# michal7kw/scRNA_seq_QAnnealing_Clustering

Measured on AMD Instinct MI355X. Metric: spin-flip updates/sec (node) + best QUBO energy vs neal, PBMC3k SNN, higher is better.
Workload: dtype f32

## Files before the change

### include/mi_sa.h

```cpp
#ifndef MI_SA_H
#define MI_SA_H

#include <stdint.h>

#ifdef __cplusplus
extern "C" {
#endif

#define MI_OK            0
#define MI_EINVAL       -1
#define MI_ENODEV       -2
#define MI_EHIP         -3
#define MI_ENOMEM       -4
#define MI_EUNSUPPORTED -5
#define MI_ESTATE       -6

#define MI_KIND_DENSE     1
#define MI_KIND_CSR_RANK1 2
#define MI_KIND_POTTS_CSR 3

typedef struct mi_sa_problem mi_sa_problem;

const char *mi_last_error(void);
int mi_abi_version(void);
int mi_device_count(int *out_count);
int mi_device_info(int device, char *name, int len, int *out_cus, uint64_t *out_hbm_bytes);


int mi_sa_problem_create_dense_f32(const float *Qs, int n, double offset, int device,
                                   mi_sa_problem **out);

int mi_sa_problem_create_csr_rank1_f32(const int32_t *rowptr, const int32_t *col, const float *val,
                                       const float *lin, float c_pair, int n, double offset,
                                       int device, mi_sa_problem **out);

int mi_sa_problem_create_potts_csr_f32(const int32_t *rowptr, const int32_t *col, const float *val,
                                       float c_pair, int n, int K, double lin_offset, int device,
                                       mi_sa_problem **out);

int mi_sa_problem_set_energy_model_f64(mi_sa_problem *p, const double *val, const double *lin, double c_pair);

int mi_sa_problem_destroy(mi_sa_problem *p);
int mi_sa_problem_info(const mi_sa_problem *p, int *kind, int *n, int *num_cases, int *device);

int mi_sa_set_option(mi_sa_problem *p, const char *key, long value);

int mi_sa_debug_pace(mi_sa_problem *p, unsigned int *out, int words);

int mi_sa_plan_slot_order(const int32_t *rowptr, const int32_t *col, int n, int slot, int64_t *out_perm);

int mi_sa_plan_slot_layout(const int32_t *rowptr, const int32_t *col, int n, int slot, int max_slots,
                           int64_t *out_pos, int *out_slots, int *out_clashes);

int mi_sa_problem_set_absent(mi_sa_problem *p, const uint8_t *absent);

int mi_sa_problem_set_pair_weights(mi_sa_problem *p, const int32_t *weights);

int mi_sa_problem_set_node_weights(mi_sa_problem *p, const int32_t *wq, const float *cw, const double *w64);

int mi_sa_problem_set_node_weight_groups(mi_sa_problem *p, int G, const float *cw, const double *c64, const double *offset);

int mi_sa_problem_set_merge_moves(mi_sa_problem *p, int interval, int proposals, const double *cq);

int mi_sa_debug_stats(mi_sa_problem *p, uint64_t *out, int words);


int mi_sa_anneal(mi_sa_problem *p, int R, uint32_t replica_offset, int num_sweeps,
                 const double *betas, uint64_t seed, const void *init, int resync_interval);

#define MI_F_CONTINUE         1u
#define MI_F_BETA_PER_REPLICA 2u
#define MI_F_TEMPS_RESIDENT   4u
#define MI_F_BETA_PER_GROUP   8u
int mi_sa_anneal_ex(mi_sa_problem *p, int R, uint32_t replica_offset, int num_sweeps,
                    const double *betas, uint64_t seed, const void *init, int resync_interval,
                    uint32_t sweep_offset, uint32_t flags);

int mi_sa_tempering_begin(mi_sa_problem *p, const double *ladder_betas, int T, int chains,
                          uint32_t first_replica, int R_local);
int mi_sa_tempering_exchange(mi_sa_problem *p, uint32_t round, uint64_t seed, const double *all_energies);
int mi_sa_tempering_exchange_dev(mi_sa_problem *p, uint32_t round, uint64_t seed, const double *d_all_energies);
int mi_sa_tempering_state(mi_sa_problem *p, int32_t *out_rung, uint64_t *out_proposed, uint64_t *out_accepted);

int mi_sa_sync(mi_sa_problem *p);

int mi_sa_device_results(mi_sa_problem *p, void **out_d_states, double **out_d_energy, int *out_R);

int mi_sa_last_kernel_ms(mi_sa_problem *p, float *out_ms);

int mi_sa_last_launch_count(mi_sa_problem *p, int *out_launches);

int mi_sa_last_kernel_name(mi_sa_problem *p, char *out, int len);

int mi_sa_fetch(mi_sa_problem *p, void *out_states, double *out_energy, uint64_t *out_stats);

int mi_sa_problem_label_agreement(mi_sa_problem *p, int groups, double *out_ari, double *out_nmi, int64_t *out_pair_sum,
                                  float *out_kernel_ms);

int mi_sa_problem_coassociation(mi_sa_problem *p, int groups, const uint16_t *ref, int Kref, const int32_t *eu,
                                const int32_t *ev, int64_t m, int64_t *out_hist, int64_t *out_rowsum, int32_t *out_edge,
                                int32_t *out_counts, float *out_kernel_ms);

int mi_sa_problem_components(mi_sa_problem *p, int32_t *out_labels, int32_t *out_count, float *out_kernel_ms);

int mi_sa_best(mi_sa_problem *p, int *out_index, double *out_energy, uint64_t *out_key,
               void *out_state);

int mi_multi_gpu_anneal(mi_sa_problem *const *problems, int ndev, int R_total, uint32_t replica_offset,
                        int num_sweeps, const double *betas, uint64_t seed, int resync_interval);
int mi_multi_gpu_best(mi_sa_problem *const *problems, int ndev, int *out_owner, uint32_t *out_global_id,
                      double *out_energy, void *out_state);
int mi_multi_gpu_fetch(mi_sa_problem *const *problems, int ndev, void *out_states, double *out_energy,
                       uint64_t *out_stats);


int mi_sa_qubo_dense_f32(const float *Qs, int n, double offset, int R, int num_sweeps,
                         const double *betas, uint64_t seed, const uint8_t *init,
                         uint8_t *out_states, double *out_energy, uint64_t *out_stats, int device);

int mi_energy_dense_f32(const float *Qs, int n, const uint8_t *X, int R, double offset,
                        double *out_energy, int device);
int mi_energy_dense_f64(const double *Qs, int n, const uint8_t *X, int R, double offset,
                        double *out_energy, int device);
int mi_energy_dense_f32_ex(const float *Qs, int n, const uint8_t *X, int R, double offset,
                           double *out_energy, int device, int path, float *out_kernel_ms);

#ifdef __cplusplus
}
#endif
#endif
```

### scrna_seq_qannealing_clustering_amd/_lib.py

```python
from __future__ import annotations

import ctypes as C
import os
import threading

_HERE = os.path.dirname(os.path.abspath(__file__))
LIB_PATH = os.environ.get("MI_SA_LIB") or os.path.join(_HERE, "libmi_sa.so")

MI_OK = 0
KIND_DENSE, KIND_CSR_RANK1, KIND_POTTS_CSR = 1, 2, 3

_lock = threading.Lock()
_lib = None


class MiSaError(RuntimeError):

    def __init__(self, code, message):
        super().__init__("libmi_sa error %d: %s" % (code, message))
        self.code = code
        self.message = message


def _declare(lib):
    u8p, u16p = C.POINTER(C.c_uint8), C.POINTER(C.c_uint16)
    i32p, f32p, f64p = C.POINTER(C.c_int32), C.POINTER(C.c_float), C.POINTER(C.c_double)
    u64p, ip, vp = C.POINTER(C.c_uint64), C.POINTER(C.c_int), C.c_void_p
    pp = C.POINTER(C.c_void_p)
    sig = {
        "mi_last_error": (C.c_char_p, []),
        "mi_abi_version": (C.c_int, []),
        "mi_device_count": (C.c_int, [ip]),
        "mi_device_info": (C.c_int, [C.c_int, C.c_char_p, C.c_int, ip, u64p]),
        "mi_sa_problem_create_dense_f32": (C.c_int, [f32p, C.c_int, C.c_double, C.c_int, pp]),
        "mi_sa_problem_create_csr_rank1_f32": (C.c_int, [i32p, i32p, f32p, f32p, C.c_float, C.c_int,
                                                         C.c_double, C.c_int, pp]),
        "mi_sa_problem_create_potts_csr_f32": (C.c_int, [i32p, i32p, f32p, C.c_float, C.c_int,
                                                         C.c_int, C.c_double, C.c_int, pp]),
        "mi_sa_problem_destroy": (C.c_int, [vp]),
        "mi_sa_problem_info": (C.c_int, [vp, ip, ip, ip, ip]),
        "mi_sa_set_option": (C.c_int, [vp, C.c_char_p, C.c_long]),
        "mi_sa_plan_slot_order": (C.c_int, [i32p, i32p, C.c_int, C.c_int, C.POINTER(C.c_int64)]),
        "mi_sa_problem_set_absent": (C.c_int, [C.c_void_p, C.POINTER(C.c_uint8)]),
        "mi_sa_problem_set_pair_weights": (C.c_int, [C.c_void_p, C.POINTER(C.c_int32)]),
        "mi_sa_problem_set_node_weights": (C.c_int, [C.c_void_p, C.POINTER(C.c_int32), C.POINTER(C.c_float),
                                                     C.POINTER(C.c_double)]),
        "mi_sa_problem_set_node_weight_groups": (C.c_int, [C.c_void_p, C.c_int, C.POINTER(C.c_float),
                                                           C.POINTER(C.c_double), C.POINTER(C.c_double)]),
        "mi_sa_problem_set_merge_moves": (C.c_int, [C.c_void_p, C.c_int, C.c_int, C.POINTER(C.c_double)]),
        "mi_sa_plan_slot_layout": (C.c_int, [i32p, i32p, C.c_int, C.c_int, C.c_int, C.POINTER(C.c_int64), C.POINTER(C.c_int), C.POINTER(C.c_int)]),
        "mi_sa_problem_set_energy_model_f64": (C.c_int, [vp, C.POINTER(C.c_double), C.POINTER(C.c_double), C.c_double]),
        "mi_sa_debug_pace": (C.c_int, [vp, C.POINTER(C.c_uint32), C.c_int]),
        "mi_sa_debug_stats": (C.c_int, [vp, u64p, C.c_int]),
        "mi_sa_anneal": (C.c_int, [vp, C.c_int, C.c_uint32, C.c_int, f64p, C.c_uint64, vp, C.c_int]),
        "mi_sa_anneal_ex": (C.c_int, [vp, C.c_int, C.c_uint32, C.c_int, f64p, C.c_uint64, vp, C.c_int,
                                      C.c_uint32, C.c_uint32]),
        "mi_sa_tempering_begin": (C.c_int, [vp, f64p, C.c_int, C.c_int, C.c_uint32, C.c_int]),
        "mi_sa_tempering_exchange": (C.c_int, [vp, C.c_uint32, C.c_uint64, f64p]),
        "mi_sa_tempering_exchange_dev": (C.c_int, [vp, C.c_uint32, C.c_uint64, vp]),
        "mi_sa_device_results": (C.c_int, [vp, pp, pp, ip]),
        "mi_sa_tempering_state": (C.c_int, [vp, i32p, u64p, u64p]),
        "mi_sa_sync": (C.c_int, [vp]),
        "mi_sa_last_kernel_ms": (C.c_int, [vp, f32p]),
        "mi_sa_last_launch_count": (C.c_int, [vp, ip]),
        "mi_sa_last_kernel_name": (C.c_int, [vp, C.c_char_p, C.c_int]),
        "mi_sa_fetch": (C.c_int, [vp, vp, f64p, u64p]),
        "mi_sa_best": (C.c_int, [vp, ip, f64p, u64p, vp]),
        "mi_multi_gpu_anneal": (C.c_int, [pp, C.c_int, C.c_int, C.c_uint32, C.c_int, f64p, C.c_uint64, C.c_int]),
        "mi_multi_gpu_best": (C.c_int, [pp, C.c_int, ip, C.POINTER(C.c_uint32), f64p, vp]),
        "mi_multi_gpu_fetch": (C.c_int, [pp, C.c_int, vp, f64p, u64p]),
        "mi_sa_qubo_dense_f32": (C.c_int, [f32p, C.c_int, C.c_double, C.c_int, C.c_int, f64p,
                                           C.c_uint64, u8p, u8p, f64p, u64p, C.c_int]),
        "mi_energy_dense_f32": (C.c_int, [f32p, C.c_int, u8p, C.c_int, C.c_double, f64p, C.c_int]),
        "mi_energy_dense_f64": (C.c_int, [f64p, C.c_int, u8p, C.c_int, C.c_double, f64p, C.c_int]),
        "mi_energy_dense_f32_ex": (C.c_int, [f32p, C.c_int, u8p, C.c_int, C.c_double, f64p, C.c_int, C.c_int,
                                             f32p]),
        "mi_snn_build_f32": (C.c_int, [f32p, C.c_int, C.c_int, C.c_int, C.c_double, C.c_int, C.c_int, pp]),
        "mi_snn_build_ex_f32": (C.c_int, [f32p, C.c_int, C.c_int, C.c_int, C.c_double, C.c_int, C.c_uint32, C.c_double,
                                          C.c_int, C.c_int, pp]),
        "mi_snn_build_rounded_f32": (C.c_int, [f32p, C.c_int, C.c_int, C.c_int, C.c_double, C.c_int, C.c_int, C.c_double,
                                               C.c_int, pp]),
        "mi_snn_fetch_codes": (C.c_int, [vp, u8p]),
        "mi_snn_info": (C.c_int, [vp, ip, ip, C.POINTER(C.c_int64), ip]),
        "mi_snn_fetch": (C.c_int, [vp, i32p, C.POINTER(C.c_int64), i32p, i32p]),
        "mi_snn_kernel_ms": (C.c_int, [vp, f32p, f32p, f32p]),
        "mi_snn_destroy": (C.c_int, [vp]),
        "mi_jaccard_cluster_stats": (C.c_int, [u64p, C.c_int, C.c_int, i32p, C.c_int, C.c_int, f64p, f64p, f64p, f64p,
                                               f64p, f32p, f32p]),
        "mi_label_agreement_u16": (C.c_int, [u16p, C.c_int, u16p, C.c_int, C.c_int, C.c_int, C.c_int, C.c_int, C.c_int,
                                             C.c_int, f64p, f64p, C.POINTER(C.c_int64), i32p, f32p]),
        "mi_sa_problem_label_agreement": (C.c_int, [vp, C.c_int, f64p, f64p, C.POINTER(C.c_int64), f32p]),
        "mi_coassociation_u16": (C.c_int, [u16p, C.c_int, C.c_int, C.c_int, C.c_int, u16p, C.c_int, i32p, i32p, C.c_int64,
                                           C.c_int, C.POINTER(C.c_int64), C.POINTER(C.c_int64), i32p, i32p, f32p]),
        "mi_sa_problem_coassociation": (C.c_int, [vp, C.c_int, u16p, C.c_int, i32p, i32p, C.c_int64, C.POINTER(C.c_int64),
                                                  C.POINTER(C.c_int64), i32p, i32p, f32p]),
        "mi_graph_components": (C.c_int, [i32p, i32p, C.c_int, u16p, u8p, C.c_int, C.c_int, C.c_uint32, i32p, i32p, f32p]),
        "mi_sa_problem_components": (C.c_int, [vp, i32p, i32p, f32p]),
        "mi_rank_sum_markers_f32": (C.c_int, [f32p, C.c_int, C.c_int, u16p, C.c_int, C.c_int, C.c_int, C.c_uint32,
                                              C.POINTER(C.c_int64), i32p, f64p, C.POINTER(C.c_int64), f32p]),
        "mi_prep_create_f32": (C.c_int, [f32p, C.c_int, C.c_int, C.c_int, pp]),
        "mi_prep_destroy": (C.c_int, [vp]),
        "mi_prep_normalize": (C.c_int, [vp, C.c_double, f32p]),
        "mi_prep_fetch_normalized": (C.c_int, [vp, f32p]),
        "mi_prep_gene_stats": (C.c_int, [vp, C.c_int, f64p, f64p, i32p, f32p]),
        "mi_prep_clipped_variance": (C.c_int, [vp, f64p, f64p, C.c_double, f64p, f32p]),
        "mi_prep_select": (C.c_int, [vp, i32p, C.c_int, f64p, f64p, C.c_double, f32p]),
        "mi_prep_fetch_scaled": (C.c_int, [vp, f32p]),
        "mi_prep_gram": (C.c_int, [vp, f64p, f32p]),
        "mi_prep_project": (C.c_int, [vp, f32p, C.c_int, f32p, f32p]),
    }
    for name, (res, args) in sig.items():
        fn = getattr(lib, name)
        fn.restype = res
        fn.argtypes = args
    return sig


EXPORTS = (
    "mi_last_error", "mi_abi_version", "mi_device_count", "mi_device_info",
    "mi_sa_problem_create_dense_f32", "mi_sa_problem_create_csr_rank1_f32",
    "mi_sa_problem_create_potts_csr_f32", "mi_sa_problem_destroy", "mi_sa_problem_info",
    "mi_sa_set_option", "mi_sa_plan_slot_order", "mi_sa_plan_slot_layout", "mi_sa_problem_set_absent", "mi_sa_problem_set_pair_weights", "mi_sa_problem_set_node_weights", "mi_sa_problem_set_node_weight_groups", "mi_sa_problem_set_merge_moves", "mi_sa_problem_set_energy_model_f64", "mi_sa_debug_pace", "mi_sa_debug_stats", "mi_sa_anneal", "mi_sa_anneal_ex", "mi_sa_tempering_begin", "mi_sa_tempering_exchange", "mi_sa_tempering_exchange_dev", "mi_sa_device_results", "mi_sa_tempering_state", "mi_sa_sync", "mi_sa_last_kernel_ms", "mi_sa_last_launch_count", "mi_sa_last_kernel_name", "mi_sa_fetch", "mi_sa_best",
    "mi_multi_gpu_anneal", "mi_multi_gpu_best", "mi_multi_gpu_fetch", "mi_sa_qubo_dense_f32", "mi_energy_dense_f32", "mi_energy_dense_f64", "mi_energy_dense_f32_ex",
    "mi_snn_build_f32", "mi_snn_build_ex_f32", "mi_snn_build_rounded_f32", "mi_snn_fetch_codes", "mi_snn_info", "mi_snn_fetch", "mi_snn_kernel_ms", "mi_snn_destroy",
    "mi_jaccard_cluster_stats", "mi_label_agreement_u16", "mi_sa_problem_label_agreement",
    "mi_coassociation_u16", "mi_sa_problem_coassociation",
    "mi_graph_components", "mi_sa_problem_components",
    "mi_rank_sum_markers_f32",
    "mi_prep_create_f32", "mi_prep_destroy", "mi_prep_normalize", "mi_prep_fetch_normalized", "mi_prep_gene_stats",
    "mi_prep_clipped_variance", "mi_prep_select", "mi_prep_fetch_scaled", "mi_prep_gram", "mi_prep_project",
)


def load():
    global _lib
    with _lock:
        if _lib is not None:
            return _lib
        if not os.path.exists(LIB_PATH):
            raise RuntimeError(
                "MI355X engine not built: %s is missing.  Build it with "
                "`python -c 'import __graft_entry__ as g; g.build()'` or "
                "`make -C scrna_seq_qannealing_clustering_amd/csrc`.  There is no CPU fallback."
                % LIB_PATH)
        try:
            import torch
        except Exception:
            pass
        try:
            lib = C.CDLL(LIB_PATH, mode=getattr(os, "RTLD_NOW", 2))
        except OSError as exc:
            raise RuntimeError("cannot load %s: %s (no CPU fallback exists)" % (LIB_PATH, exc)) from exc
        _declare(lib)
        _lib = lib
        return _lib


def check(code):
    if code != MI_OK:
        msg = load().mi_last_error()
        raise MiSaError(code, msg.decode("utf-8", "replace") if msg else "")
    return code


def device_count() -> int:
    n = C.c_int(0)
    rc = load().mi_device_count(C.byref(n))
    if rc != MI_OK:
        return 0
    return int(n.value)


def device_info(device: int = 0):
    name = C.create_string_buffer(256)
    cus = C.c_int(0)
    mem = C.c_uint64(0)
    check(load().mi_device_info(device, name, 256, C.byref(cus), C.byref(mem)))
    return {"name": name.value.decode(), "compute_units": int(cus.value), "hbm_bytes": int(mem.value)}
```

### scrna_seq_qannealing_clustering_amd/csrc/mi_sa.hip

```cpp

#include <algorithm>
#include <cmath>
#include <cstdarg>
#include <cstdint>
#include <cstdio>
#include <cstdlib>
#include <cstring>
#include <mutex>
#include <new>
#include <string>
#include <thread>
#include <type_traits>
#include <vector>

#include "../../include/mi_sa.h"

#include "mi_sa_device.h"

namespace mi_sa_impl {

thread_local std::string g_err;

thread_local std::string g_kernel;

void note_kernel(const char *fmt, ...)
{
    char buf[128];
    va_list ap;
    va_start(ap, fmt);
    vsnprintf(buf, sizeof buf, fmt, ap);
    va_end(ap);
    if (g_kernel.find(buf) == std::string::npos) g_kernel += (g_kernel.empty() ? "" : " + ") + std::string(buf);
}

int fail(int code, const char *fmt, ...)
{
    char buf[512];
    va_list ap;
    va_start(ap, fmt);
    vsnprintf(buf, sizeof buf, fmt, ap);
    va_end(ap);
    g_err = buf;
    return code;
}



__device__ __forceinline__ uint32_t sortable_f32(float v)
{
    const uint32_t b = __float_as_uint(v);
    return (b & 0x80000000u) ? ~b : (b | 0x80000000u);
}

__global__ void __launch_bounds__(1024) k_best(const double *__restrict__ energy, int R,
                                               uint32_t replica_offset,
                                               unsigned long long *__restrict__ out_key)
{
    __shared__ double s_e[16];
    __shared__ int s_i[16];
    double be = INFINITY;
    int bi = 0x7fffffff;
    for (int r = threadIdx.x; r < R; r += blockDim.x) {
        const double e = energy[r];
        if (e < be || (e == be && r < bi)) { be = e; bi = r; }
    }
#pragma unroll
    for (int off = 32; off > 0; off >>= 1) {
        const double oe = __shfl_xor(be, off, 64);
        const int oi = __shfl_xor(bi, off, 64);
        if (oe < be || (oe == be && oi < bi)) { be = oe; bi = oi; }
    }
    if ((threadIdx.x & 63) == 0) { s_e[threadIdx.x >> 6] = be; s_i[threadIdx.x >> 6] = bi; }
    __syncthreads();
    if (threadIdx.x == 0) {
        for (int w = 1; w < (int)(blockDim.x >> 6); ++w)
            if (s_e[w] < be || (s_e[w] == be && s_i[w] < bi)) { be = s_e[w]; bi = s_i[w]; }
        if (bi == 0x7fffffff) bi = 0;
        out_key[0] = ((unsigned long long)sortable_f32((float)energy[bi]) << 32) |
                     (unsigned long long)(replica_offset + (uint32_t)bi);
    }
}

__global__ void __launch_bounds__(256) k_pt_exchange(const double *__restrict__ energy, int *__restrict__ rung,
                                                     const double *__restrict__ betas,
                                                     const float *__restrict__ ladder_temps,
                                                     float *__restrict__ temps_local, int T, int lo, int hi,
                                                     uint32_t rnd, uint32_t seed_lo, uint32_t seed_hi,
                                                     unsigned long long *__restrict__ stats)
{
    extern __shared__ int holder[];
    const int c = blockIdx.x;
    for (int t = threadIdx.x; t < T; t += blockDim.x) holder[rung[c * T + t]] = c * T + t;
    __syncthreads();
    unsigned int proposed = 0, accepted = 0;
    for (int k = (int)(rnd & 1u) + 2 * (int)threadIdx.x; k + 1 < T; k += 2 * (int)blockDim.x) {
        const int a = holder[k], b = holder[k + 1];
        const double arg = (betas[k] - betas[k + 1]) * (energy[a] - energy[b]);
        ++proposed;
        const bool acc = arg >= 0.0 ||
                         -arg < (double)neglog_u(chain_word_dev((uint32_t)(c * T + k), rnd, 0xffffffffu, 3u, seed_lo, seed_hi));
        if (acc) {
            rung[a] = k + 1;
            rung[b] = k;
            ++accepted;
        }
    }
    __syncthreads();
    for (int t = threadIdx.x; t < T; t += blockDim.x) {
        const int g = c * T + t;
        if (g >= lo && g < hi) temps_local[g - lo] = ladder_temps[rung[g]];
    }
    if (proposed) { atomicAdd(&stats[0], (unsigned long long)proposed); atomicAdd(&stats[1], (unsigned long long)accepted); }
}

}
using namespace mi_sa_impl;

struct mi_sa_problem {
    int kind = 0, n = 0, K = 0, device = 0;
    double offset = 0.0;
    hipStream_t stream = nullptr;
    hipEvent_t ev0 = nullptr, ev1 = nullptr;
    int NT = 0;
    float *d_Qp = nullptr;
    float *d_Qm = nullptr;
    float *d_Qs = nullptr;
    float *d_Q2xl = nullptr, *d_diagxl = nullptr;
    void *d_xg = nullptr;
    size_t xg_bytes = 0;
    int opt_xl_batched = 0;
    int opt_xl_chain = 0;
    int opt_xl_chunk = 8;
    int opt_xl_cold_permille = 20;
    int opt_xl_async = 1;
    std::thread worker;
    int worker_rc = MI_OK;
    std::string worker_err, worker_kernel;
    int xl_chunks = 0;
    int slots = 0, D = 0;
    float c_pair = 0.0f;
    uint32_t *d_ell_col = nullptr;
    float *d_ell_val = nullptr, *d_lin = nullptr;
    double *d_ell_val64 = nullptr, *d_lin64 = nullptr;
    double c_pair64 = 0.0;
    std::vector<int32_t> h_rowptr;
    uint2 *d_rows = nullptr;
    uint32_t *d_meta = nullptr;
    std::vector<uint32_t> h_meta;
    std::vector<uint8_t> h_hole;
    uint4 *d_adj4 = nullptr;
    uint4 *d_adj4p = nullptr;
    uint4 *d_adj4r = nullptr;
    int k2p_rw = 0;
    std::vector<uint32_t> h_adj4r;
    uint32_t *d_slot_flags = nullptr;
    int k2_state_bytes = 0;
    int32_t *d_wgt = nullptr;
    int wslot = -1;
    int32_t *d_nwq = nullptr;
    float *d_ncw = nullptr;
    double *d_nw64 = nullptr;
    int ngroups = 1;
    double *d_gconst = nullptr;
    int merge_interval = 0, merge_proposals = 0;
    std::vector<double> merge_cq;
    double *d_merge_cq = nullptr;
    double merge_sumabs = 0.0;
    int k2_free_block = 0;
    int cus = 0;
    int cap_R = 0, cap_sweeps = 0;
    int last_R = 0;
    uint32_t last_offset = 0;
    bool has_run = false;
    float *d_temps = nullptr;
    void *d_init = nullptr;
    void *d_states = nullptr;
    double *d_energy = nullptr;
    unsigned long long *d_stats = nullptr;
    unsigned int *d_pace = nullptr;
    int opt_pace = 1;
    int opt_variant = 0;
    int opt_mfma_permille = 600;

    int opt_chunk_sweeps = 32;
    float *d_fields = nullptr;
    unsigned int *d_ctrl = nullptr;
    int cap_fields_R = 0;
    int opt_ondemand_permille = 40;
    int opt_debug = 0;
    int opt_min_cluster_size = 0;
    int opt_k2_waves = 0;
    int opt_k2_pair = 0;
    int opt_k2_split = 0;
    int opt_k2_wide = 0;
    int opt_k3_fast = 0;
    int opt_k2_tw = 0;
    int opt_k2_trim = 0;
    int opt_k2_split_max = 1024;
    int opt_unit_rows = 0;
    int resident_waves = 0;
    int last_launches = 1;
    std::string last_kernel;
    size_t state_elem = 1;
    int pt_T = 0, pt_chains = 0, pt_lo = 0, pt_R_local = 0;
    int *d_pt_rung = nullptr;
    double *d_pt_betas = nullptr, *d_pt_energy = nullptr;
    float *d_pt_ladder = nullptr;
    float *d_pt_temps = nullptr;
    unsigned long long *d_pt_stats = nullptr;
};

namespace {

int select_device(int device)
{
    int cnt = 0;
    hipError_t e = hipGetDeviceCount(&cnt);
    if (e != hipSuccess || cnt <= 0)
        return fail(MI_ENODEV, "no HIP device visible (%s)", hipGetErrorString(e));
    if (device < 0 || device >= cnt) return fail(MI_EINVAL, "device %d out of range [0,%d)", device, cnt);
    HIP_TRY(hipSetDevice(device));
    return MI_OK;
}

int ensure_run_buffers(mi_sa_problem *p, int R, int num_sweeps, bool need_init)
{
    if (R > p->cap_R) {
        if (p->d_states) (void)hipFree(p->d_states);
        if (p->d_energy) (void)hipFree(p->d_energy);
        if (p->d_init) { (void)hipFree(p->d_init); p->d_init = nullptr; }
        p->d_states = nullptr; p->d_energy = nullptr;
        HIP_TRY(hipMalloc(&p->d_states, (size_t)R * p->n * p->state_elem));
        HIP_TRY(hipMalloc((void **)&p->d_energy, (size_t)R * sizeof(double)));
        p->cap_R = R;
    }
    if (need_init && !p->d_init) HIP_TRY(hipMalloc(&p->d_init, (size_t)p->cap_R * p->n * p->state_elem));
    if (num_sweeps > p->cap_sweeps || !p->d_temps) {
        if (p->d_temps) (void)hipFree(p->d_temps);
        p->d_temps = nullptr;
        HIP_TRY(hipMalloc((void **)&p->d_temps, (size_t)(num_sweeps > 0 ? num_sweeps : 1) * sizeof(float)));
        p->cap_sweeps = num_sweeps;
    }
    return MI_OK;
}

int dispatch_dense(mi_sa_problem *p, const DenseArgs &a, hipStream_t st)
{
    if (p->opt_chunk_sweeps > 0 && a.num_sweeps > p->opt_chunk_sweeps && p->opt_variant != 1 && a.R >= 32 &&
        (p->cap_fields_R < a.R || !p->d_fields)) {
        if (p->d_fields) (void)hipFree(p->d_fields);
        p->d_fields = nullptr;
        HIP_TRY(hipMalloc((void **)&p->d_fields, (size_t)a.R * p->NT * 64 * sizeof(float)));
        p->cap_fields_R = a.R;
    }
    if (!p->d_ctrl) {
        HIP_TRY(hipMalloc((void **)&p->d_ctrl, kCtrlWords * sizeof(unsigned int)));
        HIP_TRY(hipMemset(p->d_ctrl, 0, kCtrlWords * sizeof(unsigned int)));
    }
    DenseLaunchCtx ctx{p->device, p->opt_pace, p->opt_variant, p->opt_unit_rows, p->opt_ondemand_permille,
                       p->opt_chunk_sweeps, p->opt_mfma_permille, p->d_fields, p->d_ctrl, p->d_pace, &p->resident_waves,
                       &p->last_launches};
    p->last_launches = 1;
    switch (p->NT) {
#define MI_CASE(N) case N: return mi_launch_dense_nt##N(ctx, a, st);
        MI_CASE(4) MI_CASE(8) MI_CASE(12) MI_CASE(16) MI_CASE(20) MI_CASE(24) MI_CASE(28)
        MI_CASE(32) MI_CASE(36) MI_CASE(40) MI_CASE(44) MI_CASE(48) MI_CASE(52) MI_CASE(56)
        MI_CASE(60) MI_CASE(64)
#undef MI_CASE
    }
    return fail(MI_EUNSUPPORTED, "dense kernel not built for NT=%d", p->NT);
}

constexpr int kMaxDenseN = 64 * 64;
constexpr int kMaxDenseXlN = 16 * 4096;

}

static int settle(mi_sa_problem *p)
{
    if (!p || !p->worker.joinable()) return MI_OK;
    p->worker.join();
    p->last_kernel = p->worker_kernel;
    if (p->worker_rc) {
        const int rc = p->worker_rc;
        p->worker_rc = MI_OK;
        return fail(rc, "%s", p->worker_err.c_str());
    }
    return MI_OK;
}

extern "C" {

const char *mi_last_error(void) { return g_err.c_str(); }

int mi_abi_version(void) { return 1; }

int mi_device_count(int *out_count)
{
    if (!out_count) return fail(MI_EINVAL, "out_count is NULL");
    int cnt = 0;
    hipError_t e = hipGetDeviceCount(&cnt);
    if (e != hipSuccess) { *out_count = 0; return fail(MI_ENODEV, "hipGetDeviceCount: %s", hipGetErrorString(e)); }
    *out_count = cnt;
    return MI_OK;
}

int mi_device_info(int device, char *name, int len, int *out_cus, uint64_t *out_hbm_bytes)
{
    int rc = select_device(device);
    if (rc) return rc;
    hipDeviceProp_t prop;
    HIP_TRY(hipGetDeviceProperties(&prop, device));
    if (name && len > 0) snprintf(name, (size_t)len, "%s (%s)", prop.name, prop.gcnArchName);
    if (out_cus) *out_cus = prop.multiProcessorCount;
    if (out_hbm_bytes) *out_hbm_bytes = (uint64_t)prop.totalGlobalMem;
    return MI_OK;
}

static int problem_common_init(mi_sa_problem *p, int device)
{
    p->device = device;
    HIP_TRY(hipStreamCreateWithFlags(&p->stream, hipStreamNonBlocking));
    HIP_TRY(hipEventCreate(&p->ev0));
    HIP_TRY(hipEventCreate(&p->ev1));
    HIP_TRY(hipMalloc((void **)&p->d_stats, 16 * sizeof(unsigned long long)));
    HIP_TRY(hipMemset(p->d_stats, 0, 16 * sizeof(unsigned long long)));
    HIP_TRY(hipMalloc((void **)&p->d_pace, kMaxChunks * kPaceWords * sizeof(unsigned int)));
    HIP_TRY(hipDeviceGetAttribute(&p->cus, hipDeviceAttributeMultiprocessorCount, device));
    return MI_OK;
}

int mi_sa_problem_create_dense_f32(const float *Qs, int n, double offset, int device,
                                   mi_sa_problem **out)
{
    if (!Qs || !out) return fail(MI_EINVAL, "NULL argument");
    if (n < 1) return fail(MI_EINVAL, "n must be >= 1 (got %d)", n);
    if (n > kMaxDenseXlN)
        return fail(MI_EUNSUPPORTED, "dense kernels support n <= %d (got %d)", kMaxDenseXlN, n);
    int rc = select_device(device);
    if (rc) return rc;
    mi_sa_problem *p = new (std::nothrow) mi_sa_problem();
    if (!p) return fail(MI_ENOMEM, "out of host memory");
    p->kind = MI_KIND_DENSE; p->n = n; p->offset = offset; p->state_elem = 1;
    rc = problem_common_init(p, device);
    if (rc) { mi_sa_problem_destroy(p); return rc; }
    if (n > kMaxDenseN) {
        p->xl_chunks = (n + 4095) / 4096;
        const size_t xstride = (size_t)p->xl_chunks * 4096;
        rc = guarded([&]() -> int {
            HIP_TRY(hipMalloc((void **)&p->d_Q2xl, (size_t)n * xstride * sizeof(float)));
            HIP_TRY(hipMalloc((void **)&p->d_diagxl, xstride * sizeof(float)));
            const int rows_per_block = 256;
            std::vector<float> blk((size_t)rows_per_block * xstride), hd(xstride, 0.0f);
            for (int r0 = 0; r0 < n; r0 += rows_per_block) {
                const int nr = n - r0 < rows_per_block ? n - r0 : rows_per_block;
                std::fill(blk.begin(), blk.begin() + (size_t)nr * xstride, 0.0f);
                for (int i = 0; i < nr; ++i) {
                    const float *row = Qs + (size_t)(r0 + i) * n;
                    float *dst = blk.data() + (size_t)i * xstride;
                    for (int j = 0; j < n; ++j) dst[j] = row[j] + row[j];
                    dst[r0 + i] = 0.0f;
                    hd[r0 + i] = row[r0 + i];
                }
                HIP_TRY(hipMemcpy(p->d_Q2xl + (size_t)r0 * xstride, blk.data(), (size_t)nr * xstride * sizeof(float), hipMemcpyHostToDevice));
            }
            HIP_TRY(hipMemcpy(p->d_diagxl, hd.data(), xstride * sizeof(float), hipMemcpyHostToDevice));
            return MI_OK;
        });
        if (rc) { mi_sa_problem_destroy(p); return rc; }
        *out = p;
        return MI_OK;
    }
    rc = guarded([&]() -> int {
        const int slots = (n + 63) / 64;
        p->NT = ((slots + 3) / 4) * 4;
        const size_t stride = (size_t)p->NT * 64;
        const int diag_row = slots * 64;
        std::vector<float> hp((size_t)(diag_row + 1) * stride, 0.0f);
        for (int i = 0; i < n; ++i) {
            const float *row = Qs + (size_t)i * n;
            float *dst = hp.data() + (size_t)i * stride;
            for (int j = 0; j < n; ++j) {
                if (j == i) continue;
                const int t = j >> 6, lane = j & 63;
                dst[((size_t)(t >> 2) * 64 + lane) * 4 + (t & 3)] = row[j] + row[j];
            }
            hp[(size_t)diag_row * stride + ((size_t)((i >> 6) >> 2) * 64 + (i & 63)) * 4 + ((i >> 6) & 3)] = row[i];
        }
        HIP_TRY(hipMalloc((void **)&p->d_Qp, hp.size() * sizeof(float)));
        HIP_TRY(hipMemcpy(p->d_Qp, hp.data(), hp.size() * sizeof(float), hipMemcpyHostToDevice));
        if (p->NT <= kMaxMfmaNT) {
            const size_t npad = (size_t)p->NT * 64;
            std::vector<float> hm((npad + 1) * npad, 0.0f);
            for (int i = 0; i < n; ++i) {
                const float *row = Qs + (size_t)i * n;
                float *dst = hm.data() + (size_t)i * npad;
                for (int j = 0; j < n; ++j) dst[j] = (j == i) ? 0.0f : row[j] + row[j];
                hm[npad * npad + i] = row[i];
            }
            HIP_TRY(hipMalloc((void **)&p->d_Qm, hm.size() * sizeof(float)));
            HIP_TRY(hipMemcpy(p->d_Qm, hm.data(), hm.size() * sizeof(float), hipMemcpyHostToDevice));
        }
        return MI_OK;
    });
    if (rc) { mi_sa_problem_destroy(p); return rc; }
    *out = p;
    return MI_OK;
}

static std::vector<uint32_t> pack_pair_adjacency(const std::vector<uint32_t> &hc, const std::vector<float> &hv, int slots, int D, int RW)
{
    const int G = D / 4, LW = RW - 4 * (G - 1);
    const size_t slot_words = (size_t)(G - 1) * 512 + (LW == 3 ? 448 : (size_t)LW * 128);
    std::vector<uint32_t> out((size_t)slots * slot_words, 0u);
    for (int t = 0; t < slots; ++t)
        for (int lane = 0; lane < 64; ++lane)
            for (int k = 0; k < RW; ++k) {
                const int g = k / 4, w = g < G - 1 ? 4 : LW;
                const size_t grp = (size_t)t * slot_words + (size_t)g * 512;
                size_t at_col = grp + (size_t)lane * w + (k & 3), at_val = at_col + (size_t)w * 64;
                if (w == 3) {
                    at_col = grp + (size_t)lane * 4 + (k & 3);
                    at_val = (k & 3) < 2 ? grp + 256 + (size_t)lane * 2 + (k & 3) : grp + 384 + (size_t)lane;
                }
                out[at_col] = 4u * hc[((size_t)t * D + k) * 64 + lane];
                memcpy(&out[at_val], &hv[((size_t)t * D + k) * 64 + lane], 4);
            }
    return out;
}

static int upload_slot_ell(mi_sa_problem *p, const int32_t *rowptr, const int32_t *col, const float *val, int n)
{
    int maxdeg = 0;
    for (int i = 0; i < n; ++i) {
        const int d = rowptr[i + 1] - rowptr[i];
        if (d < 0) return fail(MI_EINVAL, "rowptr is not monotone at %d", i);
        if (d > maxdeg) maxdeg = d;
    }
    if (maxdeg > 4096)
        return fail(MI_EUNSUPPORTED, "max degree %d exceeds the widest adjacency layout (4096); use the dense kernel", maxdeg);
    const int D = maxdeg <= 16 ? 16 : (maxdeg <= 32 ? 32 : (maxdeg <= 64 ? 64 : ((maxdeg + 15) / 16) * 16));
    const int slots = (n + 63) / 64;
    std::vector<uint32_t> hc((size_t)slots * D * 64);
    std::vector<float> hv((size_t)slots * D * 64, 0.0f);
    for (int t = 0; t < slots; ++t)
        for (int lane = 0; lane < 64; ++lane) {
            const int i = t * 64 + lane;
            for (int k = 0; k < D; ++k) hc[((size_t)t * D + k) * 64 + lane] = (uint32_t)(i < n ? i : 0);
            if (i >= n) continue;
            for (int e = rowptr[i], k = 0; e < rowptr[i + 1]; ++e, ++k) {
                if (col[e] < 0 || col[e] >= n || col[e] == i)
                    return fail(MI_EINVAL, "bad column %d in row %d", col[e], i);
                hc[((size_t)t * D + k) * 64 + lane] = (uint32_t)col[e];
                hv[((size_t)t * D + k) * 64 + lane] = val[e];
            }
        }
    HIP_TRY(hipMalloc((void **)&p->d_ell_col, hc.size() * sizeof(uint32_t)));
    HIP_TRY(hipMalloc((void **)&p->d_ell_val, hv.size() * sizeof(float)));
    HIP_TRY(hipMemcpy(p->d_ell_col, hc.data(), hc.size() * sizeof(uint32_t), hipMemcpyHostToDevice));
    HIP_TRY(hipMemcpy(p->d_ell_val, hv.data(), hv.size() * sizeof(float), hipMemcpyHostToDevice));
    p->slots = slots;
    p->D = D;
    p->h_rowptr.assign(rowptr, rowptr + n + 1);
    {
        std::vector<uint2> hr((size_t)slots * 64 * D);
        std::vector<uint32_t> hm((size_t)slots * 64, 0u);
        for (int i = 0; i < slots * 64; ++i) {
            uint2 *row = hr.data() + (size_t)i * D;
            for (int k = 0; k < D; ++k) row[k] = make_uint2((uint32_t)(i < n ? i : 0), 0u);
            if (i >= n) { hm[i] = 0x80000000u; continue; }
            int k = 0, nin = 0;
            for (int pass = 0; pass < 2; ++pass)
                for (int e = rowptr[i]; e < rowptr[i + 1]; ++e) {
                    const bool in_slot = (col[e] >> 6) == (i >> 6);
                    if (in_slot != (pass == 0)) continue;
                    uint32_t bits;
                    memcpy(&bits, &val[e], 4);
                    row[k++] = make_uint2((uint32_t)col[e], bits);
                    nin += in_slot ? 1 : 0;
                }
            hm[i] = (uint32_t)nin | ((uint32_t)k << 8);
        }
        HIP_TRY(hipMalloc((void **)&p->d_rows, hr.size() * sizeof(uint2)));
        HIP_TRY(hipMalloc((void **)&p->d_meta, hm.size() * sizeof(uint32_t)));
        HIP_TRY(hipMemcpy(p->d_rows, hr.data(), hr.size() * sizeof(uint2), hipMemcpyHostToDevice));
        HIP_TRY(hipMemcpy(p->d_meta, hm.data(), hm.size() * sizeof(uint32_t), hipMemcpyHostToDevice));
        p->h_meta = hm;
        if (p->kind == MI_KIND_POTTS_CSR && (D == 16 || D == 32) && (size_t)slots * 128 + 256 <= 160 * 1024) {
            bool any_in_slot = false;
            for (size_t i = 0; i < hm.size(); ++i) any_in_slot = any_in_slot || (hm[i] & 0xffu) != 0u;
            if (!any_in_slot) {
                const int G = D / 4;
                std::vector<uint32_t> ha((size_t)slots * G * 2 * 64 * 4, 0u);
                for (int t = 0; t < slots; ++t)
                    for (int lane = 0; lane < 64; ++lane)
                        for (int k = 0; k < D; ++k) {
                            const size_t base = (((size_t)t * G + k / 4) * 2) * 256 + (size_t)lane * 4 + (k & 3);
                            ha[base] = 2u * hc[((size_t)t * D + k) * 64 + lane];
                            memcpy(&ha[base + 256], &hv[((size_t)t * D + k) * 64 + lane], 4);
                        }
                HIP_TRY(hipMalloc((void **)&p->d_adj4p, ha.size() * sizeof(uint32_t)));
                HIP_TRY(hipMemcpy(p->d_adj4p, ha.data(), ha.size() * sizeof(uint32_t), hipMemcpyHostToDevice));
            }
        }
        if (p->kind == MI_KIND_CSR_RANK1) {
            const int G = D / 4;
            const char *force = getenv("MI_K2_STATE");
#ifdef MI_K2_DEBUG_BUILD
            const bool debug_linear = getenv("MI_K2_DEBUG_LINEAR") != nullptr;
#endif
            const bool fits_half = (size_t)slots * 128 * 16 <= 144 * 1024, fits_byte = (size_t)slots * 64 * 16 <= 144 * 1024;
            p->k2_state_bytes = fits_half ? 2 : (fits_byte ? 1 : 0);
            if (force && !strcmp(force, "byte") && fits_byte) p->k2_state_bytes = 1;
            if (force && !strcmp(force, "bit")) p->k2_state_bytes = 0;
            std::vector<uint32_t> ha((size_t)slots * G * 2 * 64 * 4, 0u), hf((size_t)slots, 0u);
            for (int t = 0; t < slots; ++t)
                for (int lane = 0; lane < 64; ++lane) {
                    if (hm[(size_t)t * 64 + lane] & 0xffu) hf[t] = 1u;
                    for (int k = 0; k < D; ++k) {
                        const uint32_t c = hc[((size_t)t * D + k) * 64 + lane];
                        uint32_t vb;
                        memcpy(&vb, &hv[((size_t)t * D + k) * 64 + lane], 4);
                        const size_t base = (((size_t)t * G + k / 4) * 2) * 256 + (size_t)lane * 4 + (k & 3);
#ifdef MI_K2_DEBUG_BUILD
                        if (debug_linear) {
                            ha[base] = (uint32_t)((lane * 2 + ((k * 128) % (slots * 128))));
                            ha[base + 256] = vb;
                            continue;
                        }
#endif
                        ha[base] = p->k2_state_bytes == 2 ? 2u * c
                                 : (p->k2_state_bytes == 1 ? c : ((((c >> 5) * 4u) << 8) | (c & 31u)));
                        ha[base + 256] = vb;
                    }
                }
            HIP_TRY(hipMalloc((void **)&p->d_adj4, ha.size() * sizeof(uint32_t)));
            HIP_TRY(hipMalloc((void **)&p->d_slot_flags, hf.size() * sizeof(uint32_t)));
            HIP_TRY(hipMemcpy(p->d_adj4, ha.data(), ha.size() * sizeof(uint32_t), hipMemcpyHostToDevice));
            HIP_TRY(hipMemcpy(p->d_slot_flags, hf.data(), hf.size() * sizeof(uint32_t), hipMemcpyHostToDevice));
            bool any_general = false;
            for (int t = 0; t < slots; ++t) any_general = any_general || hf[t] != 0u;
            p->k2_free_block = any_general ? 0 : 64;
            for (int B : {256, 128}) {
                if (any_general || slots % 4 != 0) continue;
                bool ok = true;
                for (int i = 0; i < n && ok; ++i)
                    for (int e = rowptr[i]; e < rowptr[i + 1]; ++e)
                        if (col[e] / B == i / B) { ok = false; break; }
                if (ok) { p->k2_free_block = B; break; }
            }
            if (!any_general && (D == 16 || D == 32) && (size_t)slots * 256 + 4096 <= 160 * 1024) {
                for (int t = 0; t < slots; ++t)
                    for (int lane = 0; lane < 64; ++lane)
                        for (int k = 0; k < D; ++k)
                            ha[(((size_t)t * G + k / 4) * 2) * 256 + (size_t)lane * 4 + (k & 3)] =
#ifdef MI_K2_DEBUG_BUILD
                                debug_linear ? (uint32_t)(lane * 4 + (k * 256) % (slots * 256)) :
#endif
                                4u * hc[((size_t)t * D + k) * 64 + lane];
                HIP_TRY(hipMalloc((void **)&p->d_adj4p, ha.size() * sizeof(uint32_t)));
                HIP_TRY(hipMemcpy(p->d_adj4p, ha.data(), ha.size() * sizeof(uint32_t), hipMemcpyHostToDevice));
                if (D == 16 && maxdeg >= 13 && maxdeg < 16) {
                    p->h_adj4r = pack_pair_adjacency(hc, hv, slots, D, maxdeg);
                    p->k2p_rw = maxdeg;
                    if (maxdeg != 15) {
                        HIP_TRY(hipMalloc((void **)&p->d_adj4r, p->h_adj4r.size() * sizeof(uint32_t)));
                        HIP_TRY(hipMemcpy(p->d_adj4r, p->h_adj4r.data(), p->h_adj4r.size() * sizeof(uint32_t), hipMemcpyHostToDevice));
                        std::vector<uint32_t>().swap(p->h_adj4r);
                    }
                }
            }
        }
    }
    return MI_OK;
}

static int plan_slot_order_impl(const int32_t *rowptr, const int32_t *col, int n, int slot, int64_t *perm)
{
    const int nslots = (n + slot - 1) / slot;
    if (nslots <= 1 || n > (1 << 18)) {
        for (int i = 0; i < n; ++i) perm[i] = i;
        return MI_OK;
    }
    for (int i = 0; i < n; ++i)
        if (rowptr[i + 1] < rowptr[i]) return fail(MI_EINVAL, "rowptr is not monotone at %d", i);
    int maxdeg = 0;
    for (int i = 0; i < n; ++i) maxdeg = std::max(maxdeg, rowptr[i + 1] - rowptr[i]);
    std::vector<int> start((size_t)maxdeg + 2, 0), order((size_t)n);
    for (int i = 0; i < n; ++i) start[(size_t)(maxdeg - (rowptr[i + 1] - rowptr[i])) + 1]++;
    for (int d = 0; d <= maxdeg; ++d) start[(size_t)d + 1] += start[(size_t)d];
    for (int i = 0; i < n; ++i) order[(size_t)start[(size_t)(maxdeg - (rowptr[i + 1] - rowptr[i]))]++] = i;
    std::vector<int> fill((size_t)nslots, 0), cap((size_t)nslots, slot), where((size_t)n, -1), stamp((size_t)nslots, -1);
    cap[(size_t)nslots - 1] = n - slot * (nslots - 1);
    for (int v : order) {
        for (int e = rowptr[v]; e < rowptr[v + 1]; ++e) {
            if (col[e] < 0 || col[e] >= n) return fail(MI_EINVAL, "bad column %d in row %d", col[e], v);
            const int w = where[(size_t)col[e]];
            if (w >= 0) stamp[(size_t)w] = v;
        }
        int best = -1, best_nb = -1;
        for (int s = 0; s < nslots; ++s) {
            if (fill[(size_t)s] >= cap[(size_t)s]) continue;
            if (stamp[(size_t)s] == v) { if (best_nb < 0 || fill[(size_t)s] < fill[(size_t)best_nb]) best_nb = s; }
            else if (best < 0 || fill[(size_t)s] < fill[(size_t)best]) best = s;
        }
        const int s = best >= 0 ? best : best_nb;
        where[(size_t)v] = s;
        fill[(size_t)s]++;
    }
    std::vector<int> pos((size_t)nslots + 1, 0);
    for (int i = 0; i < n; ++i) pos[(size_t)where[(size_t)i] + 1]++;
    for (int s = 0; s < nslots; ++s) pos[(size_t)s + 1] += pos[(size_t)s];
    for (int i = 0; i < n; ++i) perm[pos[(size_t)where[(size_t)i]]++] = i;
    return MI_OK;
}

static int greedy_slots(const int32_t *rowptr, const int32_t *col, int n, int slot, int nslots,
                        const std::vector<int> &order, std::vector<int> &where)
{
    std::vector<int> fill((size_t)nslots, 0), stamp((size_t)nslots, -1);
    where.assign((size_t)n, -1);
    int clashes = 0;
    for (int v : order) {
        for (int e = rowptr[v]; e < rowptr[v + 1]; ++e) {
            const int w = where[(size_t)col[e]];
            if (w >= 0) stamp[(size_t)w] = v;
        }
        int best = -1, best_nb = -1;
        for (int s = 0; s < nslots; ++s) {
            if (fill[(size_t)s] >= slot) continue;
            if (stamp[(size_t)s] == v) { if (best_nb < 0 || fill[(size_t)s] < fill[(size_t)best_nb]) best_nb = s; }
            else if (best < 0 || fill[(size_t)s] < fill[(size_t)best]) best = s;
        }
        const int s = best >= 0 ? best : best_nb;
        if (best < 0) ++clashes;
        where[(size_t)v] = s;
        fill[(size_t)s]++;
    }
    return clashes;
}

static int plan_slot_layout_impl(const int32_t *rowptr, const int32_t *col, int n, int slot, int max_slots,
                                 int64_t *pos, int *out_slots, int *out_clashes)
{
    const int s0 = (n + slot - 1) / slot;
    if (max_slots < s0) max_slots = s0;
    for (int i = 0; i < n; ++i) {
        if (rowptr[i + 1] < rowptr[i]) return fail(MI_EINVAL, "rowptr is not monotone at %d", i);
        for (int e = rowptr[i]; e < rowptr[i + 1]; ++e)
            if (col[e] < 0 || col[e] >= n) return fail(MI_EINVAL, "bad column %d in row %d", col[e], i);
    }
    if (n > (1 << 18)) {
        int clashes = 0;
        for (int i = 0; i < n; ++i) {
            pos[i] = i;
            for (int e = rowptr[i]; e < rowptr[i + 1]; ++e)
                if (col[e] / slot == i / slot) { ++clashes; break; }
        }
        *out_slots = s0;
        if (out_clashes) *out_clashes = clashes;
        return MI_OK;
    }
    int maxdeg = 0;
    for (int i = 0; i < n; ++i) maxdeg = std::max(maxdeg, rowptr[i + 1] - rowptr[i]);
    std::vector<int> start((size_t)maxdeg + 2, 0), order((size_t)n);
    for (int i = 0; i < n; ++i) start[(size_t)(maxdeg - (rowptr[i + 1] - rowptr[i])) + 1]++;
    for (int d = 0; d <= maxdeg; ++d) start[(size_t)d + 1] += start[(size_t)d];
    for (int i = 0; i < n; ++i) order[(size_t)start[(size_t)(maxdeg - (rowptr[i + 1] - rowptr[i]))]++] = i;
    std::vector<int> where, first_where;
    int nslots = s0, clashes = 0, first_clashes = 0;
    for (;;) {
        clashes = greedy_slots(rowptr, col, n, slot, nslots, order, where);
        if (nslots == s0) { first_where = where; first_clashes = clashes; }
        if (clashes == 0) break;
        const int next = nslots + std::max(1, nslots / 8);
        if (next > max_slots) { where = first_where; clashes = first_clashes; nslots = s0; break; }
        nslots = next;
    }
    if (clashes == 0 && nslots > s0 && n <= 2048) {
        const int C = nslots;
        std::vector<unsigned char> seen((size_t)n * C, 0);
        std::vector<int> sat((size_t)n, 0), colour((size_t)n, -1), fill2((size_t)C, 0);
        int used = 0;
        bool ok = true;
        for (int step = 0; step < n && ok; ++step) {
            int v = -1;
            for (int u = 0; u < n; ++u) {
                if (colour[(size_t)u] >= 0) continue;
                if (v < 0) { v = u; continue; }
                const int du = rowptr[u + 1] - rowptr[u], dv = rowptr[v + 1] - rowptr[v];
                if (sat[(size_t)u] > sat[(size_t)v] || (sat[(size_t)u] == sat[(size_t)v] && du > dv)) v = u;
            }
            int c = 0;
            while (c < C && (seen[(size_t)v * C + c] || fill2[(size_t)c] >= slot)) ++c;
            if (c >= C) { ok = false; break; }
            colour[(size_t)v] = c;
            fill2[(size_t)c]++;
            used = std::max(used, c + 1);
            if (used >= C) { ok = false; break; }
            for (int e = rowptr[v]; e < rowptr[v + 1]; ++e) {
                const int u = col[e];
                if (!seen[(size_t)u * C + c]) { seen[(size_t)u * C + c] = 1; sat[(size_t)u]++; }
            }
        }
        if (ok && used < nslots && used >= s0) {
            where = colour;
            nslots = used;
        }
    }
    std::vector<int> seat((size_t)nslots, 0);
    for (int i = 0; i < n; ++i) pos[i] = (int64_t)where[(size_t)i] * slot + seat[(size_t)where[(size_t)i]]++;
    *out_slots = nslots;
    if (out_clashes) *out_clashes = clashes;
    return MI_OK;
}

int mi_sa_plan_slot_layout(const int32_t *rowptr, const int32_t *col, int n, int slot, int max_slots,
                           int64_t *out_pos, int *out_slots, int *out_clashes)
{
    if (!rowptr || !out_pos || !out_slots || (n > 0 && rowptr[n] > 0 && !col)) return fail(MI_EINVAL, "NULL argument");
    if (n < 1 || slot < 1) return fail(MI_EINVAL, "n and slot must be >= 1");
    return guarded([&]() -> int { return plan_slot_layout_impl(rowptr, col, n, slot, max_slots, out_pos, out_slots, out_clashes); });
}

int mi_sa_plan_slot_order(const int32_t *rowptr, const int32_t *col, int n, int slot, int64_t *out_perm)
{
    if (!rowptr || !out_perm || (n > 0 && rowptr[n] > 0 && !col)) return fail(MI_EINVAL, "NULL argument");
    if (n < 0 || slot < 1) return fail(MI_EINVAL, "n must be >= 0 and slot >= 1");
    return guarded([&]() -> int { return plan_slot_order_impl(rowptr, col, n, slot, out_perm); });
}

int mi_sa_problem_create_csr_rank1_f32(const int32_t *rowptr, const int32_t *col, const float *val,
                                       const float *lin, float c_pair, int n, double offset, int device,
                                       mi_sa_problem **out)
{
    if (!rowptr || !lin || !out || (rowptr[n > 0 ? n : 0] > 0 && (!col || !val))) return fail(MI_EINVAL, "NULL argument");
    if (n < 1) return fail(MI_EINVAL, "n must be >= 1 (got %d)", n);
    if (n > (1 << 20)) return fail(MI_EUNSUPPORTED, "csr_rank1 kernel supports n <= 1048576 (got %d)", n);
    int rc = select_device(device);
    if (rc) return rc;
    mi_sa_problem *p = new (std::nothrow) mi_sa_problem();
    if (!p) return fail(MI_ENOMEM, "out of host memory");
    p->kind = MI_KIND_CSR_RANK1; p->n = n; p->K = 2; p->offset = offset; p->state_elem = 1; p->c_pair = c_pair;
    rc = problem_common_init(p, device);
    if (!rc) rc = guarded([&]() -> int { return upload_slot_ell(p, rowptr, col, val, n); });
    if (!rc) rc = guarded([&]() -> int {
        std::vector<float> hl((size_t)p->slots * 64, INFINITY);
        for (int i = 0; i < n; ++i) hl[i] = lin[i];
        p->h_hole.assign((size_t)n, 0);
        for (int i = 0; i < n; ++i) p->h_hole[(size_t)i] = std::isinf(lin[i]) ? 1 : 0;
        HIP_TRY(hipMalloc((void **)&p->d_lin, hl.size() * sizeof(float)));
        HIP_TRY(hipMemcpy(p->d_lin, hl.data(), hl.size() * sizeof(float), hipMemcpyHostToDevice));
        if (!p->h_adj4r.empty()) {
            const size_t slot_words = p->h_adj4r.size() / (size_t)p->slots;
            for (int t = 0; t < p->slots; ++t)
                for (int lane = 0; lane < 64; ++lane)
                    memcpy(&p->h_adj4r[(size_t)t * slot_words + 3 * 512 + (size_t)lane * 4 + 3], &hl[(size_t)t * 64 + lane], 4);
            HIP_TRY(hipMalloc((void **)&p->d_adj4r, p->h_adj4r.size() * sizeof(uint32_t)));
            HIP_TRY(hipMemcpy(p->d_adj4r, p->h_adj4r.data(), p->h_adj4r.size() * sizeof(uint32_t), hipMemcpyHostToDevice));
            std::vector<uint32_t>().swap(p->h_adj4r);
        }
        return MI_OK;
    });
    if (rc) { mi_sa_problem_destroy(p); return rc; }
    *out = p;
    return MI_OK;
}

int mi_sa_problem_create_potts_csr_f32(const int32_t *rowptr, const int32_t *col, const float *val,
                                       float c_pair, int n, int K, double lin_offset, int device,
                                       mi_sa_problem **out)
{
    if (!rowptr || !out || (rowptr[n > 0 ? n : 0] > 0 && (!col || !val))) return fail(MI_EINVAL, "NULL argument");
    if (n < 1) return fail(MI_EINVAL, "n must be >= 1 (got %d)", n);
    if (K < 1 || K > 64) return fail(MI_EUNSUPPORTED, "potts kernel supports 1 <= K <= 64 cases (got %d)", K);
    if (n > 40000) return fail(MI_EUNSUPPORTED, "potts kernel supports n <= 40000 (got %d)", n);
    int rc = select_device(device);
    if (rc) return rc;
    mi_sa_problem *p = new (std::nothrow) mi_sa_problem();
    if (!p) return fail(MI_ENOMEM, "out of host memory");
    p->kind = MI_KIND_POTTS_CSR; p->n = n; p->K = K; p->offset = lin_offset; p->state_elem = 2; p->c_pair = c_pair;
    for (int e = 0; e < rowptr[n]; ++e) p->merge_sumabs += std::fabs((double)val[e]);
    rc = problem_common_init(p, device);
    if (!rc) rc = guarded([&]() -> int { return upload_slot_ell(p, rowptr, col, val, n); });
    if (rc) { mi_sa_problem_destroy(p); return rc; }
    *out = p;
    return MI_OK;
}

static int set_energy_model_impl(mi_sa_problem *p, const double *val, const double *lin, double c_pair)
{
    if (const int rc_w = settle(p)) return rc_w;
    if (!p) return fail(MI_EINVAL, "NULL problem");
    if (p->kind != MI_KIND_CSR_RANK1 && p->kind != MI_KIND_POTTS_CSR)
        return fail(MI_EUNSUPPORTED, "an fp64 energy model is defined for the structured kinds only");
    const int n = p->n, D = p->D;
    const int64_t nnz = p->h_rowptr.empty() ? 0 : p->h_rowptr[n];
    if ((nnz > 0 && !val) || (p->kind == MI_KIND_CSR_RANK1 && !lin)) return fail(MI_EINVAL, "NULL argument");
    HIP_TRY(hipSetDevice(p->device));
    HIP_TRY(hipStreamSynchronize(p->stream));
    std::vector<double> hv((size_t)p->slots * D * 64, 0.0), hl((size_t)p->slots * 64, 0.0);
    for (int i = 0; i < n; ++i) {
        const int t = i >> 6, lane = i & 63;
        for (int e = p->h_rowptr[i], k = 0; e < p->h_rowptr[i + 1]; ++e, ++k) hv[((size_t)t * D + k) * 64 + lane] = val[e];
        if (lin) hl[i] = lin[i];
    }
    if (!p->d_ell_val64) HIP_TRY(hipMalloc((void **)&p->d_ell_val64, hv.size() * sizeof(double)));
    if (!p->d_lin64) HIP_TRY(hipMalloc((void **)&p->d_lin64, hl.size() * sizeof(double)));
    HIP_TRY(hipMemcpy(p->d_ell_val64, hv.data(), hv.size() * sizeof(double), hipMemcpyHostToDevice));
    HIP_TRY(hipMemcpy(p->d_lin64, hl.data(), hl.size() * sizeof(double), hipMemcpyHostToDevice));
    p->c_pair64 = c_pair;
    return MI_OK;
}

int mi_sa_problem_set_absent(mi_sa_problem *p, const uint8_t *absent)
{
    if (!p || !absent) return fail(MI_EINVAL, "NULL argument");
    if (const int rc_w = settle(p)) return rc_w;
    if (p->kind != MI_KIND_POTTS_CSR)
        return fail(MI_EUNSUPPORTED, "holes of a Potts model only (a binary CSR model marks them by lin = +inf)");
    return guarded([&]() -> int {
        for (int i = 0; i < p->n; ++i) {
            if (absent[i] && (p->h_meta[(size_t)i] & 0x00ffff00u))
                return fail(MI_EINVAL, "variable %d is marked absent but has couplings", i);
            p->h_meta[(size_t)i] = (p->h_meta[(size_t)i] & 0x7fffffffu) | (absent[i] ? 0x80000000u : 0u);
        }
        HIP_TRY(hipSetDevice(p->device));
        HIP_TRY(hipStreamSynchronize(p->stream));
        HIP_TRY(hipMemcpy(p->d_meta, p->h_meta.data(), p->h_meta.size() * sizeof(uint32_t), hipMemcpyHostToDevice));
        return MI_OK;
    });
}

int mi_sa_problem_set_pair_weights(mi_sa_problem *p, const int32_t *weights)
{
    if (!p || !weights) return fail(MI_EINVAL, "NULL argument");
    if (const int rc_w = settle(p)) return rc_w;
    if (p->kind != MI_KIND_CSR_RANK1)
        return fail(MI_EUNSUPPORTED, "pair-term weights: structured binary (CSR + uniform pair) problems only");
    return guarded([&]() -> int {
        int wslot = -1;
        for (int i = 0; i < p->n; ++i) {
            if (p->h_meta[(size_t)i] >> 31) continue;
            const bool hole = !p->h_hole.empty() && p->h_hole[(size_t)i];
            if (hole) continue;
            if (weights[i] < 1) return fail(MI_EINVAL, "weight %d of variable %d: weights are positive integers", weights[i], i);
            if (weights[i] > (1 << 20)) return fail(MI_EINVAL, "weight %d of variable %d exceeds 2^20", weights[i], i);
            if (weights[i] == 1) continue;
            if (p->h_rowptr[(size_t)i + 1] != p->h_rowptr[(size_t)i])
                return fail(MI_EINVAL, "variable %d has weight %d and sparse couplings: weighted variables couple through the pair term only", i, weights[i]);
            if (wslot >= 0 && wslot != i / 64)
                return fail(MI_EINVAL, "variables with weights other than 1 in slots %d and %d: they must share one 64-variable slot", wslot, i / 64);
            wslot = i / 64;
        }
        std::vector<int32_t> hw(64, 0);
        if (wslot >= 0) {
            for (int l = 0; l < 64; ++l) {
                const int i = wslot * 64 + l;
                if (i >= p->n || (!p->h_hole.empty() && p->h_hole[(size_t)i])) continue;
                hw[(size_t)l] = weights[i];
            }
            for (int l = 0; l < 64; ++l) {
                const int i = wslot * 64 + l;
                if (i < p->n && hw[(size_t)l] != 0 && p->h_rowptr[(size_t)i + 1] != p->h_rowptr[(size_t)i])
                    return fail(MI_EINVAL, "variable %d shares the weighted slot %d and has sparse couplings", i, wslot);
            }
        }
        HIP_TRY(hipSetDevice(p->device));
        HIP_TRY(hipStreamSynchronize(p->stream));
        if (!p->d_wgt) HIP_TRY(hipMalloc((void **)&p->d_wgt, 64 * sizeof(int32_t)));
        HIP_TRY(hipMemcpy(p->d_wgt, hw.data(), 64 * sizeof(int32_t), hipMemcpyHostToDevice));
        p->wslot = wslot;
        return MI_OK;
    });
}

int mi_sa_problem_set_node_weights(mi_sa_problem *p, const int32_t *wq, const float *cw, const double *w64)
{
    if (!p || !wq || !cw) return fail(MI_EINVAL, "NULL argument");
    if (const int rc_w = settle(p)) return rc_w;
    if (p->kind != MI_KIND_POTTS_CSR) return fail(MI_EINVAL, "node weights: Potts problems only");
    if (p->has_run) return fail(MI_EINVAL, "node weights must be set before the first anneal");
    if (p->opt_min_cluster_size > 0) return fail(MI_EUNSUPPORTED, "node weights together with min_cluster_size are not supported");
    return guarded([&]() -> int {
        const size_t seats = (size_t)p->slots * 64;
        std::vector<int32_t> hq(seats, 0);
        std::vector<float> hc(seats, 0.0f);
        std::vector<double> hw(seats, 0.0);
        int64_t total = 0;
        for (int i = 0; i < p->n; ++i) {
            if (p->h_meta[(size_t)i] >> 31) continue;
            if (wq[i] < 0 || (w64 && !(w64[i] >= 0.0)))
                return fail(MI_EINVAL, "weight of variable %d is negative", i);
            total += wq[i];
            if (total > (int64_t)1 << 30) return fail(MI_EINVAL, "the node weights sum to more than 2^30");
            hq[(size_t)i] = wq[i];
            hc[(size_t)i] = cw[i];
            hw[(size_t)i] = w64 ? w64[i] : (double)wq[i];
        }
        HIP_TRY(hipSetDevice(p->device));
        HIP_TRY(hipStreamSynchronize(p->stream));
        if (!p->d_nwq) HIP_TRY(hipMalloc((void **)&p->d_nwq, seats * sizeof(int32_t)));
        if (!p->d_ncw) HIP_TRY(hipMalloc((void **)&p->d_ncw, seats * sizeof(float)));
        if (!p->d_nw64) HIP_TRY(hipMalloc((void **)&p->d_nw64, seats * sizeof(double)));
        HIP_TRY(hipMemcpy(p->d_nwq, hq.data(), seats * sizeof(int32_t), hipMemcpyHostToDevice));
        HIP_TRY(hipMemcpy(p->d_ncw, hc.data(), seats * sizeof(float), hipMemcpyHostToDevice));
        HIP_TRY(hipMemcpy(p->d_nw64, hw.data(), seats * sizeof(double), hipMemcpyHostToDevice));
        return MI_OK;
    });
}

int mi_sa_problem_set_node_weight_groups(mi_sa_problem *p, int G, const float *cw, const double *c64, const double *offset)
{
    if (!p || !cw || !c64 || !offset) return fail(MI_EINVAL, "NULL argument");
    if (const int rc_w = settle(p)) return rc_w;
    if (G < 1 || G > 256) return fail(MI_EINVAL, "resolution groups: 1 .. 256 (got %d)", G);
    if (!p->d_nwq) return fail(MI_EINVAL, "resolution groups need node weights (mi_sa_problem_set_node_weights) first");
    if (p->has_run) return fail(MI_EINVAL, "resolution groups must be set before the first anneal");
    return guarded([&]() -> int {
        const size_t seats = (size_t)p->slots * 64;
        std::vector<float> hc((size_t)G * seats, 0.0f);
        for (int g = 0; g < G; ++g) {
            for (int i = 0; i < p->n; ++i)
                if (!(p->h_meta[(size_t)i] >> 31)) hc[(size_t)g * seats + i] = cw[(size_t)g * p->n + i];
        }
        HIP_TRY(hipSetDevice(p->device));
        HIP_TRY(hipStreamSynchronize(p->stream));
        if (G != p->ngroups) {
            HIP_TRY(hipFree(p->d_ncw));
            p->d_ncw = nullptr;
            HIP_TRY(hipMalloc((void **)&p->d_ncw, (size_t)G * seats * sizeof(float)));
            p->ngroups = G;
        }
        if (!p->d_gconst) HIP_TRY(hipMalloc((void **)&p->d_gconst, 2 * 256 * sizeof(double)));
        std::vector<double> hk(c64, c64 + G);
        hk.insert(hk.end(), offset, offset + G);
        HIP_TRY(hipMemcpy(p->d_ncw, hc.data(), hc.size() * sizeof(float), hipMemcpyHostToDevice));
        HIP_TRY(hipMemcpy(p->d_gconst, hk.data(), hk.size() * sizeof(double), hipMemcpyHostToDevice));
        return MI_OK;
    });
}

static int merge_fixed_exponent(double sumabs)
{
    if (!(sumabs > 0.0)) return 0;
    int E = 0;
    const double m = std::frexp(sumabs, &E);
    const int f = 62 - E + (m == 0.5 ? 1 : 0);
    return f < -1000 ? -1000 : (f > 1000 ? 1000 : f);
}

int mi_sa_problem_set_merge_moves(mi_sa_problem *p, int interval, int proposals, const double *cq)
{
    if (!p) return fail(MI_EINVAL, "NULL problem");
    if (const int rc_w = settle(p)) return rc_w;
    if (p->kind != MI_KIND_POTTS_CSR) return fail(MI_EINVAL, "merge moves: Potts problems only");
    if (interval < 0) return fail(MI_EINVAL, "merge interval must be >= 0 (got %d)", interval);
    if (proposals < 1) return fail(MI_EINVAL, "merge proposals must be >= 1 (got %d)", proposals);
    if (interval == 0) { p->merge_interval = 0; return MI_OK; }
    if (p->K < 2) return fail(MI_EINVAL, "merge moves need K >= 2");
    if (p->d_nwq && !cq) return fail(MI_EINVAL, "merge moves on a problem with node weights need the coefficients cq");
    if (p->opt_min_cluster_size > 0) return fail(MI_EUNSUPPORTED, "merge moves together with min_cluster_size are not supported");
    if (p->pt_T > 0) return fail(MI_EUNSUPPORTED, "merge moves under tempering are not supported");
    return guarded([&]() -> int {
        const int G = p->ngroups;
        std::vector<double> h((size_t)G, (double)p->c_pair);
        if (cq)
            for (int g = 0; g < G; ++g) {
                if (!std::isfinite(cq[g])) return fail(MI_EINVAL, "cq[%d] is not finite", g);
                h[(size_t)g] = cq[g];
            }
        HIP_TRY(hipSetDevice(p->device));
        HIP_TRY(hipStreamSynchronize(p->stream));
        if (!p->d_merge_cq) HIP_TRY(hipMalloc((void **)&p->d_merge_cq, 256 * sizeof(double)));
        HIP_TRY(hipMemcpy(p->d_merge_cq, h.data(), h.size() * sizeof(double), hipMemcpyHostToDevice));
        p->merge_cq = cq ? h : std::vector<double>();
        p->merge_interval = interval;
        p->merge_proposals = proposals;
        return MI_OK;
    });
}

int mi_sa_problem_set_energy_model_f64(mi_sa_problem *p, const double *val, const double *lin, double c_pair)
{
    return guarded([&]() -> int { return set_energy_model_impl(p, val, lin, c_pair); });
}

int mi_sa_problem_destroy(mi_sa_problem *p)
{
    if (!p) return MI_OK;
    (void)settle(p);
    (void)hipSetDevice(p->device);
    if (p->stream) (void)hipStreamSynchronize(p->stream);
    void *bufs[] = {p->d_merge_cq, p->d_gconst, p->d_nwq, p->d_ncw, p->d_nw64, p->d_wgt, p->d_xg, p->d_pt_rung, p->d_pt_betas, p->d_pt_energy, p->d_pt_ladder, p->d_pt_temps, p->d_pt_stats, p->d_adj4p, p->d_adj4r, p->d_ell_val64, p->d_lin64, p->d_Q2xl, p->d_diagxl, p->d_rows, p->d_meta, p->d_adj4, p->d_slot_flags, p->d_Qm, p->d_fields, p->d_ctrl, p->d_ell_col, p->d_ell_val, p->d_lin, p->d_pace, p->d_Qp, p->d_Qs, p->d_temps, p->d_init, p->d_states, p->d_energy, p->d_stats};
    for (void *b : bufs)
        if (b) (void)hipFree(b);
    if (p->ev0) (void)hipEventDestroy(p->ev0);
    if (p->ev1) (void)hipEventDestroy(p->ev1);
    if (p->stream) (void)hipStreamDestroy(p->stream);
    delete p;
    return MI_OK;
}

int mi_sa_problem_info(const mi_sa_problem *p, int *kind, int *n, int *num_cases, int *device)
{
    if (!p) return fail(MI_EINVAL, "NULL problem");
    if (kind) *kind = p->kind;
    if (n) *n = p->n;
    if (num_cases) *num_cases = p->K;
    if (device) *device = p->device;
    return MI_OK;
}

int mi_sa_debug_stats(mi_sa_problem *p, uint64_t *out, int words)
{
    if (!p || !out) return fail(MI_EINVAL, "NULL argument");
    if (const int rc_w = settle(p)) return rc_w;
    HIP_TRY(hipSetDevice(p->device));
    HIP_TRY(hipStreamSynchronize(p->stream));
    if (words > 16) words = 16;
    HIP_TRY(hipMemcpy(out, p->d_stats, (size_t)words * sizeof(uint64_t), hipMemcpyDeviceToHost));
    if (words == 16 && p->d_ctrl) {
        unsigned int c[2] = {0, 0};
        HIP_TRY(hipMemcpy(c, p->d_ctrl + 4, sizeof c, hipMemcpyDeviceToHost));
        out[14] = c[0]; out[15] = c[1];
    }
    return MI_OK;
}

int mi_sa_debug_pace(mi_sa_problem *p, unsigned int *out, int words)
{
    if (!p || !out) return fail(MI_EINVAL, "NULL argument");
    if (const int rc_w = settle(p)) return rc_w;
    HIP_TRY(hipSetDevice(p->device));
    HIP_TRY(hipStreamSynchronize(p->stream));
    if (words > kPaceWords) words = kPaceWords;
    HIP_TRY(hipMemcpy(out, p->d_pace, (size_t)words * sizeof(unsigned int), hipMemcpyDeviceToHost));
    return MI_OK;
}

int mi_sa_set_option(mi_sa_problem *p, const char *key, long value)
{
    if (!p || !key) return fail(MI_EINVAL, "NULL argument");
    if (const int rc_w = settle(p)) return rc_w;
    if (!strcmp(key, "pace")) { p->opt_pace = value != 0; return MI_OK; }
    if (!strcmp(key, "xl_batched") && value >= 0 && value <= 2) { p->opt_xl_batched = (int)value; return MI_OK; }
    if (!strcmp(key, "xl_chunk") && value >= 1) { p->opt_xl_chunk = (int)value; return MI_OK; }
    if (!strcmp(key, "xl_chain") && value >= 0 && value <= 2) { p->opt_xl_chain = (int)value; return MI_OK; }
    if (!strcmp(key, "xl_cold_permille") && value >= 0 && value <= 1000) { p->opt_xl_cold_permille = (int)value; return MI_OK; }
    if (!strcmp(key, "xl_async") && value >= 0 && value <= 1) { p->opt_xl_async = (int)value; return MI_OK; }
    if (!strcmp(key, "mfma_permille") && value >= 0 && value <= 1000) { p->opt_mfma_permille = (int)value; return MI_OK; }
    if (!strcmp(key, "chunk_sweeps") && value >= 0) { p->opt_chunk_sweeps = (int)value; return MI_OK; }
    if (!strcmp(key, "ondemand_permille") && value >= 0 && value <= 1000) { p->opt_ondemand_permille = (int)value; return MI_OK; }
    if (!strcmp(key, "debug")) { p->opt_debug = (int)value; return MI_OK; }
    if (!strcmp(key, "k2_waves") && ((value >= 0 && value <= 16) || value == 99)) { p->opt_k2_waves = (int)value; return MI_OK; }
    if (!strcmp(key, "k2_pair") && value >= 0 && value <= 2) { p->opt_k2_pair = (int)value; return MI_OK; }
    if (!strcmp(key, "k2_split") && value >= 0 && value <= 2) { p->opt_k2_split = (int)value; return MI_OK; }
    if (!strcmp(key, "k2_split_max") && value >= 0) { p->opt_k2_split_max = (int)value; return MI_OK; }
    if (!strcmp(key, "k2_wide") && value >= 0 && value <= 2) { p->opt_k2_wide = (int)value; return MI_OK; }
    if (!strcmp(key, "k2_tw") && value >= 0 && value <= 2) { p->opt_k2_tw = (int)value; return MI_OK; }
    if (!strcmp(key, "k2_trim") && value >= 0 && value <= 2) { p->opt_k2_trim = (int)value; return MI_OK; }
    if (!strcmp(key, "k3_fast") && value >= 0 && value <= 2) { p->opt_k3_fast = (int)value; return MI_OK; }
    if (!strcmp(key, "min_cluster_size") && value >= 0) {
        if (p->kind != MI_KIND_POTTS_CSR) return fail(MI_EINVAL, "min_cluster_size applies to Potts problems");
        if (value > 0 && p->d_nwq) return fail(MI_EUNSUPPORTED, "min_cluster_size together with node weights is not supported");
        if (value > 0 && p->merge_interval > 0) return fail(MI_EUNSUPPORTED, "min_cluster_size together with merge moves is not supported");
        p->opt_min_cluster_size = (int)value;
        return MI_OK;
    }
    if (!strcmp(key, "variant") && value >= 0 && value <= 4) { p->opt_variant = (int)value; return MI_OK; }
    if (!strcmp(key, "unit_rows") && (value == 0 || value == 2 || value == 4)) { p->opt_unit_rows = (int)value; return MI_OK; }
    return fail(MI_EINVAL, "unknown option '%s'", key);
}

static int anneal_ex_impl(mi_sa_problem *p, int R, uint32_t replica_offset, int num_sweeps,
                          const double *betas, uint64_t seed, const void *init, int resync_interval,
                          uint32_t sweep_offset, uint32_t flags)
{
    if (const int rc_w = settle(p)) return rc_w;
    const bool cont = (flags & MI_F_CONTINUE) != 0, resident = (flags & MI_F_TEMPS_RESIDENT) != 0;
    const bool per_replica = (flags & MI_F_BETA_PER_REPLICA) != 0 || resident;
    const bool per_group = (flags & MI_F_BETA_PER_GROUP) != 0;
    if (flags & ~(uint32_t)(MI_F_CONTINUE | MI_F_BETA_PER_REPLICA | MI_F_TEMPS_RESIDENT | MI_F_BETA_PER_GROUP))
        return fail(MI_EINVAL, "unknown flags 0x%x", flags);
    if (!p) return fail(MI_EINVAL, "NULL problem");
    const int G = p->ngroups;
    if (per_group && per_replica) return fail(MI_EINVAL, "MI_F_BETA_PER_GROUP together with per-replica temperatures");
    if (G > 1 && per_replica)
        return fail(MI_EUNSUPPORTED, "resolution groups together with per-replica or resident temperatures are not supported");
    if (R % G != 0) return fail(MI_EINVAL, "R = %d is not a multiple of the %d resolution groups", R, G);
    const int num_betas = per_replica ? R : (per_group ? G * num_sweeps : num_sweeps);
    if (resident && (p->pt_T == 0 || p->pt_R_local != R))
        return fail(MI_ESTATE, "MI_F_TEMPS_RESIDENT needs mi_sa_tempering_begin for %d replicas on this problem", R);
    if (R < 1) return fail(MI_EINVAL, "R must be >= 1 (got %d)", R);
    if (num_sweeps < 0) return fail(MI_EINVAL, "num_sweeps must be >= 0");
    if (num_betas > 0 && num_sweeps > 0 && !betas && !resident) return fail(MI_EINVAL, "betas is NULL");
    if (cont && (!p || !p->has_run || p->last_R != R))
        return fail(MI_ESTATE, "MI_F_CONTINUE needs a previous run with the same number of replicas");
    if (cont && init) return fail(MI_EINVAL, "MI_F_CONTINUE and init are mutually exclusive");
    if (resync_interval < 0) return fail(MI_EINVAL, "resync_interval must be >= 0");
    const bool merges = p->kind == MI_KIND_POTTS_CSR && p->merge_interval > 0 && num_sweeps > 0;
    if (merges && resident) return fail(MI_EUNSUPPORTED, "merge moves with resident (tempering) temperatures are not supported");
    if (merges && p->d_nwq && p->merge_cq.empty())
        return fail(MI_EINVAL, "merge moves on a problem with node weights need the coefficients cq");
    if (merges && !p->merge_cq.empty() && p->merge_cq.size() != (size_t)G)
        return fail(MI_EINVAL, "merge moves: %zu coefficients for %d resolution groups", p->merge_cq.size(), G);
    for (int s = 0; s < (num_sweeps > 0 && !resident ? num_betas : 0); ++s)
        if (!(betas[s] > 0.0) || !std::isfinite(betas[s]))
            return fail(MI_EINVAL, "betas[%d] = %g is not a positive finite number", s, betas[s]);
    HIP_TRY(hipSetDevice(p->device));
    int rc = ensure_run_buffers(p, R, G * num_sweeps > num_betas ? G * num_sweeps : num_betas, init != nullptr);
    if (rc) return rc;
    if (!resident) {
        std::vector<float> temps((size_t)(num_betas > 0 ? num_betas : 1), 1.0f);
        for (int s = 0; s < (num_sweeps > 0 ? num_betas : 0); ++s) temps[s] = (float)(1.0 / betas[s]);
        HIP_TRY(hipMemcpyAsync(p->d_temps, temps.data(), temps.size() * sizeof(float), hipMemcpyHostToDevice, p->stream));
    }
    if (init)
        HIP_TRY(hipMemcpyAsync(p->d_init, init, (size_t)R * p->n * p->state_elem, hipMemcpyHostToDevice, p->stream));
    HIP_TRY(hipMemsetAsync(p->d_stats, 0, 16 * sizeof(unsigned long long), p->stream));
    if (!resident || init)
        HIP_TRY(hipStreamSynchronize(p->stream));
    g_kernel.clear();
    const float *temps_buf = resident ? p->d_pt_temps : p->d_temps;

    if (p->kind == MI_KIND_DENSE && p->xl_chunks > 0) {
        DenseXlArgs a;
        a.Q2 = p->d_Q2xl; a.diag = p->d_diagxl; a.temps = temps_buf;
        a.init = cont ? (const uint8_t *)p->d_states : (init ? (const uint8_t *)p->d_init : nullptr);
        a.states = (uint8_t *)p->d_states; a.energy = p->d_energy; a.stats = p->d_stats;
        a.offset = p->offset; a.n = p->n; a.R = R; a.num_sweeps = num_sweeps; a.resync = resync_interval;
        a.replica_offset = replica_offset; a.seed_lo = (uint32_t)seed; a.seed_hi = (uint32_t)(seed >> 32);
        a.sweep_offset = sweep_offset; a.temps_per_replica = per_replica ? 1 : 0;
        a.xg_chain = p->opt_xl_chain;
        p->last_launches = 1;
        const bool batched = p->opt_xl_batched == 1 || (p->opt_xl_batched == 0 && (R >= 256 || p->n >= 16384));
        if (batched) {
            const size_t need = mi_dense_xg_workspace_bytes(p->n, R);
            if (need > p->xg_bytes) {
                if (p->d_xg) HIP_TRY(hipFree(p->d_xg));
                p->d_xg = nullptr; p->xg_bytes = 0;
                HIP_TRY(hipMalloc(&p->d_xg, need));
                p->xg_bytes = need;
            }
        }
        HIP_TRY(hipEventRecord(p->ev0, p->stream));
        if (!batched) {
            rc = mi_launch_dense_xl(a, p->xl_chunks, p->stream);
        } else if (resync_interval > 0 || per_replica || num_sweeps <= p->opt_xl_chunk || p->opt_xl_cold_permille == 0) {
            rc = mi_launch_dense_xg(a, p->xl_chunks, p->d_xg, p->stream, 3);
        } else {
            auto cooling_run = [p, a, num_sweeps, R]() -> int {
                HIP_TRY(hipSetDevice(p->device));
                int rc = MI_OK, s0 = 0;
                while (!rc && s0 < num_sweeps) {
                    const int len = num_sweeps - s0 < p->opt_xl_chunk ? num_sweeps - s0 : p->opt_xl_chunk;
                    DenseXlArgs b = a;
                    b.num_sweeps = len; b.temps = a.temps + s0; b.sweep_offset = a.sweep_offset + (uint32_t)s0;
                    unsigned long long before = 0, after = 0;
                    HIP_TRY(hipMemcpyAsync(&before, p->d_stats + 1, sizeof before, hipMemcpyDeviceToHost, p->stream));
                    rc = mi_launch_dense_xg(b, p->xl_chunks, p->d_xg, p->stream, (s0 == 0 ? 1 : 0) | 2);
                    if (rc) break;
                    s0 += len;
                    if (s0 >= num_sweeps) break;
                    HIP_TRY(hipMemcpyAsync(&after, p->d_stats + 1, sizeof after, hipMemcpyDeviceToHost, p->stream));
                    HIP_TRY(hipStreamSynchronize(p->stream));
                    const double share = (double)(after - before) / ((double)R * (double)p->n * (double)len);
                    if (share * 1000.0 < (double)p->opt_xl_cold_permille) {
                        DenseXlArgs c = a;
                        c.num_sweeps = num_sweeps - s0; c.temps = a.temps + s0; c.sweep_offset = a.sweep_offset + (uint32_t)s0;
                        c.init = (const uint8_t *)p->d_states;
                        c.fields_in = mi_dense_xg_fields(p->d_xg);
                        c.fin_ncols = (p->n + 255) / 256 * 256;
                        rc = mi_launch_dense_xl(c, p->xl_chunks, p->stream);
                        break;
                    }
                }
                if (rc) return rc;
                HIP_TRY(hipEventRecord(p->ev1, p->stream));
                return MI_OK;
            };
            if (p->opt_xl_async) {
                p->last_R = R; p->last_offset = replica_offset; p->has_run = true;
                p->worker = std::thread([p, cooling_run]() {
                    g_kernel.clear(); g_err.clear();
                    p->worker_rc = cooling_run();
                    p->worker_err = g_err;
                    p->worker_kernel = g_kernel;
                });
                return MI_OK;
            }
            rc = cooling_run();
            if (rc) return rc;
            p->last_R = R; p->last_offset = replica_offset; p->has_run = true;
            p->last_kernel = g_kernel;
            return MI_OK;
        }
        if (rc) return rc;
        HIP_TRY(hipEventRecord(p->ev1, p->stream));
    } else if (p->kind == MI_KIND_DENSE) {
        DenseArgs a;
        a.Qp = p->d_Qp; a.Qm = p->d_Qm; a.temps = temps_buf;
        a.init = cont ? (const uint8_t *)p->d_states : (init ? (const uint8_t *)p->d_init : nullptr);
        a.states = (uint8_t *)p->d_states; a.energy = p->d_energy; a.stats = p->d_stats; a.pace = nullptr;
        a.offset = p->offset; a.n = p->n; a.R = R; a.num_sweeps = num_sweeps; a.resync = resync_interval;
        a.replica_offset = replica_offset; a.seed_lo = (uint32_t)seed; a.seed_hi = (uint32_t)(seed >> 32);
        a.debug = p->opt_debug; a.ondemand_flips = 0; a.sweep_offset = sweep_offset; a.temps_per_replica = per_replica ? 1 : 0;
        HIP_TRY(hipEventRecord(p->ev0, p->stream));
        rc = dispatch_dense(p, a, p->stream);
        if (rc) return rc;
        HIP_TRY(hipEventRecord(p->ev1, p->stream));
    } else {
        EllArgs a;
        a.ell_col = p->d_ell_col; a.ell_val = p->d_ell_val; a.lin = p->d_lin; a.temps = temps_buf;
        a.init = cont ? p->d_states : (init ? p->d_init : nullptr); a.states = p->d_states; a.energy = p->d_energy; a.stats = p->d_stats;
        a.c_pair = p->c_pair; a.offset = p->offset; a.n = p->n; a.K = p->K; a.R = R; a.num_sweeps = num_sweeps;
        a.resync = resync_interval; a.slots = p->slots; a.D = p->D;
        a.replica_offset = replica_offset; a.seed_lo = (uint32_t)seed; a.seed_hi = (uint32_t)(seed >> 32);
        a.sweep_offset = sweep_offset; a.temps_per_replica = per_replica ? 1 : 0;
        a.rows = p->d_rows; a.meta = p->d_meta; a.adj4 = p->d_adj4; a.slot_flags = p->d_slot_flags; a.state_bytes = p->k2_state_bytes; a.waves_override = p->opt_k2_waves; a.min_size = p->opt_min_cluster_size;
        a.ell_val64 = p->d_ell_val64; a.lin64 = p->d_lin64; a.c_pair64 = p->c_pair64;
        a.wgt = p->d_wgt; a.wslot = p->kind == MI_KIND_CSR_RANK1 ? p->wslot : -1;
        a.adj4_trim = p->opt_k2_trim != 2 ? p->d_adj4r : nullptr; a.trim_rw = p->k2p_rw;
        a.nwq = p->d_nwq; a.ncw = p->d_ncw; a.nw64 = p->d_nw64;
        a.groups = G; a.temps_group_stride = per_group ? num_sweeps : 0; a.gconst = p->d_gconst;
        if (p->kind == MI_KIND_POTTS_CSR && init) {
            const uint16_t *l = static_cast<const uint16_t *>(init);
            for (size_t k = 0; k < (size_t)R * p->n; ++k)
                if (l[k] >= (uint16_t)p->K) return fail(MI_EINVAL, "initial label %u >= K = %d", (unsigned)l[k], p->K);
        }
        p->last_launches = 1;
        HIP_TRY(hipEventRecord(p->ev0, p->stream));
        if (p->kind == MI_KIND_POTTS_CSR) {
            const bool fast = p->d_adj4p && p->opt_k3_fast != 2 && mi_potts_fast_eligible(p->D, p->K, a.min_size);
            auto anneal_launch = [&](EllArgs &b) -> int {
                if (fast) {
                    b.adj4 = p->d_adj4p;
                    return mi_launch_potts_fast(b, p->opt_k2_tw != 2 && R <= 1024, p->stream);
                }
                return mi_launch_potts(b, p->stream);
            };
            if (!merges) {
                rc = anneal_launch(a);
            } else {
                MergeArgs m;
                m.ell_col = p->d_ell_col; m.ell_val = p->d_ell_val; m.meta = p->d_meta; m.nwq = p->d_nwq;
                m.cq = p->d_merge_cq; m.temps = temps_buf; m.temps_per_replica = per_replica ? 1 : 0;
                m.temps_group_stride = a.temps_group_stride; m.states = static_cast<uint16_t *>(p->d_states);
                m.stats = p->d_stats;
                const int f = merge_fixed_exponent(p->merge_sumabs);
                m.scale = std::ldexp(1.0, f); m.inv_scale = std::ldexp(1.0, -f);
                m.n = p->n; m.K = p->K; m.R = R; m.D = p->D; m.groups = G; m.proposals = p->merge_proposals;
                m.replica_offset = replica_offset; m.seed_lo = a.seed_lo; m.seed_hi = a.seed_hi;
                const uint32_t M = (uint32_t)p->merge_interval;
                const void *labels = a.init;
                int launches = 0, merge_launches = 0;
                for (int s0 = 0; !rc && s0 < num_sweeps;) {
                    const uint32_t s = sweep_offset + (uint32_t)s0;
                    if (s > 0 && s % M == 0) {
                        m.src = static_cast<const uint16_t *>(labels); m.sweep = s; m.sweep_local = s0;
                        rc = mi_launch_potts_merge(m, p->stream);
                        if (rc) break;
                        labels = p->d_states;
                        ++launches; ++merge_launches;
                    }
                    const int len = (int)std::min<uint32_t>((uint32_t)(num_sweeps - s0), M - s % M);
                    EllArgs b = a;
                    b.init = labels; b.num_sweeps = len; b.sweep_offset = s;
                    if (!per_replica) b.temps = a.temps + s0;
                    rc = anneal_launch(b);
                    labels = p->d_states;
                    ++launches;
                    s0 += len;
                }
                if (merge_launches) note_kernel("k_potts_merge");
                p->last_launches = launches;
            }
        } else {
            const bool split_ok = p->k2_free_block >= 64 && p->d_adj4p != nullptr, pair_ok = p->d_adj4p != nullptr;
            const bool tw = p->opt_k2_tw != 2;
            const long cus = p->cus > 0 ? p->cus : 256;
            auto one_round = [&](size_t lds_per_wg, long wgs) {
                return lds_per_wg * (size_t)((wgs + cus - 1) / cus) <= (size_t)160 * 1024;
            };
            const size_t cells = (size_t)p->slots * 256;
            const long pair_wgs = ((long)R + 1) / 2;
            const long tw_rounds = (pair_wgs + 8 * cus - 1) / (8 * cus);
            const bool tw_pair = tw && p->D == 16 &&
                                 ((pair_wgs <= 8 * cus && one_round(cells + 4096, pair_wgs)) ||
                                  (10 * pair_wgs >= 9 * tw_rounds * 8 * cus && (cells + 4096) * 8 <= (size_t)160 * 1024));
            const bool pair_run = pair_ok && (cells * 8 <= (size_t)150 * 1024 || one_round(cells + (tw_pair ? 4096 : 0), pair_wgs));
            int choice = 0;
            const bool weighted = p->wslot >= 0;
            if (weighted) {
                if (p->opt_k2_pair != 2 && pair_run && p->D == 16 && R > 1024) choice = 1;
                else if (p->opt_k2_split != 2 && tw && p->opt_k2_wide != 2 && split_ok &&
                         R <= p->opt_k2_split_max && one_round(cells + 2048, R)) choice = 2;
            } else
            if (p->opt_k2_split == 1 && split_ok) choice = 2;
            else if (p->opt_k2_pair == 1 && pair_ok) choice = 1;
            else if (p->opt_k2_split != 2 && split_ok && R <= p->opt_k2_split_max && one_round(cells + 2048, R)) choice = 2;
            else if (p->opt_k2_pair != 2 && pair_run && R > 1024) choice = 1;
            if (choice == 2 && weighted) {
                a.adj4 = p->d_adj4p;
                rc = mi_launch_csr_rank1_wide(a, 1, true, p->stream);
            } else if (choice == 2 && p->k2_free_block > 64 && p->opt_k2_wide != 2 && (p->D == 16 || p->k2_free_block == 128)) {
                a.adj4 = p->d_adj4p;
                rc = mi_launch_csr_rank1_wide(a, p->k2_free_block / 64, tw, p->stream);
            } else if (choice == 2 && p->k2_free_block == 64 && p->opt_k2_wide != 2 && tw) {
                a.adj4 = p->d_adj4p;
                rc = mi_launch_csr_rank1_wide(a, 1, true, p->stream);
            } else if (choice == 2) {
                a.adj4 = p->d_adj4p;
                rc = mi_launch_csr_rank1_split(a, p->k2_free_block / 64, p->stream);
            } else if (choice == 1) {
                a.adj4 = p->d_adj4p;
                rc = mi_launch_csr_rank1_pair(a, p->opt_k2_pair == 1 ? (tw && p->D == 16 && pair_wgs <= 8 * cus) : tw_pair, p->stream);
            } else {
                rc = mi_launch_csr_rank1(a, p->stream, tw && R <= 1024 && (p->D == 16 || p->D == 32) && p->k2_state_bytes <= 1);
            }
        }
        if (rc) return rc;
        HIP_TRY(hipEventRecord(p->ev1, p->stream));
    }
    p->last_R = R; p->last_offset = replica_offset; p->has_run = true;
    p->last_kernel = g_kernel;
    return MI_OK;
}

int mi_sa_tempering_begin(mi_sa_problem *p, const double *ladder_betas, int T, int chains,
                          uint32_t first_replica, int R_local)
{
    if (!p || !ladder_betas) return fail(MI_EINVAL, "NULL argument");
    if (const int rc_w = settle(p)) return rc_w;
    if (p->ngroups > 1) return fail(MI_EUNSUPPORTED, "tempering with resolution groups is not supported");
    if (p->merge_interval > 0) return fail(MI_EUNSUPPORTED, "tempering with merge moves is not supported");
    if (T < 2 || T > 1024) return fail(MI_EINVAL, "a tempering ladder has 2 .. 1024 temperatures (got %d)", T);
    if (chains < 1) return fail(MI_EINVAL, "chains must be >= 1");
    const long long total = (long long)T * chains;
    if (R_local < 1 || (long long)first_replica + R_local > total)
        return fail(MI_EINVAL, "local replicas [%u, %u + %d) do not lie inside the %lld replicas of the run", first_replica, first_replica, R_local, total);
    for (int k = 0; k < T; ++k)
        if (!(ladder_betas[k] > 0.0) || !std::isfinite(ladder_betas[k]))
            return fail(MI_EINVAL, "ladder beta %d = %g is not a positive finite number", k, ladder_betas[k]);
    HIP_TRY(hipSetDevice(p->device));
    HIP_TRY(hipStreamSynchronize(p->stream));
    int rc = ensure_run_buffers(p, R_local, R_local, false);
    if (rc) return rc;
    for (void *b : {(void *)p->d_pt_rung, (void *)p->d_pt_betas, (void *)p->d_pt_energy, (void *)p->d_pt_ladder, (void *)p->d_pt_temps, (void *)p->d_pt_stats})
        if (b) (void)hipFree(b);
    p->d_pt_rung = nullptr; p->d_pt_betas = nullptr; p->d_pt_energy = nullptr; p->d_pt_ladder = nullptr; p->d_pt_temps = nullptr; p->d_pt_stats = nullptr;
    p->pt_T = 0;
    rc = guarded([&]() -> int {
        std::vector<int> rung((size_t)total);
        for (long long g = 0; g < total; ++g) rung[(size_t)g] = (int)(g % T);
        std::vector<float> lt((size_t)T), local((size_t)R_local);
        for (int k = 0; k < T; ++k) lt[(size_t)k] = (float)(1.0 / ladder_betas[k]);
        for (int r = 0; r < R_local; ++r) local[(size_t)r] = lt[(size_t)(((long long)first_replica + r) % T)];
        HIP_TRY(hipMalloc((void **)&p->d_pt_rung, (size_t)total * sizeof(int)));
        HIP_TRY(hipMalloc((void **)&p->d_pt_betas, (size_t)T * sizeof(double)));
        HIP_TRY(hipMalloc((void **)&p->d_pt_energy, (size_t)total * sizeof(double)));
        HIP_TRY(hipMalloc((void **)&p->d_pt_ladder, (size_t)T * sizeof(float)));
        HIP_TRY(hipMalloc((void **)&p->d_pt_stats, 2 * sizeof(unsigned long long)));
        HIP_TRY(hipMalloc((void **)&p->d_pt_temps, (size_t)R_local * sizeof(float)));
        HIP_TRY(hipMemcpy(p->d_pt_rung, rung.data(), rung.size() * sizeof(int), hipMemcpyHostToDevice));
        HIP_TRY(hipMemcpy(p->d_pt_betas, ladder_betas, (size_t)T * sizeof(double), hipMemcpyHostToDevice));
        HIP_TRY(hipMemcpy(p->d_pt_ladder, lt.data(), lt.size() * sizeof(float), hipMemcpyHostToDevice));
        HIP_TRY(hipMemcpy(p->d_pt_temps, local.data(), local.size() * sizeof(float), hipMemcpyHostToDevice));
        HIP_TRY(hipMemset(p->d_pt_stats, 0, 2 * sizeof(unsigned long long)));
        return MI_OK;
    });
    if (rc) return rc;
    p->pt_T = T; p->pt_chains = chains; p->pt_lo = (int)first_replica; p->pt_R_local = R_local;
    return MI_OK;
}

static int tempering_exchange_impl(mi_sa_problem *p, uint32_t round, uint64_t seed, const double *all_energies, bool on_device)
{
    if (const int rc_w = settle(p)) return rc_w;
    if (!p) return fail(MI_EINVAL, "NULL problem");
    if (p->pt_T == 0) return fail(MI_ESTATE, "mi_sa_tempering_begin has not been called on this problem");
    if (!p->has_run || p->last_R != p->pt_R_local) return fail(MI_ESTATE, "no tempering round has run on this problem");
    const long long total = (long long)p->pt_T * p->pt_chains;
    if (!all_energies && p->pt_R_local != total)
        return fail(MI_EINVAL, "this GPU holds %d of the %lld replicas: the exchange needs all energies", p->pt_R_local, total);
    HIP_TRY(hipSetDevice(p->device));
    const double *en = p->d_energy;
    if (all_energies && on_device) {
        en = all_energies;
    } else if (all_energies) {
        HIP_TRY(hipMemcpyAsync(p->d_pt_energy, all_energies, (size_t)total * sizeof(double), hipMemcpyHostToDevice, p->stream));
        en = p->d_pt_energy;
    }
    hipLaunchKernelGGL(k_pt_exchange, dim3(p->pt_chains), dim3(256), (size_t)p->pt_T * sizeof(int), p->stream, en,
                       p->d_pt_rung, p->d_pt_betas, p->d_pt_ladder, p->d_pt_temps, p->pt_T, p->pt_lo, p->pt_lo + p->pt_R_local,
                       round, (uint32_t)seed, (uint32_t)(seed >> 32), p->d_pt_stats);
    HIP_TRY(hipGetLastError());
    if (all_energies) HIP_TRY(hipStreamSynchronize(p->stream));
    return MI_OK;
}

int mi_sa_tempering_exchange(mi_sa_problem *p, uint32_t round, uint64_t seed, const double *all_energies)
{
    return tempering_exchange_impl(p, round, seed, all_energies, false);
}

int mi_sa_tempering_exchange_dev(mi_sa_problem *p, uint32_t round, uint64_t seed, const double *d_all_energies)
{
    if (!d_all_energies) return fail(MI_EINVAL, "d_all_energies is NULL");
    return tempering_exchange_impl(p, round, seed, d_all_energies, true);
}

int mi_sa_device_results(mi_sa_problem *p, void **out_d_states, double **out_d_energy, int *out_R)
{
    if (!p) return fail(MI_EINVAL, "NULL problem");
    if (const int rc_w = settle(p)) return rc_w;
    if (!p->has_run) return fail(MI_ESTATE, "no anneal has been run on this problem");
    HIP_TRY(hipSetDevice(p->device));
    HIP_TRY(hipStreamSynchronize(p->stream));
    if (out_d_states) *out_d_states = p->d_states;
    if (out_d_energy) *out_d_energy = p->d_energy;
    if (out_R) *out_R = p->last_R;
    return MI_OK;
}

int mi_sa_tempering_state(mi_sa_problem *p, int32_t *out_rung, uint64_t *out_proposed, uint64_t *out_accepted)
{
    if (!p) return fail(MI_EINVAL, "NULL problem");
    if (const int rc_w = settle(p)) return rc_w;
    if (p->pt_T == 0) return fail(MI_ESTATE, "mi_sa_tempering_begin has not been called on this problem");
    HIP_TRY(hipSetDevice(p->device));
    HIP_TRY(hipStreamSynchronize(p->stream));
    if (out_rung)
        HIP_TRY(hipMemcpy(out_rung, p->d_pt_rung, (size_t)p->pt_T * p->pt_chains * sizeof(int), hipMemcpyDeviceToHost));
    unsigned long long st[2];
    HIP_TRY(hipMemcpy(st, p->d_pt_stats, sizeof st, hipMemcpyDeviceToHost));
    if (out_proposed) *out_proposed = st[0];
    if (out_accepted) *out_accepted = st[1];
    return MI_OK;
}

int mi_sa_anneal_ex(mi_sa_problem *p, int R, uint32_t replica_offset, int num_sweeps,
                    const double *betas, uint64_t seed, const void *init, int resync_interval,
                    uint32_t sweep_offset, uint32_t flags)
{
    return guarded([&]() -> int {
        return anneal_ex_impl(p, R, replica_offset, num_sweeps, betas, seed, init, resync_interval, sweep_offset, flags);
    });
}

int mi_sa_anneal(mi_sa_problem *p, int R, uint32_t replica_offset, int num_sweeps,
                 const double *betas, uint64_t seed, const void *init, int resync_interval)
{
    return mi_sa_anneal_ex(p, R, replica_offset, num_sweeps, betas, seed, init, resync_interval, 0u, 0u);
}

int mi_sa_sync(mi_sa_problem *p)
{
    if (!p) return fail(MI_EINVAL, "NULL problem");
    if (const int rc_w = settle(p)) return rc_w;
    HIP_TRY(hipSetDevice(p->device));
    HIP_TRY(hipStreamSynchronize(p->stream));
    return MI_OK;
}

int mi_sa_last_kernel_ms(mi_sa_problem *p, float *out_ms)
{
    if (!p || !out_ms) return fail(MI_EINVAL, "NULL argument");
    if (const int rc_w = settle(p)) return rc_w;
    if (!p->has_run) return fail(MI_ESTATE, "no anneal has been run on this problem");
    HIP_TRY(hipSetDevice(p->device));
    HIP_TRY(hipEventSynchronize(p->ev1));
    HIP_TRY(hipEventElapsedTime(out_ms, p->ev0, p->ev1));
    return MI_OK;
}

int mi_sa_last_launch_count(mi_sa_problem *p, int *out_launches)
{
    if (!p || !out_launches) return fail(MI_EINVAL, "NULL argument");
    if (const int rc_w = settle(p)) return rc_w;
    if (!p->has_run) return fail(MI_ESTATE, "no anneal has been run on this problem");
    *out_launches = p->last_launches;
    return MI_OK;
}

int mi_sa_last_kernel_name(mi_sa_problem *p, char *out, int len)
{
    if (!p || !out || len < 1) return fail(MI_EINVAL, "NULL argument");
    if (const int rc_w = settle(p)) return rc_w;
    if (!p->has_run) return fail(MI_ESTATE, "no anneal has been run on this problem");
    snprintf(out, (size_t)len, "%s", p->last_kernel.c_str());
    return MI_OK;
}

int mi_sa_fetch(mi_sa_problem *p, void *out_states, double *out_energy, uint64_t *out_stats)
{
    if (!p) return fail(MI_EINVAL, "NULL problem");
    if (const int rc_w = settle(p)) return rc_w;
    if (!p->has_run) return fail(MI_ESTATE, "no anneal has been run on this problem");
    HIP_TRY(hipSetDevice(p->device));
    HIP_TRY(hipStreamSynchronize(p->stream));
    if (out_states)
        HIP_TRY(hipMemcpy(out_states, p->d_states, (size_t)p->last_R * p->n * p->state_elem, hipMemcpyDeviceToHost));
    if (out_energy)
        HIP_TRY(hipMemcpy(out_energy, p->d_energy, (size_t)p->last_R * sizeof(double), hipMemcpyDeviceToHost));
    if (out_stats) {
        unsigned long long st[4];
        HIP_TRY(hipMemcpy(st, p->d_stats, sizeof st, hipMemcpyDeviceToHost));
        out_stats[0] = st[0]; out_stats[1] = st[1]; out_stats[2] = st[2];
    }
    return MI_OK;
}

int mi_sa_problem_label_agreement(mi_sa_problem *p, int groups, double *out_ari, double *out_nmi, int64_t *out_pair_sum,
                                  float *out_kernel_ms)
{
    if (!p) return fail(MI_EINVAL, "NULL problem");
    if (const int rc_w = settle(p)) return rc_w;
    if (p->kind != MI_KIND_POTTS_CSR) return fail(MI_ESTATE, "label agreement needs a Potts problem");
    if (!p->has_run) return fail(MI_ESTATE, "no anneal has been run on this problem");
    const int G = groups > 0 ? groups : p->ngroups;
    if (p->last_R % G != 0) return fail(MI_EINVAL, "R = %d is not a multiple of groups = %d", p->last_R, G);
    return guarded([&]() -> int {
        int n_real = 0;
        for (int i = 0; i < p->n; ++i) n_real += (p->h_meta[(size_t)i] >> 31) ? 0 : 1;
        if (n_real < 1) return fail(MI_EINVAL, "every variable of the problem is a hole");
        HIP_TRY(hipSetDevice(p->device));
        AgreeArgs a;
        a.A = static_cast<const uint16_t *>(p->d_states); a.lda = (size_t)p->n;
        a.Ra = p->last_R; a.cols = p->n; a.Ka = a.Kb = p->K; a.groups = G;
        a.meta = p->d_meta; a.n_real = n_real;
        return mi_label_agreement_dev(a, p->stream, out_ari, out_nmi, out_pair_sum, nullptr, out_kernel_ms);
    });
}

int mi_sa_problem_coassociation(mi_sa_problem *p, int groups, const uint16_t *ref, int Kref, const int32_t *eu,
                                const int32_t *ev, int64_t m, int64_t *out_hist, int64_t *out_rowsum, int32_t *out_edge,
                                int32_t *out_counts, float *out_kernel_ms)
{
    if (!p) return fail(MI_EINVAL, "NULL problem");
    if (const int rc_w = settle(p)) return rc_w;
    if (p->kind != MI_KIND_POTTS_CSR) return fail(MI_ESTATE, "co-association needs a Potts problem");
    if (!p->has_run) return fail(MI_ESTATE, "no anneal has been run on this problem");
    const int G = groups > 0 ? groups : p->ngroups;
    if (const int rc = mi_coassociation_check(p->last_R, p->n, p->K, G, ref, Kref, eu, ev, m, out_rowsum, out_edge)) return rc;
    return guarded([&]() -> int {
        HIP_TRY(hipSetDevice(p->device));
        CoassocArgs a;
        a.L = static_cast<const uint16_t *>(p->d_states); a.ld = (size_t)p->n;
        a.R = p->last_R; a.cols = p->n; a.K = p->K; a.groups = G; a.meta = p->d_meta;
        a.ref = ref; a.Kref = ref ? Kref : 1; a.eu = eu; a.ev = ev; a.m = out_edge ? m : 0;
        return mi_coassociation_dev(a, p->stream, out_hist, out_rowsum, out_edge, out_counts, out_kernel_ms);
    });
}

int mi_sa_problem_components(mi_sa_problem *p, int32_t *out_labels, int32_t *out_count, float *out_kernel_ms)
{
    if (!p) return fail(MI_EINVAL, "NULL problem");
    if (!out_labels || !out_count) return fail(MI_EINVAL, "NULL argument");
    if (const int rc_w = settle(p)) return rc_w;
    if (p->kind != MI_KIND_POTTS_CSR) return fail(MI_ESTATE, "components need a Potts problem");
    if (!p->has_run) return fail(MI_ESTATE, "no anneal has been run on this problem");
    return guarded([&]() -> int {
        HIP_TRY(hipSetDevice(p->device));
        ComponentsArgs a;
        a.rows = p->d_rows; a.meta = p->d_meta; a.D = p->D; a.n = p->n;
        a.L = static_cast<const uint16_t *>(p->d_states); a.ldl = (size_t)p->n;
        return mi_components_dev(a, p->last_R, false, p->stream, out_labels, out_count, out_kernel_ms);
    });
}

int mi_sa_best(mi_sa_problem *p, int *out_index, double *out_energy, uint64_t *out_key, void *out_state)
{
    if (!p) return fail(MI_EINVAL, "NULL problem");
    if (const int rc_w = settle(p)) return rc_w;
    if (p->ngroups > 1) return fail(MI_EUNSUPPORTED, "best of a run with resolution groups: one minimum across different objectives");
    if (!p->has_run) return fail(MI_ESTATE, "no anneal has been run on this problem");
    HIP_TRY(hipSetDevice(p->device));
    unsigned long long init_key = ~0ull, key = 0;
    HIP_TRY(hipMemcpyAsync(p->d_stats + 3, &init_key, sizeof init_key, hipMemcpyHostToDevice, p->stream));
    hipLaunchKernelGGL(k_best, dim3(1), dim3(1024), 0, p->stream, p->d_energy, p->last_R, p->last_offset, p->d_stats + 3);
    HIP_TRY(hipGetLastError());
    HIP_TRY(hipMemcpyAsync(&key, p->d_stats + 3, sizeof key, hipMemcpyDeviceToHost, p->stream));
    HIP_TRY(hipStreamSynchronize(p->stream));
    const int idx = (int)((uint32_t)(key & 0xffffffffull) - p->last_offset);
    if (idx < 0 || idx >= p->last_R) return fail(MI_EHIP, "best-of reduction returned an invalid index %d", idx);
    if (out_index) *out_index = idx;
    if (out_key) *out_key = key;
    if (out_energy) HIP_TRY(hipMemcpy(out_energy, p->d_energy + idx, sizeof(double), hipMemcpyDeviceToHost));
    if (out_state)
        HIP_TRY(hipMemcpy(out_state, (const char *)p->d_states + (size_t)idx * p->n * p->state_elem,
                          (size_t)p->n * p->state_elem, hipMemcpyDeviceToHost));
    return MI_OK;
}

static void shard_of(int R_total, int d, int ndev, int *lo, int *hi)
{
    const int base = R_total / ndev, rem = R_total % ndev;
    *lo = d * base + (d < rem ? d : rem);
    *hi = *lo + base + (d < rem ? 1 : 0);
}

static int multi_check(mi_sa_problem *const *problems, int ndev)
{
    if (!problems || ndev < 1) return fail(MI_EINVAL, "need ndev >= 1 problem handles");
    for (int d = 0; d < ndev; ++d) {
        if (!problems[d]) return fail(MI_EINVAL, "problem %d is NULL", d);
        if (problems[d]->ngroups > 1) return fail(MI_EUNSUPPORTED, "problem %d has resolution groups: not sharded over GPUs", d);
        if (problems[d]->kind != problems[0]->kind || problems[d]->n != problems[0]->n || problems[d]->K != problems[0]->K)
            return fail(MI_EINVAL, "problem %d is not the model of problem 0 (kind / size differ)", d);
    }
    return MI_OK;
}

int mi_multi_gpu_anneal(mi_sa_problem *const *problems, int ndev, int R_total, uint32_t replica_offset,
                        int num_sweeps, const double *betas, uint64_t seed, int resync_interval)
{
    int rc = multi_check(problems, ndev);
    if (rc) return rc;
    if (R_total < ndev) return fail(MI_EINVAL, "R_total = %d replicas cannot be sharded over %d devices", R_total, ndev);
    for (int d = 0; d < ndev; ++d) {
        int lo, hi;
        shard_of(R_total, d, ndev, &lo, &hi);
        rc = mi_sa_anneal_ex(problems[d], hi - lo, replica_offset + (uint32_t)lo, num_sweeps, betas, seed, nullptr,
                             resync_interval, 0u, 0u);
        if (rc) return rc;
    }
    return MI_OK;
}

int mi_multi_gpu_best(mi_sa_problem *const *problems, int ndev, int *out_owner, uint32_t *out_global_id,
                      double *out_energy, void *out_state)
{
    int rc = multi_check(problems, ndev);
    if (rc) return rc;
    int owner = -1, best_idx = 0;
    uint64_t best_key = ~0ull;
    double best_e = 0.0;
    for (int d = 0; d < ndev; ++d) {
        int idx = 0;
        uint64_t key = 0;
        double e = 0.0;
        rc = mi_sa_best(problems[d], &idx, &e, &key, nullptr);
        if (rc) return rc;
        if (owner < 0 || e < best_e) { owner = d; best_key = key; best_idx = idx; best_e = e; }
    }
    mi_sa_problem *p = problems[owner];
    HIP_TRY(hipSetDevice(p->device));
    if (out_owner) *out_owner = owner;
    if (out_global_id) *out_global_id = (uint32_t)(best_key & 0xffffffffull);
    if (out_energy) HIP_TRY(hipMemcpy(out_energy, p->d_energy + best_idx, sizeof(double), hipMemcpyDeviceToHost));
    if (out_state)
        HIP_TRY(hipMemcpy(out_state, (const char *)p->d_states + (size_t)best_idx * p->n * p->state_elem,
                          (size_t)p->n * p->state_elem, hipMemcpyDeviceToHost));
    return MI_OK;
}

int mi_multi_gpu_fetch(mi_sa_problem *const *problems, int ndev, void *out_states, double *out_energy, uint64_t *out_stats)
{
    int rc = multi_check(problems, ndev);
    if (rc) return rc;
    size_t done = 0;
    uint64_t tot[3] = {0, 0, 0};
    for (int d = 0; d < ndev; ++d) {
        mi_sa_problem *p = problems[d];
        if (!p->has_run) return fail(MI_ESTATE, "no anneal has been run on problem %d", d);
        uint64_t st[3] = {0, 0, 0};
        rc = mi_sa_fetch(p, out_states ? (char *)out_states + done * p->n * p->state_elem : nullptr,
                         out_energy ? out_energy + done : nullptr, st);
        if (rc) return rc;
        for (int k = 0; k < 3; ++k) tot[k] += st[k];
        done += (size_t)p->last_R;
    }
    if (out_stats) { out_stats[0] = tot[0]; out_stats[1] = tot[1]; out_stats[2] = tot[2]; }
    return MI_OK;
}

int mi_sa_qubo_dense_f32(const float *Qs, int n, double offset, int R, int num_sweeps,
                         const double *betas, uint64_t seed, const uint8_t *init,
                         uint8_t *out_states, double *out_energy, uint64_t *out_stats, int device)
{
    mi_sa_problem *p = nullptr;
    int rc = mi_sa_problem_create_dense_f32(Qs, n, offset, device, &p);
    if (rc) return rc;
    rc = mi_sa_anneal(p, R, 0, num_sweeps, betas, seed, init, 0);
    if (!rc) rc = mi_sa_fetch(p, out_states, out_energy, out_stats);
    if (!rc && out_stats) out_stats[0] = (uint64_t)R * (uint64_t)num_sweeps * (uint64_t)n;
    mi_sa_problem_destroy(p);
    return rc;
}

int mi_energy_dense_f32_ex(const float *Qs, int n, const uint8_t *X, int R, double offset,
                           double *out_energy, int device, int path, float *out_kernel_ms)
{
    if (!Qs || !X || !out_energy) return fail(MI_EINVAL, "NULL argument");
    if (n < 1 || R < 1) return fail(MI_EINVAL, "n and R must be >= 1");
    if (path < 0 || path > 2) return fail(MI_EINVAL, "path must be 0 (auto), 1 (VALU) or 2 (MFMA)");
    if (path != 1 && (path == 2 || R >= 32)) {
        bool symmetric = true;
        for (int i = 0; i < n && symmetric; ++i)
            for (int j = i + 1; j < n; ++j)
                if (Qs[(size_t)i * n + j] != Qs[(size_t)j * n + i]) { symmetric = false; break; }
        if (!symmetric) {
            if (path == 2) return fail(MI_EINVAL, "the MFMA energy path (path = 2) needs a symmetric Qs; use (Q + Q^T) / 2 or path 0 / 1");
            path = 1;
        }
    }
    if (path == 0) path = (R >= 32) ? 2 : 1;
    int rc = select_device(device);
    if (rc) return rc;
    float *dQ = nullptr; uint8_t *dX = nullptr, *dXt = nullptr; double *dE = nullptr;
    hipEvent_t e0 = nullptr, e1 = nullptr;
    rc = [&]() -> int {
        const size_t ldq = path == 2 ? ((size_t)n + 127) / 128 * 128 : (size_t)n;
        const size_t rows = path == 2 ? ldq : (size_t)n;
        HIP_TRY(hipMalloc((void **)&dQ, rows * ldq * sizeof(float)));
        HIP_TRY(hipMalloc((void **)&dX, (size_t)R * n));
        HIP_TRY(hipMalloc((void **)&dE, (size_t)R * sizeof(double)));
        if (path == 2) {
            HIP_TRY(hipMalloc((void **)&dXt, mi_energy_dense_scratch_bytes(n, R)));
            HIP_TRY(hipMemset(dQ, 0, rows * ldq * sizeof(float)));
        }
        HIP_TRY(hipMemcpy2D(dQ, ldq * sizeof(float), Qs, (size_t)n * sizeof(float), (size_t)n * sizeof(float), (size_t)n,
                            hipMemcpyHostToDevice));
        HIP_TRY(hipMemcpy(dX, X, (size_t)R * n, hipMemcpyHostToDevice));
        HIP_TRY(hipEventCreate(&e0));
        HIP_TRY(hipEventCreate(&e1));
        HIP_TRY(hipEventRecord(e0, 0));
        int r2 = mi_launch_energy_dense(dQ, n, (int)ldq, dX, R, offset, dE, dXt, path, 0);
        if (r2) return r2;
        HIP_TRY(hipEventRecord(e1, 0));
        HIP_TRY(hipEventSynchronize(e1));
        if (out_kernel_ms) HIP_TRY(hipEventElapsedTime(out_kernel_ms, e0, e1));
        HIP_TRY(hipMemcpy(out_energy, dE, (size_t)R * sizeof(double), hipMemcpyDeviceToHost));
        return MI_OK;
    }();
    if (e0) (void)hipEventDestroy(e0);
    if (e1) (void)hipEventDestroy(e1);
    if (dQ) (void)hipFree(dQ);
    if (dX) (void)hipFree(dX);
    if (dXt) (void)hipFree(dXt);
    if (dE) (void)hipFree(dE);
    return rc;
}

int mi_energy_dense_f64(const double *Qs, int n, const uint8_t *X, int R, double offset,
                        double *out_energy, int device)
{
    if (!Qs || !X || !out_energy) return fail(MI_EINVAL, "NULL argument");
    if (n < 1 || R < 1) return fail(MI_EINVAL, "n and R must be >= 1");
    int rc = select_device(device);
    if (rc) return rc;
    double *dQ = nullptr, *dE = nullptr; uint8_t *dX = nullptr;
    rc = [&]() -> int {
        HIP_TRY(hipMalloc((void **)&dQ, (size_t)n * n * sizeof(double)));
        HIP_TRY(hipMalloc((void **)&dX, (size_t)R * n));
        HIP_TRY(hipMalloc((void **)&dE, (size_t)R * sizeof(double)));
        HIP_TRY(hipMemcpy(dQ, Qs, (size_t)n * n * sizeof(double), hipMemcpyHostToDevice));
        HIP_TRY(hipMemcpy(dX, X, (size_t)R * n, hipMemcpyHostToDevice));
        int r2 = mi_launch_energy_dense_f64(dQ, n, dX, R, offset, dE, 0);
        if (r2) return r2;
        HIP_TRY(hipMemcpy(out_energy, dE, (size_t)R * sizeof(double), hipMemcpyDeviceToHost));
        return MI_OK;
    }();
    if (dQ) (void)hipFree(dQ);
    if (dX) (void)hipFree(dX);
    if (dE) (void)hipFree(dE);
    return rc;
}

int mi_energy_dense_f32(const float *Qs, int n, const uint8_t *X, int R, double offset,
                        double *out_energy, int device)
{
    return mi_energy_dense_f32_ex(Qs, n, X, R, offset, out_energy, device, 0, nullptr);
}

}
```

### scrna_seq_qannealing_clustering_amd/csrc/mi_sa_device.h

```cpp
#pragma once

#include <hip/hip_runtime.h>

#include <cmath>
#include <cstdint>
#include <exception>
#include <new>
#include <type_traits>

#include "../../include/mi_sa.h"

namespace mi_sa_impl {

int fail(int code, const char *fmt, ...);
void note_kernel(const char *fmt, ...);

template <typename F>
int guarded(F &&body) noexcept
{
    try {
        return body();
    } catch (const std::bad_alloc &) {
        return fail(MI_ENOMEM, "out of host memory");
    } catch (const std::exception &e) {
        return fail(MI_EINVAL, "unexpected C++ exception: %s", e.what());
    } catch (...) {
        return fail(MI_EINVAL, "unexpected C++ exception");
    }
}

#define HIP_TRY(expr)                                                                            \
    do {                                                                                         \
        hipError_t e_ = (expr);                                                                  \
        if (e_ != hipSuccess)                                                                    \
            return ::mi_sa_impl::fail(MI_EHIP, "%s failed: %s (%s:%d)", #expr, hipGetErrorString(e_),  \
                                      __FILE__, __LINE__);                                       \
    } while (0)

constexpr uint32_t PH_M0 = 0xD2511F53u, PH_M1 = 0xCD9E8D57u;
constexpr uint32_t PH_W0 = 0x9E3779B9u, PH_W1 = 0xBB67AE85u;

__device__ __forceinline__ void philox4x32_10(uint32_t c0, uint32_t c1, uint32_t c2, uint32_t c3,
                                              uint32_t k0, uint32_t k1, uint32_t (&out)[4])
{
#pragma unroll
    for (int r = 0; r < 10; ++r) {
        const uint64_t p0 = (uint64_t)PH_M0 * c0, p1 = (uint64_t)PH_M1 * c2;
        const uint32_t hi0 = (uint32_t)(p0 >> 32), lo0 = (uint32_t)p0;
        const uint32_t hi1 = (uint32_t)(p1 >> 32), lo1 = (uint32_t)p1;
        const uint32_t n0 = hi1 ^ c1 ^ k0, n2 = hi0 ^ c3 ^ k1;
        c0 = n0; c1 = lo1; c2 = n2; c3 = lo0;
        k0 += PH_W0; k1 += PH_W1;
    }
    out[0] = c0; out[1] = c1; out[2] = c2; out[3] = c3;
}

__device__ __forceinline__ float neglog_u(uint32_t r)
{
    const float mm = __uint_as_float(0x3f800000u | (r >> 9));
    const float u = 2.0f - mm;
    const uint32_t ub = __float_as_uint(u);
    const int neg_e = 127 - (int)((ub + 0x004afb0cu) >> 23);
    const float m = __uint_as_float(ub + ((uint32_t)neg_e << 23));
    const float t = m - 1.0f;
    float p = -0x1.9f9af6p-4f;
    p = __fmaf_rn(p, t, 0x1.4cd8dcp-3f);
    p = __fmaf_rn(p, t, -0x1.61491cp-3f);
    p = __fmaf_rn(p, t, 0x1.977bcp-3f);
    p = __fmaf_rn(p, t, -0x1.ff611p-3f);
    p = __fmaf_rn(p, t, 0x1.555a22p-2f);
    p = __fmaf_rn(p, t, -0x1.00007cp-1f);
    p = __fmaf_rn(p, t, 0x1.fffffep-1f);
    const float lnm = p * t;
    return __fmaf_rn((float)neg_e, 0x1.62e43p-1f, -lnm);
}

typedef float f32x2_t __attribute__((ext_vector_type(2)));
__device__ __forceinline__ f32x2_t neglog_u2(uint32_t ra, uint32_t rb)
{
    const f32x2_t mm = {__uint_as_float(__builtin_amdgcn_alignbit(0x7fu, ra, 9)),
                        __uint_as_float(__builtin_amdgcn_alignbit(0x7fu, rb, 9))};
    const f32x2_t u = f32x2_t{2.0f, 2.0f} - mm;
    const uint32_t ta = (__float_as_uint(u.x) + 0x004afb0cu) & 0x7f800000u;
    const uint32_t tb = (__float_as_uint(u.y) + 0x004afb0cu) & 0x7f800000u;
    const f32x2_t scale = {__uint_as_float(0x7f000000u - ta), __uint_as_float(0x7f000000u - tb)};
    const f32x2_t m = u * scale;
    const f32x2_t ef = {(float)(int)ta, (float)(int)tb};
    const f32x2_t neg_e = __builtin_elementwise_fma(ef, f32x2_t{-0x1p-23f, -0x1p-23f}, f32x2_t{127.0f, 127.0f});
    const f32x2_t t = m - f32x2_t{1.0f, 1.0f};
    f32x2_t p = {-0x1.9f9af6p-4f, -0x1.9f9af6p-4f};
    p = __builtin_elementwise_fma(p, t, f32x2_t{0x1.4cd8dcp-3f, 0x1.4cd8dcp-3f});
    p = __builtin_elementwise_fma(p, t, f32x2_t{-0x1.61491cp-3f, -0x1.61491cp-3f});
    p = __builtin_elementwise_fma(p, t, f32x2_t{0x1.977bcp-3f, 0x1.977bcp-3f});
    p = __builtin_elementwise_fma(p, t, f32x2_t{-0x1.ff611p-3f, -0x1.ff611p-3f});
    p = __builtin_elementwise_fma(p, t, f32x2_t{0x1.555a22p-2f, 0x1.555a22p-2f});
    p = __builtin_elementwise_fma(p, t, f32x2_t{-0x1.00007cp-1f, -0x1.00007cp-1f});
    p = __builtin_elementwise_fma(p, t, f32x2_t{0x1.fffffep-1f, 0x1.fffffep-1f});
    const f32x2_t lnm = p * t;
    return __builtin_elementwise_fma(neg_e, f32x2_t{0x1.62e43p-1f, 0x1.62e43p-1f}, -lnm);
}

__device__ __forceinline__ float readlane_f(float v, int l)
{
    return __int_as_float(__builtin_amdgcn_readlane(__float_as_int(v), l));
}


template <int I, int N, typename F>
__device__ __forceinline__ void static_for(F &&body)
{
    if constexpr (I < N) {
        body(std::integral_constant<int, I>{});
        static_for<I + 1, N>(body);
    }
}

__device__ __forceinline__ double wave_sum_f64(double v)
{
#pragma unroll
    for (int off = 32; off > 0; off >>= 1) v += __shfl_xor(v, off, 64);
    return v;
}

constexpr int kPaceWords = 32 * 9;
constexpr long long kPaceStartTicks = 400000;
constexpr long long kPaceSweepTicks = 200000;

__device__ __forceinline__ unsigned int pace_load(const unsigned int *p)
{
    return (unsigned int)__builtin_amdgcn_readfirstlane(
        (int)__hip_atomic_load(p, __ATOMIC_RELAXED, __HIP_MEMORY_SCOPE_AGENT));
}

__device__ __forceinline__ long long pace_clock()
{
    return (long long)__builtin_amdgcn_s_memrealtime();
}

__device__ __forceinline__ unsigned int sweep_pace_begin(unsigned int *pace, unsigned int total_waves,
                                                         unsigned int &xcc)
{
    if (!pace) return 0;
    xcc = (unsigned int)__builtin_amdgcn_readfirstlane(
              (int)__builtin_amdgcn_s_getreg(20 | (0 << 6) | (3 << 11))) & 7u;
    if ((threadIdx.x & 63) == 0) {
        atomicAdd(&pace[32 * (1 + xcc)], 1u);
        __builtin_amdgcn_fence(__ATOMIC_RELEASE, "agent");
        atomicAdd(&pace[0], 1u);
    }
    const long long t0 = pace_clock();
    bool ok = true;
    while (pace_load(&pace[0]) < total_waves) {
        if (pace_load(&pace[1]) != 0 || pace_clock() - t0 > kPaceStartTicks) { ok = false; break; }
        __builtin_amdgcn_s_sleep(32);
    }
    if (!ok) {
        if ((threadIdx.x & 63) == 0)
            __hip_atomic_store(&pace[1], 1u, __ATOMIC_RELAXED, __HIP_MEMORY_SCOPE_AGENT);
        return 0;
    }
    return pace_load(&pace[32 * (1 + xcc)]);
}

__device__ __forceinline__ void sweep_pace_arrive_wait(unsigned int *pace, unsigned int xcc,
                                                       unsigned int pop, unsigned int sweeps_done,
                                                       bool wait = true)
{
    unsigned int *arr = &pace[32 * (1 + xcc) + 1];
    if ((threadIdx.x & 63) == 0) atomicAdd(arr, 1u);
    if (!wait) return;
    const unsigned int target = pop * sweeps_done;
    const long long t0 = pace_clock();
    while (pace_load(arr) < target) {
        if (pace_clock() - t0 > kPaceSweepTicks) {
            if ((threadIdx.x & 63) == 0) atomicAdd(&pace[2], 1u);
            break;
        }
        __builtin_amdgcn_s_sleep(64);
    }
}

struct DenseArgs {
    const float *Qp;
    const float *Qm;
    const float *temps;
    const uint8_t *init;
    uint8_t *states;
    double *energy;
    unsigned long long *stats;
    unsigned int *pace;
    double offset;
    int n, R, num_sweeps, resync;
    uint32_t replica_offset, seed_lo, seed_hi;
    uint32_t sweep_offset;
    int temps_per_replica;
    float *fields;
    unsigned int *ctrl;
    int flags;
    int resync_first;
    int my_mode;
    int chunk_index;
    unsigned int mode_up_flips;
    int ondemand_flips;
    int debug;
};

constexpr int kDenseFieldsIn = 1;
constexpr int kDenseFieldsOut = 2;
constexpr int kDenseNoEnergy = 4;

typedef float f32x4 __attribute__((ext_vector_type(4)));
typedef unsigned int u32x4 __attribute__((ext_vector_type(4)));
typedef unsigned int u32x2 __attribute__((ext_vector_type(2)));


typedef float f32x2 __attribute__((ext_vector_type(2)));

struct EllArgs {
    const uint32_t *ell_col;
    const float *ell_val;
    const float *lin;
    const float *temps;
    const void *init;
    void *states;
    double *energy;
    unsigned long long *stats;
    float c_pair;
    double offset;
    int n, K, R, num_sweeps, resync, slots, D;
    uint32_t replica_offset, seed_lo, seed_hi;
    uint32_t sweep_offset;
    int temps_per_replica;
    const uint2 *rows;
    const uint32_t *meta;
    const uint4 *adj4;
    int state_bytes;
    const uint32_t *slot_flags;
    int waves_override;
    int min_size;
    const double *ell_val64;
    const double *lin64;
    double c_pair64;
    const int32_t *wgt = nullptr;
    int wslot = -1;
    int ring_off = 0;
    const uint4 *adj4_trim = nullptr;
    int trim_rw = 0;
    const int32_t *nwq = nullptr;
    const float *ncw = nullptr;
    const double *nw64 = nullptr;
    int groups = 1;
    int temps_group_stride = 0;
    const double *gconst = nullptr;
};

struct ReplicaGroup { int g; int rank; };
__device__ __forceinline__ ReplicaGroup replica_group(const EllArgs &a, int r)
{
    if (a.groups <= 1) return {0, r};
    const int rg = a.R / a.groups;
    const int g = r / rg;
    return {g, r - g * rg};
}

template <typename LabelF>
__device__ double node_weight_energy(const EllArgs &a, int lane, int grp, LabelF label)
{
    double own = 0.0, tot = 0.0;
    for (int t = 0; t < a.slots; ++t) {
        const double w = a.nw64[t * 64 + lane];
        own -= w * w;
    }
    for (int q = 0; q < a.K; ++q) {
        double s = 0.0;
        for (int t = 0; t < a.slots; ++t) {
            const int i = t * 64 + lane;
            if (label(i) == (uint32_t)q) s += a.nw64[i];
        }
        s = wave_sum_f64(s);
        tot += s * s;
    }
    const double c64 = a.gconst ? a.gconst[grp] : (a.ell_val64 ? a.c_pair64 : (double)a.c_pair);
    return 0.5 * c64 * (own + (lane == 0 ? tot : 0.0));
}

__device__ __forceinline__ uint64_t weighted_slot_sweep(float g, float thr, int w, float c_pair, uint32_t z, int &A, int lane)
{
    const float cw = c_pair * (float)w;
    uint64_t todo = __ballot(w != 0), flipped = 0ull;
    uint32_t zz = z;
    while (todo != 0ull) {
        const int l = __ffsll((unsigned long long)todo) - 1;
        todo &= todo - 1ull;
        const float f = g + cw * (float)(A - w * (int)zz);
        const float dE = zz ? -f : f;
        if ((__ballot(dE < thr) >> l) & 1ull) {
            const int wl = __builtin_amdgcn_readlane(w, l);
            const int zl = __builtin_amdgcn_readlane((int)zz, l);
            A += zl ? -wl : wl;
            if (lane == l) zz ^= 1u;
            flipped |= 1ull << l;
        }
    }
    return flipped;
}

__device__ __forceinline__ long long wave_sum_i64(long long v)
{
#pragma unroll
    for (int off = 32; off > 0; off >>= 1) v += __shfl_xor(v, off, 64);
    return v;
}
int mi_launch_csr_rank1(const EllArgs &, hipStream_t, bool tw = false);
int mi_launch_csr_rank1_pair(const EllArgs &, bool tw, hipStream_t);
int mi_launch_csr_rank1_split(const EllArgs &, int nw, hipStream_t);
int mi_launch_csr_rank1_wide(const EllArgs &, int spb, bool tw, hipStream_t);
int mi_launch_potts(const EllArgs &, hipStream_t);
bool mi_potts_fast_eligible(int D, int K, int min_size);
int mi_launch_potts_fast(const EllArgs &, bool tw, hipStream_t);
struct MergeArgs {
    const uint32_t *ell_col;
    const float *ell_val;
    const uint32_t *meta;
    const int32_t *nwq;
    const double *cq;
    const float *temps;
    int temps_per_replica, temps_group_stride, sweep_local;
    const uint16_t *src;
    uint16_t *states;
    unsigned long long *stats;
    double scale, inv_scale;
    int n, K, R, D, groups, proposals;
    uint32_t sweep, replica_offset, seed_lo, seed_hi;
};
size_t mi_potts_merge_lds_bytes(int K);
int mi_launch_potts_merge(const MergeArgs &, hipStream_t);

struct DenseXlArgs {
    const float *Q2;
    const float *diag;
    const float *temps;
    const uint8_t *init;
    uint8_t *states;
    double *energy;
    unsigned long long *stats;
    double offset;
    int n, R, num_sweeps, resync;
    uint32_t replica_offset, seed_lo, seed_hi, sweep_offset;
    int temps_per_replica;
    const float *fields_in = nullptr;
    int fin_ncols = 0;
    int xg_chain = 0;
};
int mi_launch_dense_xl(const DenseXlArgs &, int chunks, hipStream_t);
size_t mi_dense_xg_workspace_bytes(int n, int R);
int mi_launch_dense_xg(const DenseXlArgs &, int chunks, void *workspace, hipStream_t, int phase);
const float *mi_dense_xg_fields(void *workspace);

__device__ __forceinline__ uint32_t chain_word_dev(uint32_t i, uint32_t s, uint32_t g, uint32_t tag, uint32_t k0, uint32_t k1)
{
    uint32_t w[4];
    philox4x32_10(((i >> 8) << 6) | (i & 63u), s, g, tag, k0, k1, w);
    const uint32_t sel = (i >> 6) & 3u;
    return sel == 0 ? w[0] : (sel == 1 ? w[1] : (sel == 2 ? w[2] : w[3]));
}

size_t mi_energy_dense_scratch_bytes(int n, int R);
int mi_launch_energy_dense(const float *dQ, int n, int ldq, const uint8_t *dX, int R, double offset, double *dE,
                           uint8_t *dXt, int path, hipStream_t st);
int mi_launch_energy_dense_f64(const double *dQ, int n, const uint8_t *dX, int R, double offset, double *dE, hipStream_t st);

struct AgreeArgs {
    const uint16_t *A = nullptr, *B = nullptr;
    size_t lda = 0, ldb = 0;
    int Ra = 0, Rb = 0, cols = 0, Ka = 0, Kb = 0, groups = 1;
    const uint32_t *meta = nullptr;
    int n_real = 0;
};
int mi_label_agreement_dev(const AgreeArgs &a, hipStream_t st, double *out_ari, double *out_nmi, int64_t *out_pair_sum,
                           int32_t *out_tables, float *out_kernel_ms);

struct CoassocArgs {
    const uint16_t *L = nullptr;
    size_t ld = 0;
    int R = 0, cols = 0, K = 0, groups = 1;
    const uint32_t *meta = nullptr;
    const uint16_t *ref = nullptr;
    int Kref = 1;
    const int32_t *eu = nullptr, *ev = nullptr;
    int64_t m = 0;
};
int mi_coassociation_check(int R, int n, int K, int groups, const uint16_t *ref, int Kref, const int32_t *eu, const int32_t *ev,
                           int64_t m, const int64_t *out_rowsum, const int32_t *out_edge);
int mi_coassociation_dev(const CoassocArgs &a, hipStream_t st, int64_t *out_hist, int64_t *out_rowsum, int32_t *out_edge,
                         int32_t *out_counts, float *out_kernel_ms);

struct ComponentsArgs {
    const int32_t *rowptr = nullptr, *col = nullptr;
    const uint2 *rows = nullptr;
    const uint32_t *meta = nullptr;
    int D = 0, n = 0;
    long long nnz = 0;
    const uint16_t *L = nullptr;
    size_t ldl = 0;
    const uint8_t *keep = nullptr;
};
int mi_components_dev(const ComponentsArgs &a, int B, bool force_global, hipStream_t st, int32_t *out_labels,
                      int32_t *out_count, float *out_kernel_ms);

template <int NT>
__device__ __forceinline__ double dense_energy_f64(__amdgpu_buffer_rsrc_t rsrc, int diag_row, uint64_t xb,
                                                   int lane)
{
    constexpr int G = NT / 4;
    const int voff = lane * 16;
    double pair = 0.0, lin = 0.0;
#pragma unroll 1
    for (int t = -1; t < NT; ++t) {
        uint64_t m = (t < 0) ? 1ull : __ballot((xb >> t) & 1ull);
        while (m) {
            const int l = __ffsll((unsigned long long)m) - 1;
            m &= m - 1;
            const int soff = ((t < 0) ? diag_row : t * 64 + l) * (NT * 256);
            double acc = 0.0;
#pragma unroll
            for (int g = 0; g < G; ++g) {
                const u32x4 q = __builtin_amdgcn_raw_buffer_load_b128(rsrc, voff, soff + g * 1024, 0);
                acc += ((xb >> (4 * g + 0)) & 1ull) ? (double)__uint_as_float(q.x) : 0.0;
                acc += ((xb >> (4 * g + 1)) & 1ull) ? (double)__uint_as_float(q.y) : 0.0;
                acc += ((xb >> (4 * g + 2)) & 1ull) ? (double)__uint_as_float(q.z) : 0.0;
                acc += ((xb >> (4 * g + 3)) & 1ull) ? (double)__uint_as_float(q.w) : 0.0;
            }
            if (t < 0) lin = acc; else pair += acc;
        }
    }
    return wave_sum_f64(lin + 0.5 * pair);
}

constexpr unsigned int kModeWg = 0, kModeMfma = 1;
constexpr int kCtrlModes = 8, kCtrlWords = 4096;

__device__ __forceinline__ bool sched_my_turn(const DenseArgs &a)
{
    if (!a.ctrl) return true;
    return (unsigned int)__builtin_amdgcn_readfirstlane(
               (int)__hip_atomic_load(a.ctrl + kCtrlModes + a.chunk_index, __ATOMIC_RELAXED,
                                      __HIP_MEMORY_SCOPE_AGENT)) == (unsigned int)a.my_mode;
}

__device__ __forceinline__ void sched_finish(const DenseArgs &a, unsigned int wg_flips)
{
    if (!a.ctrl) return;
    atomicAdd(&a.ctrl[2], wg_flips);
    __threadfence();
    const unsigned int ticket = atomicAdd(&a.ctrl[1], 1u);
    if (ticket == gridDim.x - 1) {
        __threadfence();
        const unsigned int total = __hip_atomic_load(&a.ctrl[2], __ATOMIC_RELAXED, __HIP_MEMORY_SCOPE_AGENT);
        const unsigned int next = (a.mode_up_flips != 0 && total >= a.mode_up_flips) ? kModeMfma : kModeWg;
        __hip_atomic_store(&a.ctrl[kCtrlModes + a.chunk_index + 1], next, __ATOMIC_RELAXED, __HIP_MEMORY_SCOPE_AGENT);
        __hip_atomic_store(&a.ctrl[1], 0u, __ATOMIC_RELAXED, __HIP_MEMORY_SCOPE_AGENT);
        __hip_atomic_store(&a.ctrl[2], 0u, __ATOMIC_RELAXED, __HIP_MEMORY_SCOPE_AGENT);
        atomicAdd(&a.ctrl[4 + a.my_mode], 1u);
    }
}

#define MI_DECLARE_MFMA(N) int mi_launch_dense_mfma_nt##N(const DenseArgs &, hipStream_t);
MI_DECLARE_MFMA(4) MI_DECLARE_MFMA(8) MI_DECLARE_MFMA(12) MI_DECLARE_MFMA(16) MI_DECLARE_MFMA(20)
MI_DECLARE_MFMA(24) MI_DECLARE_MFMA(28) MI_DECLARE_MFMA(32) MI_DECLARE_MFMA(36) MI_DECLARE_MFMA(40)
MI_DECLARE_MFMA(44)
#undef MI_DECLARE_MFMA
constexpr int kMaxMfmaNT = 44;

struct DenseLaunchCtx {
    int device;
    int opt_pace, opt_variant, opt_unit_rows, opt_ondemand_permille, opt_chunk_sweeps, opt_mfma_permille;
    float *d_fields;
    unsigned int *d_ctrl;
    unsigned int *d_pace;
    int *resident_waves;
    int *launches;
};

constexpr int kMaxChunks = 64;

#define MI_DECLARE_DENSE(N) int mi_launch_dense_nt##N(const DenseLaunchCtx &, const DenseArgs &, hipStream_t);
MI_DECLARE_DENSE(4) MI_DECLARE_DENSE(8) MI_DECLARE_DENSE(12) MI_DECLARE_DENSE(16) MI_DECLARE_DENSE(20)
MI_DECLARE_DENSE(24) MI_DECLARE_DENSE(28) MI_DECLARE_DENSE(32) MI_DECLARE_DENSE(36) MI_DECLARE_DENSE(40)
MI_DECLARE_DENSE(44) MI_DECLARE_DENSE(48) MI_DECLARE_DENSE(52) MI_DECLARE_DENSE(56) MI_DECLARE_DENSE(60)
MI_DECLARE_DENSE(64)
#undef MI_DECLARE_DENSE

}
```

### scrna_seq_qannealing_clustering_amd/csrc/sparse_pair_kernels.hip

```cpp
#include "mi_sa_device.h"

namespace mi_sa_impl {

namespace {

typedef _Float16 half_t;

#ifdef MI_K2P_PROFILE
#define K2P_TICK(var) do { asm volatile("s_waitcnt lgkmcnt(0)" ::: "memory"); const unsigned long long now_ = __builtin_amdgcn_s_memtime(); var += now_ - tick_; tick_ = now_; } while (0)
#else
#define K2P_TICK(var) do { } while (0)
#endif

__device__ __forceinline__ float half_lo(uint32_t w) { return (float)__builtin_bit_cast(half_t, (uint16_t)w); }
__device__ __forceinline__ float half_hi(uint32_t w) { return (float)__builtin_bit_cast(half_t, (uint16_t)(w >> 16)); }

template <int D, bool TW, bool WGT = false, int RW = D>
__global__ void __launch_bounds__(TW ? 128 : 64, TW ? 1 : 2) k_anneal_csr_rank1_pair(EllArgs a)
{
    static_assert(RW > D - 4 && RW <= D, "trimmed rows drop part of the last group of four only");
    extern __shared__ __attribute__((aligned(16))) char lds[];
    const int lane = threadIdx.x & 63;
    const int pair = blockIdx.x;
    const int rA = 2 * pair, rB = 2 * pair + 1;
    if (rA >= a.R) return;
    const bool liveB = rB < a.R;
    const uint32_t gidA = a.replica_offset + (uint32_t)rA, gidB = gidA + 1u;
    const int n = a.n, slots = a.slots;
    const uint8_t *init = static_cast<const uint8_t *>(a.init);
    uint32_t *cell = reinterpret_cast<uint32_t *>(lds);
    const uint32_t ring_lane = (uint32_t)slots * 256u + (uint32_t)lane * 8u;

    if constexpr (TW) {
        if (__builtin_amdgcn_readfirstlane((int)(threadIdx.x >> 6)) == 1) {
            uint32_t wa[4], wb[4];
            uint32_t buf = 0;
            for (int s = 0; s < a.num_sweeps; ++s) {
                float TA, TB;
                if (a.temps_per_replica) {
                    TA = __int_as_float(__builtin_amdgcn_readfirstlane(__float_as_int(a.temps[rA])));
                    TB = __int_as_float(__builtin_amdgcn_readfirstlane(__float_as_int(a.temps[liveB ? rB : rA])));
                } else {
                    TA = TB = __int_as_float(__builtin_amdgcn_readfirstlane(__float_as_int(a.temps[s])));
                }
                const uint32_t sw = (uint32_t)s + a.sweep_offset;
#pragma unroll 1
                for (int t = 0; t < slots; t += 4) {
#ifdef MI_K2P_DBG_NOPROD
                    for (int c = 0; c < 4; ++c) wa[c] = wb[c] = (uint32_t)(t + c) * 0x9E3779B9u + lane * 77u;
#else
                    philox4x32_10((uint32_t)((t >> 2) * 64 + lane), sw, gidA, 0u, a.seed_lo, a.seed_hi, wa);
                    philox4x32_10((uint32_t)((t >> 2) * 64 + lane), sw, gidB, 0u, a.seed_lo, a.seed_hi, wb);
#endif
                    const uint32_t at = ring_lane + buf;
#pragma unroll
                    for (int c = 0; c < 4; ++c) {
                        const f32x2_t thr = neglog_u2(wa[c], wb[c]) * f32x2_t{TA, TB};
                        asm volatile("ds_write_b64 %0, %1 offset:%2" :: "v"(at), "v"(thr), "n"(c * 512) : "memory");
                    }
                    buf ^= 2048u;
                    asm volatile("s_waitcnt lgkmcnt(0)" ::: "memory");
                    __builtin_amdgcn_s_barrier();
                }
            }
            return;
        }
    }

    const int wslot = WGT ? a.wslot : -1;
    const int wl = wslot >= 0 ? a.wgt[lane] : 0;
    int SA = 0, SB = 0;
    for (int tg = 0; tg * 4 < slots; ++tg) {
        uint32_t wa[4] = {0u, 0u, 0u, 0u}, wb[4] = {0u, 0u, 0u, 0u};
        if (!init) {
            philox4x32_10((uint32_t)(tg * 64 + lane), 0u, gidA, 1u, a.seed_lo, a.seed_hi, wa);
            philox4x32_10((uint32_t)(tg * 64 + lane), 0u, gidB, 1u, a.seed_lo, a.seed_hi, wb);
        }
#pragma unroll
        for (int c = 0; c < 4; ++c) {
            const int t = 4 * tg + c;
            if (t >= slots) break;
            const int i = t * 64 + lane;
            bool xa, xb;
            const bool real = i < n && a.lin[i] < INFINITY;
            if (init) {
                xa = real && init[(size_t)rA * n + i] != 0;
                xb = real && liveB && init[(size_t)rB * n + i] != 0;
            } else {
                xa = real && (wa[c] >> 31);
                xb = real && (wb[c] >> 31);
            }
            cell[i] = (xa ? 0x3c00u : 0u) | (xb ? 0x3c000000u : 0u);
            if (WGT && t == wslot) {
                SA += (int)wave_sum_i64(xa ? (long long)wl : 0ll);
                SB += (int)wave_sum_i64(xb ? (long long)wl : 0ll);
            } else {
                SA += __popcll(__ballot(xa));
                SB += __popcll(__ballot(xb));
            }
        }
    }

    constexpr int G = D / 4;
    constexpr int LW = RW - 4 * (G - 1);
    constexpr int SLOT_BYTES = (G - 1) * 2048 + (LW == 3 ? 1792 : LW * 512);
    const __amdgpu_buffer_rsrc_t rs_adj = __builtin_amdgcn_make_buffer_rsrc(
        const_cast<uint4 *>(a.adj4), 0, slots * SLOT_BYTES, 0x00020000);
    const __amdgpu_buffer_rsrc_t rs_lin = __builtin_amdgcn_make_buffer_rsrc(
        const_cast<float *>(a.lin), 0, slots * 256, 0x00020000);
    struct SlotAdj { u32x4 col[G]; u32x4 val[G]; uint32_t lin; };
    const int lane16 = lane * 16;
#ifdef MI_K2P_NOFETCH
    auto fetch_real = [&](int t) {
#else
    auto fetch_adj = [&](int t) {
#endif
        SlotAdj p;
        const int tt = t < slots ? t : slots - 1;
        const int soff = tt * SLOT_BYTES;
#pragma unroll
        for (int g = 0; g < G; ++g) {
            const int so = soff + (g / 2) * 4096, io = (g & 1) * 2048;
            if (LW == 4 || g < G - 1) {
                p.col[g] = __builtin_amdgcn_raw_buffer_load_b128(rs_adj, lane16 + io, so, 0);
                p.val[g] = __builtin_amdgcn_raw_buffer_load_b128(rs_adj, lane16 + io + 1024, so, 0);
            } else if constexpr (LW == 3) {
                p.col[g] = __builtin_amdgcn_raw_buffer_load_b128(rs_adj, lane16 + io, so, 0);
                const u32x2 v = __builtin_amdgcn_raw_buffer_load_b64(rs_adj, lane * 8 + io + 1024, so, 0);
                p.val[g] = u32x4{v.x, v.y, __builtin_amdgcn_raw_buffer_load_b32(rs_adj, lane * 4 + io + 1536, so, 0), 0u};
            } else if constexpr (LW == 2) {
                const u32x2 c = __builtin_amdgcn_raw_buffer_load_b64(rs_adj, lane * 8 + io, so, 0);
                const u32x2 v = __builtin_amdgcn_raw_buffer_load_b64(rs_adj, lane * 8 + io + 512, so, 0);
                p.col[g] = __builtin_shufflevector(c, c, 0, 1, -1, -1);
                p.val[g] = __builtin_shufflevector(v, v, 0, 1, -1, -1);
            } else {
                p.col[g][0] = __builtin_amdgcn_raw_buffer_load_b32(rs_adj, lane * 4 + io, so, 0);
                p.val[g][0] = __builtin_amdgcn_raw_buffer_load_b32(rs_adj, lane * 4 + io + 256, so, 0);
            }
        }
        if constexpr (LW == 3) p.lin = p.col[G - 1][3];
        else p.lin = __builtin_amdgcn_raw_buffer_load_b32(rs_lin, lane * 4, tt * 256, 0);
        return p;
    };
#ifdef MI_K2P_NOFETCH
    const SlotAdj adj0 = fetch_real(0);
    auto fetch_adj = [&](int) { return adj0; };
#endif

#ifdef MI_K2P_PROFILE
    unsigned long long tick_ = __builtin_amdgcn_s_memtime(), t_top = 0, t_gather = 0, t_sum = 0, t_rounds = 0, t_barrier = 0;
#endif
#ifndef MI_K2P_DBG_NOPRIO
    if constexpr (TW) __builtin_amdgcn_s_setprio(3);
#endif
    unsigned long long accepted = 0;
    uint32_t accA = 0, accB = 0;
    uint32_t wa[4] = {0u, 0u, 0u, 0u}, wb[4] = {0u, 0u, 0u, 0u};
    float TA = 1.0f, TB = 1.0f;
    const float cp = a.c_pair;
    uint32_t ring_buf = 0u;

    auto slot_body = [&](auto c_in_group, int t, const SlotAdj &cur, uint32_t wordA, uint32_t wordB) {
        constexpr int C = decltype(c_in_group)::value;
        const int i = t * 64 + lane;
        uint32_t own;
        float gA = __uint_as_float(cur.lin), gB = gA;
        float thrA = 0.0f, thrB = 0.0f;
        f32x2_t thr2 = {0.0f, 0.0f};
        uint32_t xiA = 0u, xiB = 0u, sgA = 0u, sgB = 0u;
        uint64_t XA = 0ull, XB = 0ull;
        f32x2_t cs = {0.0f, 0.0f}, csf = {0.0f, 0.0f};
        int ownA = 0, ownB = 0;
        auto own_terms = [&]() {
            xiA = (own >> 13) & 1u;
            xiB = own >> 29;
            XA = __ballot((own & 0xffffu) != 0u);
            XB = __ballot((own >> 16) != 0u);
            sgA = xiA << 31;
            sgB = xiB << 31;
            cs = f32x2_t{__uint_as_float(__float_as_uint(cp) ^ sgA), __uint_as_float(__float_as_uint(cp) ^ sgB)};
            ownA = SA - (int)xiA;
            ownB = SB - (int)xiB;
            csf = cs * f32x2_t{(float)ownA, (float)ownB};
        };
        K2P_TICK(t_top);
#pragma unroll
        for (int g0 = 0; g0 < G; g0 += 4) {
            constexpr int NK0 = RW < 16 ? RW : 16;
            const int NK = g0 == 0 ? NK0 : (RW - 4 * g0 < 16 ? RW - 4 * g0 : 16);
            uint32_t word[16];
            if (g0 == 0) asm volatile("ds_read_b32 %0, %1" : "=v"(own) : "v"(i * 4));
            if (g0 == 0 && TW) asm volatile("ds_read_b64 %0, %1 offset:%2" : "=v"(thr2) : "v"(ring_lane + ring_buf), "n"(C * 512));
#pragma unroll
            for (int k = 0; k < 16; ++k)
                if (k < NK)
#ifdef MI_K2P_DBG_LINEAR
                asm volatile("ds_read_b32 %0, %1" : "=v"(word[k]) : "v"((cur.col[g0 + k / 4][k & 3] & 0x3f00u) + lane * 4));
#else
                asm volatile("ds_read_b32 %0, %1" : "=v"(word[k]) : "v"(cur.col[g0 + k / 4][k & 3]));
#endif
            if (g0 == 0 && TW) {
                asm volatile("s_waitcnt lgkmcnt(%2)" : "+v"(own), "+v"(thr2) : "n"(NK0 < 15 ? NK0 : 15) : "memory");
#ifndef MI_K2P_DBG_TERMS_AFTER
                own_terms();
#endif
                asm volatile("s_waitcnt lgkmcnt(0)"
                             : "+v"(word[0]), "+v"(word[1]), "+v"(word[2]), "+v"(word[3]), "+v"(word[4]), "+v"(word[5]),
                               "+v"(word[6]), "+v"(word[7]), "+v"(word[8]), "+v"(word[9]), "+v"(word[10]), "+v"(word[11]),
                               "+v"(word[12]), "+v"(word[13]), "+v"(word[14]), "+v"(word[15]), "+v"(csf)
                             :: "memory");
                thrA = thr2.x;
                thrB = thr2.y;
            } else if (g0 == 0) {
                asm volatile("" : "+v"(wordA), "+v"(wordB));
                const f32x2_t thr = neglog_u2(wordA, wordB) * f32x2_t{TA, TB};
                thrA = thr.x;
                thrB = thr.y;
                asm volatile("s_waitcnt lgkmcnt(0)"
                             : "+v"(word[0]), "+v"(word[1]), "+v"(word[2]), "+v"(word[3]), "+v"(word[4]), "+v"(word[5]),
                               "+v"(word[6]), "+v"(word[7]), "+v"(word[8]), "+v"(word[9]), "+v"(word[10]), "+v"(word[11]),
                               "+v"(word[12]), "+v"(word[13]), "+v"(word[14]), "+v"(word[15]), "+v"(own), "+v"(thrA), "+v"(thrB)
                             :: "memory");
            } else {
                asm volatile("s_waitcnt lgkmcnt(0)"
                             : "+v"(word[0]), "+v"(word[1]), "+v"(word[2]), "+v"(word[3]), "+v"(word[4]), "+v"(word[5]),
                               "+v"(word[6]), "+v"(word[7]), "+v"(word[8]), "+v"(word[9]), "+v"(word[10]), "+v"(word[11]),
                               "+v"(word[12]), "+v"(word[13]), "+v"(word[14]), "+v"(word[15])
                             :: "memory");
            }
            K2P_TICK(t_gather);
#pragma unroll
            for (int k = 0; k < NK; ++k) {
                const float v = __uint_as_float(cur.val[g0 + k / 4][k & 3]);
                gA = __builtin_fmaf(v, half_lo(word[k]), gA);
                gB = __builtin_fmaf(v, half_hi(word[k]), gB);
            }
        }
#ifdef MI_K2P_DBG_TERMS_AFTER
        own_terms();
#else
        if constexpr (!TW) own_terms();
#endif
        if (WGT && t == wslot) {
            const uint64_t FA = weighted_slot_sweep(gA, thrA, wl, cp, xiA, SA, lane);
            const uint64_t FB = weighted_slot_sweep(gB, thrB, wl, cp, xiB, SB, lane);
            accA += (uint32_t)__popcll(FA);
            accB += (uint32_t)__popcll(FB);
            uint32_t fA, fB;
            asm("v_cndmask_b32 %0, 0, %1, %2" : "=v"(fA) : "v"(0x3c00u), "s"(FA));
            asm("v_cndmask_b32 %0, 0, %1, %2" : "=v"(fB) : "v"(0x3c000000u), "s"(FB));
            cell[i] = own ^ fA ^ fB;
            K2P_TICK(t_rounds);
            return;
        }
        const f32x2_t gs = {__uint_as_float(__float_as_uint(gA) ^ sgA), __uint_as_float(__float_as_uint(gB) ^ sgB)};
        f32x2_t de = gs + csf;
        bool mA = de.x < thrA, mB = de.y < thrB;
        uint64_t AA = __ballot(mA), AB = __ballot(mB);
        K2P_TICK(t_sum);
        if ((AA | AB) != 0ull) {
            const int baseA = ownA - (int)__builtin_amdgcn_mbcnt_hi((uint32_t)(XA >> 32), __builtin_amdgcn_mbcnt_lo((uint32_t)XA, 0u));
            const int baseB = ownB - (int)__builtin_amdgcn_mbcnt_hi((uint32_t)(XB >> 32), __builtin_amdgcn_mbcnt_lo((uint32_t)XB, 0u));
            uint64_t BA = AA ^ XA, BB = AB ^ XB;
#ifndef MI_K2P_DBG_NOROUNDS
#pragma nounroll
            for (;;) {
                const int sA = (int)__builtin_amdgcn_mbcnt_hi((uint32_t)(BA >> 32), __builtin_amdgcn_mbcnt_lo((uint32_t)BA, (uint32_t)baseA));
                const int sB = (int)__builtin_amdgcn_mbcnt_hi((uint32_t)(BB >> 32), __builtin_amdgcn_mbcnt_lo((uint32_t)BB, (uint32_t)baseB));
                de = gs + cs * f32x2_t{(float)sA, (float)sB};
                const uint64_t NBA = __ballot(de.x < thrA) ^ XA, NBB = __ballot(de.y < thrB) ^ XB;
                uint64_t d0 = NBA ^ BA, d1 = NBB ^ BB;
                asm("" : "+s"(d0), "+s"(d1));
                BA = NBA;
                BB = NBB;
                if ((d0 | d1) == 0ull) break;
            }
#endif
            AA = BA ^ XA;
            AB = BB ^ XB;
            SA += __popcll(BA) - __popcll(XA);
            SB += __popcll(BB) - __popcll(XB);
            accA += (uint32_t)__popcll(AA);
            accB += (uint32_t)__popcll(AB);
            uint32_t tA, tB;
            asm("v_cndmask_b32 %0, 0, %1, %2" : "=v"(tA) : "v"(0x3c00u), "s"(AA));
            asm("v_cndmask_b32 %0, 0, %1, %2" : "=v"(tB) : "v"(0x3c000000u), "s"(AB));
            cell[i] = own ^ tA ^ tB;
        }
        K2P_TICK(t_rounds);
    };

    using std::integral_constant;
    for (int s = 0; s < a.num_sweeps; ++s) {
        if constexpr (!TW) {
            if (a.temps_per_replica) {
                TA = __int_as_float(__builtin_amdgcn_readfirstlane(__float_as_int(a.temps[rA])));
                TB = __int_as_float(__builtin_amdgcn_readfirstlane(__float_as_int(a.temps[liveB ? rB : rA])));
            } else {
                TA = TB = __int_as_float(__builtin_amdgcn_readfirstlane(__float_as_int(a.temps[s])));
            }
        }
        const uint32_t sw = (uint32_t)s + a.sweep_offset;
        SlotAdj P = fetch_adj(0), Q;
#pragma unroll 1
        for (int t = 0; t < slots; t += 4) {
            if constexpr (TW) {
                K2P_TICK(t_top);
                __builtin_amdgcn_s_barrier();
                K2P_TICK(t_barrier);
            } else {
                philox4x32_10((uint32_t)((t >> 2) * 64 + lane), sw, gidA, 0u, a.seed_lo, a.seed_hi, wa);
                philox4x32_10((uint32_t)((t >> 2) * 64 + lane), sw, gidB, 0u, a.seed_lo, a.seed_hi, wb);
            }
            Q = fetch_adj(t + 1);
            slot_body(integral_constant<int, 0>{}, t, P, wa[0], wb[0]);
            if (t + 1 < slots) {
                P = fetch_adj(t + 2);
                slot_body(integral_constant<int, 1>{}, t + 1, Q, wa[1], wb[1]);
                if (t + 2 < slots) {
                    Q = fetch_adj(t + 3);
                    slot_body(integral_constant<int, 2>{}, t + 2, P, wa[2], wb[2]);
                    P = fetch_adj(t + 4);
                    if (t + 3 < slots) slot_body(integral_constant<int, 3>{}, t + 3, Q, wa[3], wb[3]);
                }
            }
            if constexpr (TW) ring_buf ^= 2048u;
        }
        accepted += (unsigned long long)accA + (liveB ? (unsigned long long)accB : 0ull);
        accA = accB = 0;
    }

#pragma unroll 1
    for (int rep = 0; rep < 2; ++rep) {
        if (rep == 1 && !liveB) break;
        const int r = rep ? rB : rA;
        const int sh = rep ? 16 : 0;
        uint8_t *dst = static_cast<uint8_t *>(a.states) + (size_t)r * n;
        long long cnt = 0, cnt2 = 0;
        double e = 0.0;
        for (int t = 0; t < slots; ++t) {
            const int i = t * 64 + lane;
            const bool on = ((cell[i] >> sh) & 0xffffu) != 0u;
            if (i < n) dst[i] = (uint8_t)on;
            if (WGT && t == wslot) {
                cnt += wave_sum_i64(on ? (long long)wl : 0ll);
                cnt2 += wave_sum_i64(on ? (long long)wl * wl : 0ll);
            } else {
                const int c1 = __popcll(__ballot(on));
                cnt += c1;
                cnt2 += c1;
            }
            if (!on) continue;
            double acc = 0.0;
            for (int k = 0; k < D; ++k) {
                const size_t at = ((size_t)t * D + k) * 64 + lane;
                const uint32_t cc = a.ell_col[at];
                const double vv = a.ell_val64 ? a.ell_val64[at] : (double)a.ell_val[at];
                if (((cell[cc] >> sh) & 0xffffu) != 0u) acc += vv;
            }
            e += (a.lin64 ? a.lin64[i] : (double)a.lin[i]) + 0.5 * acc;
        }
        e = wave_sum_f64(e);
        if (lane == 0) {
            const double cp64 = a.ell_val64 ? a.c_pair64 : (double)a.c_pair;
            a.energy[r] = e + cp64 * 0.5 * ((double)cnt * (double)cnt - (double)cnt2) + a.offset;
        }
    }
    if (lane == 0) atomicAdd(&a.stats[1], accepted);
#ifdef MI_K2P_PROFILE
    if (lane == 0) {
        atomicAdd(&a.stats[8], t_top); atomicAdd(&a.stats[9], t_gather); atomicAdd(&a.stats[10], t_sum);
        atomicAdd(&a.stats[11], t_rounds); atomicAdd(&a.stats[12], t_barrier);
    }
#endif
}

template <typename KernelT>
int launch_pair(KernelT kernel, const EllArgs &a, bool tw, hipStream_t st, int rw = 0)
{
    const size_t lds = (size_t)a.slots * 256 + (tw ? 4096 : 0);
    if (lds > 160 * 1024) return fail(MI_EUNSUPPORTED, "csr_rank1 pair kernel: n = %d exceeds the state LDS budget", a.n);
    if (lds > 64 * 1024)
        HIP_TRY(hipFuncSetAttribute(reinterpret_cast<const void *>(kernel), hipFuncAttributeMaxDynamicSharedMemorySize, (int)lds));
    if (rw) note_kernel("k_anneal_csr_rank1_pair<%d, tw> r%d", a.D, rw);
    else note_kernel(tw ? "k_anneal_csr_rank1_pair<%d, tw>" : "k_anneal_csr_rank1_pair<%d>", a.D);
    hipLaunchKernelGGL(kernel, dim3((a.R + 1) / 2), dim3(tw ? 128 : 64), lds, st, a);
    HIP_TRY(hipGetLastError());
    return MI_OK;
}

}

int mi_launch_csr_rank1_pair(const EllArgs &a, bool tw, hipStream_t st)
{
    if (!a.adj4) return fail(MI_EHIP, "csr_rank1 pair kernel: packed adjacency missing");
    if (tw && ((size_t)a.slots * 256 + 4096) * 8 > 160 * 1024 && a.R > 2 * 7 * 256) tw = false;
    if (a.wslot >= 0) {
        if (a.D != 16) return fail(MI_EUNSUPPORTED, "csr_rank1 pair kernel: pair-term weights at slot-ELL width %d not built", a.D);
        return tw ? launch_pair(k_anneal_csr_rank1_pair<16, true, true>, a, true, st)
                  : launch_pair(k_anneal_csr_rank1_pair<16, false, true>, a, false, st);
    }
    if (a.D == 16 && tw && a.adj4_trim) {
        EllArgs b = a;
        b.adj4 = a.adj4_trim;
        if (a.trim_rw == 15) return launch_pair(k_anneal_csr_rank1_pair<16, true, false, 15>, b, true, st, 15);
        if (a.trim_rw == 14) return launch_pair(k_anneal_csr_rank1_pair<16, true, false, 14>, b, true, st, 14);
        if (a.trim_rw == 13) return launch_pair(k_anneal_csr_rank1_pair<16, true, false, 13>, b, true, st, 13);
    }
    if (a.D == 16 && tw) return launch_pair(k_anneal_csr_rank1_pair<16, true>, a, true, st);
    if (a.D == 16) return launch_pair(k_anneal_csr_rank1_pair<16, false>, a, false, st);
    if (a.D == 32) return launch_pair(k_anneal_csr_rank1_pair<32, false>, a, false, st);
    return fail(MI_EUNSUPPORTED, "csr_rank1 pair kernel: slot-ELL width %d not built", a.D);
}

}
```

### scrna_seq_qannealing_clustering_amd/engine.py

```python
from __future__ import annotations

import ctypes as C
from typing import Optional

import numpy as np

from . import _lib


_POTTS_MAX_N = 40000


def layout_block_for(n: int, num_reads: int, max_degree: int = 16):
    if num_reads > 1024 or max_degree > 32 or n > 16384 or n < 1024:
        return 64
    return "auto"


_WIDE_STEP_RATIO = 439.0 / 236.0


def _ptr(a, ctype):
    return a.ctypes.data_as(C.POINTER(ctype)) if a is not None else None


class Problem:

    def __init__(self, handle, kind, n, num_cases, device, perm=None, seats=None, n_dev=None):
        self._h = handle
        self.kind = kind
        self.n = n
        self.num_cases = num_cases
        self.device = device
        self._last = None
        self.perm = perm
        self._inv = None if perm is None else np.argsort(perm)
        if seats is not None:
            self._inv = np.asarray(seats, dtype=np.int64)
        self.n_dev = int(n if n_dev is None else n_dev)
        self.groups = 1

    @classmethod
    def dense(cls, Qs: np.ndarray, offset: float = 0.0, device: int = 0) -> "Problem":
        Qs = np.ascontiguousarray(Qs, dtype=np.float32)
        if Qs.ndim != 2 or Qs.shape[0] != Qs.shape[1]:
            raise ValueError("Qs must be a square matrix")
        if not np.array_equal(Qs, Qs.T):
            raise ValueError("Qs must be symmetric (use (Q + Q.T)/2 with the diagonal kept)")
        lib = _lib.load()
        h = C.c_void_p()
        _lib.check(lib.mi_sa_problem_create_dense_f32(_ptr(Qs, C.c_float), Qs.shape[0],
                                                      float(offset), int(device), C.byref(h)))
        return cls(h, _lib.KIND_DENSE, Qs.shape[0], 2, device)

    @classmethod
    def csr_rank1(cls, rowptr, col, val, lin, c_pair: float, offset: float = 0.0,
                  device: int = 0, order: Optional[str] = None, energy_model=None, block=64, weights=None) -> "Problem":
        if weights is not None:
            weights = np.asarray(weights, dtype=np.int64)
            if np.all(weights == 1):
                weights = None
        if weights is not None:
            return cls._csr_rank1_weighted(rowptr, col, val, lin, c_pair, offset, device, order, energy_model, weights)
        perm = None
        val64 = lin64 = None
        if energy_model is not None:
            val64, lin64 = np.asarray(energy_model[0], dtype=np.float64), np.asarray(energy_model[1], dtype=np.float64)
        if order == "slots":
            from .models import permute_csr, slot_independent_order
            perm = slot_independent_order(rowptr, col)
            if val64 is not None:
                rowptr, col, val, val64 = permute_csr(rowptr, col, val, perm, also=val64)
                lin64 = lin64[perm]
            else:
                rowptr, col, val = permute_csr(rowptr, col, val, perm)
            lin = np.asarray(lin)[perm]
        elif order == "padded":
            from .models import pad_csr, padded_slot_layout
            if block == "auto":
                s64 = padded_slot_layout(rowptr, col, slot=64)
                s128 = padded_slot_layout(rowptr, col, slot=128)
                wide = s128[2] == 0 and s64[2] == 0 and (s128[1] + (s128[1] & 1)) * _WIDE_STEP_RATIO < s64[1]
                block = 128 if wide else 64
                seats, nslots, clashes = s128 if wide else s64
            elif block in (64, 128, 256):
                seats, nslots, clashes = padded_slot_layout(rowptr, col, slot=block)
            else:
                raise ValueError("block must be 64, 128, 256 or 'auto'")
            if block > 64 and clashes:
                return cls.csr_rank1(rowptr, col, val, lin, c_pair, offset, device, "padded", energy_model)
            if int(np.diff(np.asarray(rowptr)).max(initial=0)) > 64 and nslots * block * 5 > ((len(lin) + 63) // 64) * 64 * 6:
                return cls.csr_rank1(rowptr, col, val, lin, c_pair, offset, device, "slots", energy_model)
            if block == 128 and nslots % 2:
                nslots += 1
            n_caller, n_dev = len(lin), nslots * block
            if n_dev > (1 << 20) >= n_caller:
                return cls.csr_rank1(rowptr, col, val, lin, c_pair, offset, device, "slots", energy_model)
            if val64 is not None:
                rowptr, col, val, val64 = pad_csr(rowptr, col, val, seats, n_dev, also=val64)
                l64 = np.zeros(n_dev, dtype=np.float64)
                l64[seats] = lin64
                lin64 = l64
            else:
                rowptr, col, val = pad_csr(rowptr, col, val, seats, n_dev)
            lpad = np.full(n_dev, np.inf, dtype=np.float32)
            lpad[seats] = np.asarray(lin, dtype=np.float32)
            lin = lpad
        elif order is not None:
            raise ValueError("order must be None, 'slots' or 'padded'")
        rowptr = np.ascontiguousarray(rowptr, dtype=np.int32)
        col = np.ascontiguousarray(col, dtype=np.int32)
        val = np.ascontiguousarray(val, dtype=np.float32)
        lin = np.ascontiguousarray(lin, dtype=np.float32)
        n = len(lin)
        lib = _lib.load()
        h = C.c_void_p()
        _lib.check(lib.mi_sa_problem_create_csr_rank1_f32(
            _ptr(rowptr, C.c_int32), _ptr(col, C.c_int32), _ptr(val, C.c_float),
            _ptr(lin, C.c_float), float(c_pair), n, float(offset), int(device), C.byref(h)))
        if order == "padded":
            prob = cls(h, _lib.KIND_CSR_RANK1, n_caller, 2, device, seats=seats, n_dev=n_dev)
        else:
            prob = cls(h, _lib.KIND_CSR_RANK1, n, 2, device, perm=perm)
        if val64 is not None:
            prob._set_energy_model(val64, lin64, float(energy_model[2]), len(val))
        return prob

    @classmethod
    def _csr_rank1_weighted(cls, rowptr, col, val, lin, c_pair, offset, device, order, energy_model, weights) -> "Problem":
        from .models import pad_csr, padded_slot_layout
        if order != "padded":
            raise ValueError("a model with pair-term weights needs order='padded'")
        rowptr = np.asarray(rowptr, dtype=np.int64)
        col = np.asarray(col, dtype=np.int64)
        n_caller = len(lin)
        deg = np.diff(rowptr)
        heavy = np.flatnonzero(weights != 1)
        light = np.flatnonzero(weights == 1)
        if np.any(weights < 1) or len(heavy) > 64 or np.any(deg[heavy] != 0):
            raise ValueError("pair-term weights: positive integers; at most 64 variables with a weight other than 1, "
                             "and those without sparse couplings")
        renum = np.full(n_caller, -1, dtype=np.int64)
        renum[light] = np.arange(len(light))
        rp_l = np.concatenate([[0], np.cumsum(deg[light])]).astype(np.int32)
        keep = np.repeat(weights == 1, deg)
        seats_l, nslots, _ = padded_slot_layout(rp_l, renum[col[keep]].astype(np.int32), slot=64)
        seats = np.empty(n_caller, dtype=np.int64)
        seats[light] = seats_l
        seats[heavy] = nslots * 64 + np.arange(len(heavy))
        n_dev = (nslots + 1) * 64
        val64 = lin64 = None
        if energy_model is not None:
            val64, lin64 = np.asarray(energy_model[0], dtype=np.float64), np.asarray(energy_model[1], dtype=np.float64)
            rp, cc, vv, val64 = pad_csr(rowptr, col, val, seats, n_dev, also=val64)
            l64 = np.zeros(n_dev, dtype=np.float64)
            l64[seats] = lin64
            lin64 = l64
        else:
            rp, cc, vv = pad_csr(rowptr, col, val, seats, n_dev)
        lpad = np.full(n_dev, np.inf, dtype=np.float32)
        lpad[seats] = np.asarray(lin, dtype=np.float32)
        rp = np.ascontiguousarray(rp, dtype=np.int32)
        cc = np.ascontiguousarray(cc, dtype=np.int32)
        vv = np.ascontiguousarray(vv, dtype=np.float32)
        lib = _lib.load()
        h = C.c_void_p()
        _lib.check(lib.mi_sa_problem_create_csr_rank1_f32(
            _ptr(rp, C.c_int32), _ptr(cc, C.c_int32), _ptr(vv, C.c_float),
            _ptr(lpad, C.c_float), float(c_pair), n_dev, float(offset), int(device), C.byref(h)))
        prob = cls(h, _lib.KIND_CSR_RANK1, n_caller, 2, device, seats=seats, n_dev=n_dev)
        wdev = np.ones(n_dev, dtype=np.int32)
        wdev[seats] = weights
        rc = lib.mi_sa_problem_set_pair_weights(h, _ptr(wdev, C.c_int32))
        if rc:
            prob.close()
            _lib.check(rc)
        if val64 is not None:
            prob._set_energy_model(val64, lin64, float(energy_model[2]), len(vv))
        return prob

    @classmethod
    def potts_csr(cls, rowptr, col, val, c_pair: float, n: int, num_cases: int,
                  lin_offset: float = 0.0, device: int = 0, order: Optional[str] = None,
                  energy_model=None, node_weights=None) -> "Problem":
        perm = None
        val64 = None if energy_model is None else np.asarray(energy_model[0], dtype=np.float64)
        if order == "slots":
            from .models import permute_csr, slot_independent_order
            perm = slot_independent_order(rowptr, col)
            if val64 is not None:
                rowptr, col, val, val64 = permute_csr(rowptr, col, val, perm, also=val64)
            else:
                rowptr, col, val = permute_csr(rowptr, col, val, perm)
        elif order == "padded":
            from .models import pad_csr, padded_slot_layout
            seats, nslots, _ = padded_slot_layout(rowptr, col)
            if nslots * 64 > _POTTS_MAX_N >= int(n):
                return cls.potts_csr(rowptr, col, val, c_pair, n, num_cases, lin_offset, device, "slots", energy_model,
                                     node_weights)
            n_caller, n = int(n), nslots * 64
            if val64 is not None:
                rowptr, col, val, val64 = pad_csr(rowptr, col, val, seats, n, also=val64)
            else:
                rowptr, col, val = pad_csr(rowptr, col, val, seats, n)
        elif order is not None:
            raise ValueError("order must be None, 'slots' or 'padded'")
        rowptr = np.ascontiguousarray(rowptr, dtype=np.int32)
        col = np.ascontiguousarray(col, dtype=np.int32)
        val = np.ascontiguousarray(val, dtype=np.float32)
        lib = _lib.load()
        h = C.c_void_p()
        _lib.check(lib.mi_sa_problem_create_potts_csr_f32(
            _ptr(rowptr, C.c_int32), _ptr(col, C.c_int32), _ptr(val, C.c_float), float(c_pair),
            int(n), int(num_cases), float(lin_offset), int(device), C.byref(h)))
        if order == "padded":
            prob = cls(h, _lib.KIND_POTTS_CSR, n_caller, int(num_cases), device, seats=seats, n_dev=n)
            absent = np.ones(n, dtype=np.uint8)
            absent[seats] = 0
            rc = lib.mi_sa_problem_set_absent(h, absent.ctypes.data_as(C.POINTER(C.c_uint8)))
            if rc:
                prob.close()
                _lib.check(rc)
        else:
            prob = cls(h, _lib.KIND_POTTS_CSR, int(n), int(num_cases), device, perm=perm)
        if val64 is not None:
            prob._set_energy_model(val64, None, float(energy_model[1]), len(val))
        if node_weights is not None:
            try:
                prob.set_node_weights(*node_weights)
            except Exception:
                prob.close()
                raise
        return prob

    def set_node_weights(self, wq, cw, w64=None):
        wq = np.asarray(wq)
        cw = np.asarray(cw, dtype=np.float32)
        w64 = None if w64 is None else np.asarray(w64, dtype=np.float64)
        if wq.shape != (self.n,) or cw.shape != (self.n,) or (w64 is not None and w64.shape != (self.n,)):
            raise ValueError("node weights need one entry per variable (%d)" % self.n)
        if np.any(wq < 0) or np.any(wq > np.iinfo(np.int32).max):
            raise ValueError("node weights must be non-negative int32 values")
        cols = np.arange(self.n) if self._inv is None else self._inv
        dq = np.zeros(self.n_dev, dtype=np.int32)
        dc = np.zeros(self.n_dev, dtype=np.float32)
        dw = np.zeros(self.n_dev, dtype=np.float64)
        dq[cols] = wq.astype(np.int32)
        dc[cols] = cw
        dw[cols] = wq.astype(np.float64) if w64 is None else w64
        _lib.check(_lib.load().mi_sa_problem_set_node_weights(self._h, _ptr(dq, C.c_int32), _ptr(dc, C.c_float),
                                                               _ptr(dw, C.c_double)))

    def set_node_weight_groups(self, cw, c64, offset):
        cw = np.asarray(cw, dtype=np.float32)
        c64 = np.ascontiguousarray(c64, dtype=np.float64)
        offset = np.ascontiguousarray(offset, dtype=np.float64)
        if cw.ndim != 2 or cw.shape[1] != self.n:
            raise ValueError("cw must have shape [G, n] with n = %d" % self.n)
        G = cw.shape[0]
        if c64.shape != (G,) or offset.shape != (G,):
            raise ValueError("c64 and offset need one entry per group (%d)" % G)
        cols = np.arange(self.n) if self._inv is None else self._inv
        dc = np.zeros((G, self.n_dev), dtype=np.float32)
        dc[:, cols] = cw
        _lib.check(_lib.load().mi_sa_problem_set_node_weight_groups(self._h, int(G), _ptr(dc, C.c_float),
                                                                    _ptr(c64, C.c_double), _ptr(offset, C.c_double)))
        self.groups = int(G)

    def set_merge_moves(self, interval: int, proposals: Optional[int] = None, cq=None):
        if proposals is None:
            proposals = 2 * int(self.num_cases)
        cq_arr = None
        if cq is not None:
            cq_arr = np.ascontiguousarray(np.atleast_1d(np.asarray(cq, dtype=np.float64)))
            if cq_arr.shape != (self.groups,):
                raise ValueError("cq needs one value per resolution group (%d)" % self.groups)
        _lib.check(_lib.load().mi_sa_problem_set_merge_moves(self._h, int(interval), int(proposals),
                                                             _ptr(cq_arr, C.c_double)))

    def merges_accepted(self) -> int:
        return int(self.debug_stats(5)[4])

    def _set_energy_model(self, val64, lin64, c_pair64, nnz):
        if len(val64) != nnz or (lin64 is not None and len(lin64) != self.n_dev):
            self.close()
            raise ValueError("energy_model must have the structure of the fp32 model")
        val64 = np.ascontiguousarray(val64, dtype=np.float64)
        lin64 = None if lin64 is None else np.ascontiguousarray(lin64, dtype=np.float64)
        try:
            _lib.check(_lib.load().mi_sa_problem_set_energy_model_f64(
                self._h, _ptr(val64, C.c_double), None if lin64 is None else _ptr(lin64, C.c_double), float(c_pair64)))
        except Exception:
            self.close()
            raise

    def close(self):
        if self._h is not None and self._h.value:
            _lib.load().mi_sa_problem_destroy(self._h)
        self._h = None

    def __del__(self):
        try:
            self.close()
        except Exception:
            pass

    def __enter__(self):
        return self

    def __exit__(self, *exc):
        self.close()

    def set_option(self, key: str, value: int):
        _lib.check(_lib.load().mi_sa_set_option(self._h, key.encode(), int(value)))

    def debug_pace(self, words: int = 288):
        out = np.zeros(words, dtype=np.uint32)
        _lib.check(_lib.load().mi_sa_debug_pace(self._h, _ptr(out, C.c_uint32), words))
        return out

    def debug_stats(self, words: int = 16):
        out = np.zeros(words, dtype=np.uint64)
        _lib.check(_lib.load().mi_sa_debug_stats(self._h, _ptr(out, C.c_uint64), words))
        return out

    @property
    def state_dtype(self):
        return np.uint16 if self.kind == _lib.KIND_POTTS_CSR else np.uint8

    def anneal(self, num_reads: int, betas, seed: int, replica_offset: int = 0,
               initial_states: Optional[np.ndarray] = None, resync_interval: int = 0,
               sweep_offset: int = 0, continue_run: bool = False, num_sweeps: Optional[int] = None):
        resident = betas is None
        if resident and num_sweeps is None:
            raise ValueError("betas=None (temperatures resident on the device) needs num_sweeps")
        betas = None if resident else np.ascontiguousarray(betas, dtype=np.float64)
        per_replica = num_sweeps is not None
        per_group = not resident and betas.ndim == 2
        if per_group and (per_replica or betas.shape[0] != self.groups):
            raise ValueError("per-group betas need shape [G, num_sweeps] with G = %d groups" % self.groups)
        if per_replica and not resident and len(betas) != num_reads:
            raise ValueError("per-replica betas need one entry per replica")
        flags = (1 if continue_run else 0) | (2 if per_replica else 0) | (4 if resident else 0) | (8 if per_group else 0)
        sweeps = int(num_sweeps) if per_replica else (betas.shape[1] if per_group else len(betas))
        init = None
        if initial_states is not None:
            init = np.ascontiguousarray(initial_states, dtype=self.state_dtype)
            if init.shape != (num_reads, self.n):
                raise ValueError("initial_states must have shape (num_reads, n) = (%d, %d)"
                                 % (num_reads, self.n))
            if self._inv is not None:
                dev = np.zeros((num_reads, self.n_dev), dtype=self.state_dtype)
                dev[:, self._inv] = init
                init = dev
        _lib.check(_lib.load().mi_sa_anneal_ex(
            self._h, int(num_reads), C.c_uint32(int(replica_offset) & 0xFFFFFFFF), sweeps,
            _ptr(betas, C.c_double), C.c_uint64(int(seed) & 0xFFFFFFFFFFFFFFFF),
            init.ctypes.data_as(C.c_void_p) if init is not None else None, int(resync_interval),
            C.c_uint32(int(sweep_offset) & 0xFFFFFFFF), C.c_uint32(flags)))
        self._last = (int(num_reads), sweeps)

    def tempering_begin(self, ladder_betas, chains: int, first_replica: int, num_local: int):
        lad = np.ascontiguousarray(ladder_betas, dtype=np.float64)
        self._pt_total = len(lad) * int(chains)
        _lib.check(_lib.load().mi_sa_tempering_begin(self._h, _ptr(lad, C.c_double), len(lad), int(chains),
                                                     C.c_uint32(int(first_replica)), int(num_local)))

    def tempering_exchange(self, rnd: int, seed: int, all_energies: Optional[np.ndarray] = None):
        en = None if all_energies is None else np.ascontiguousarray(all_energies, dtype=np.float64)
        if en is not None and len(en) != self._pt_total:
            raise ValueError("all_energies must hold the %d energies of the run" % self._pt_total)
        _lib.check(_lib.load().mi_sa_tempering_exchange(self._h, C.c_uint32(int(rnd) & 0xFFFFFFFF),
                                                        C.c_uint64(int(seed) & 0xFFFFFFFFFFFFFFFF), _ptr(en, C.c_double)))

    def tempering_exchange_device(self, rnd: int, seed: int, all_energies_dev):
        if all_energies_dev.numel() != self._pt_total or not all_energies_dev.is_contiguous():
            raise ValueError("all_energies_dev must hold the %d energies of the run, contiguous" % self._pt_total)
        _lib.check(_lib.load().mi_sa_tempering_exchange_dev(self._h, C.c_uint32(int(rnd) & 0xFFFFFFFF),
                                                            C.c_uint64(int(seed) & 0xFFFFFFFFFFFFFFFF),
                                                            C.c_void_p(all_energies_dev.data_ptr())))

    def device_energies(self):
        import torch
        d_en, R = C.c_void_p(), C.c_int(0)
        _lib.check(_lib.load().mi_sa_device_results(self._h, None, C.byref(d_en), C.byref(R)))

        class _Alias:
            __cuda_array_interface__ = {"shape": (int(R.value),), "typestr": "<f8", "data": (int(d_en.value), False),
                                        "version": 2, "strides": None}
        return torch.as_tensor(_Alias(), device=torch.device("cuda", self.device))

    def tempering_state(self):
        rung = np.empty(self._pt_total, dtype=np.int32)
        prop, acc = C.c_uint64(0), C.c_uint64(0)
        _lib.check(_lib.load().mi_sa_tempering_state(self._h, _ptr(rung, C.c_int32), C.byref(prop), C.byref(acc)))
        return rung.astype(np.int64), int(prop.value), int(acc.value)

    def sync(self):
        _lib.check(_lib.load().mi_sa_sync(self._h))

    def kernel_ms(self) -> float:
        ms = C.c_float(0.0)
        _lib.check(_lib.load().mi_sa_last_kernel_ms(self._h, C.byref(ms)))
        return float(ms.value)

    def label_agreement(self, groups: Optional[int] = None) -> dict:
        if self._last is None:
            raise RuntimeError("label_agreement() before anneal()")
        R = self._last[0]
        G = self.groups if groups is None else int(groups)
        if G < 1 or R % G:
            raise ValueError("%d replicas do not split into %d equal groups" % (R, G))
        P = (R // G) * (R // G - 1) // 2
        ari, nmi = np.empty((G, P)), np.empty((G, P))
        S = np.empty((G, P), dtype=np.int64)
        ms = C.c_float(0.0)
        _lib.check(_lib.load().mi_sa_problem_label_agreement(self._h, G, _ptr(ari, C.c_double), _ptr(nmi, C.c_double),
                                                             _ptr(S, C.c_int64), C.byref(ms)))
        return {"ari": ari, "nmi": nmi, "pair_sum": S, "kernel_ms": float(ms.value)}

    def coassociation(self, groups: Optional[int] = None, ref=None, edges=None, matrix: bool = False,
                      hist: bool = True) -> dict:
        from .metrics import _coassoc_outputs, _coassoc_result, _edge_arrays
        if self._last is None:
            raise RuntimeError("coassociation() before anneal()")
        R = self._last[0]
        G = self.groups if groups is None else int(groups)
        if G < 1 or R % G:
            raise ValueError("%d replicas do not split into %d equal groups" % (R, G))
        Rg, n, nd = R // G, self.n, self.n_dev
        cols = np.arange(n) if self._inv is None else np.asarray(self._inv)
        dref, Kref = None, None
        if ref is not None:
            r = np.asarray(ref)
            r = np.broadcast_to(r[None, :], (G, r.shape[0])) if r.ndim == 1 else r
            if r.shape != (G, n) or not np.issubdtype(r.dtype, np.integer) or r.min() < 0 or r.max() >= 64:
                raise ValueError("ref must be (n,) or (groups, n) integer labels in [0, 64)")
            Kref = int(r.max()) + 1
            dref = np.zeros((G, nd), dtype=np.uint16)
            dref[:, cols] = r
        eu = ev = None
        if edges is not None:
            eu, ev = _edge_arrays(edges, n)
            eu = np.ascontiguousarray(cols[eu], dtype=np.int32)
            ev = np.ascontiguousarray(cols[ev], dtype=np.int32)
        hist, rowsum, edge, counts = _coassoc_outputs(G, Rg, nd, Kref, None if eu is None else len(eu), matrix, hist)
        ms = C.c_float(0.0)
        _lib.check(_lib.load().mi_sa_problem_coassociation(
            self._h, G, _ptr(dref, C.c_uint16), int(Kref or 1), _ptr(eu, C.c_int32), _ptr(ev, C.c_int32),
            0 if eu is None else len(eu), _ptr(hist, C.c_int64), _ptr(rowsum, C.c_int64), _ptr(edge, C.c_int32),
            _ptr(counts, C.c_int32), C.byref(ms)))
        if nd != n or self._inv is not None:
            rowsum = None if rowsum is None else np.ascontiguousarray(rowsum[:, cols])
            counts = None if counts is None else np.ascontiguousarray(counts[:, cols][:, :, cols])
        return _coassoc_result(G, Rg, hist, rowsum, edge, counts, ms.value)

    def components(self):
        from .metrics import renumber_by_first_cell
        if self._last is None:
            raise RuntimeError("components() before anneal()")
        R = self._last[0]
        out = np.empty((R, self.n_dev), dtype=np.int32)
        cnt = np.empty(R, dtype=np.int32)
        _lib.check(_lib.load().mi_sa_problem_components(self._h, _ptr(out, C.c_int32), _ptr(cnt, C.c_int32), None))
        if self._inv is not None:
            out = renumber_by_first_cell(np.take(out, self._inv, axis=1))
        return out, cnt

    def launch_count(self) -> int:
        k = C.c_int(0)
        _lib.check(_lib.load().mi_sa_last_launch_count(self._h, C.byref(k)))
        return int(k.value)

    def kernel_name(self) -> str:
        buf = C.create_string_buffer(256)
        _lib.check(_lib.load().mi_sa_last_kernel_name(self._h, buf, 256))
        return buf.value.decode()

    def fetch(self, states: bool = True, energies: bool = True):
        if self._last is None:
            raise RuntimeError("fetch() before anneal()")
        R = self._last[0]
        st = np.empty((R, self.n_dev), dtype=self.state_dtype) if states else None
        en = np.empty(R, dtype=np.float64) if energies else None
        stats = np.zeros(3, dtype=np.uint64)
        _lib.check(_lib.load().mi_sa_fetch(
            self._h, st.ctypes.data_as(C.c_void_p) if st is not None else None,
            _ptr(en, C.c_double), _ptr(stats, C.c_uint64)))
        info = {"proposals": int(R) * int(self._last[1]) * int(self.n),
                "accepted": int(stats[1]), "row_bytes": int(stats[2])}
        if st is not None and self._inv is not None:
            st = np.take(st, self._inv, axis=1)
        return st, en, info

    def best(self, want_state: bool = True):
        idx = C.c_int(0)
        en = C.c_double(0.0)
        key = C.c_uint64(0)
        st = np.empty(self.n_dev, dtype=self.state_dtype) if want_state else None
        _lib.check(_lib.load().mi_sa_best(
            self._h, C.byref(idx), C.byref(en), C.byref(key),
            st.ctypes.data_as(C.c_void_p) if st is not None else None))
        if st is not None and self._inv is not None:
            st = st[self._inv]
        return int(idx.value), float(en.value), int(key.value), st


def energy_dense(Qs: np.ndarray, X: np.ndarray, offset: float = 0.0, device: int = 0, path: int = 0,
                 return_ms: bool = False):
    Qs = np.ascontiguousarray(Qs, dtype=np.float32)
    X = np.ascontiguousarray(X, dtype=np.uint8)
    if X.ndim != 2 or X.shape[1] != Qs.shape[0]:
        raise ValueError("X must have shape (R, n)")
    out = np.empty(X.shape[0], dtype=np.float64)
    ms = C.c_float(0.0)
    _lib.check(_lib.load().mi_energy_dense_f32_ex(_ptr(Qs, C.c_float), Qs.shape[0], _ptr(X, C.c_uint8),
                                                  X.shape[0], float(offset), _ptr(out, C.c_double),
                                                  int(device), int(path), C.byref(ms)))
    return (out, float(ms.value)) if return_ms else out


def energy_dense_f64(Qs: np.ndarray, X: np.ndarray, offset: float = 0.0, device: int = 0) -> np.ndarray:
    Qs = np.ascontiguousarray(Qs, dtype=np.float64)
    X = np.ascontiguousarray(X, dtype=np.uint8)
    if X.ndim != 2 or Qs.ndim != 2 or Qs.shape[0] != Qs.shape[1] or X.shape[1] != Qs.shape[0]:
        raise ValueError("Qs must be n x n and X must have shape (R, n)")
    out = np.empty(X.shape[0], dtype=np.float64)
    _lib.check(_lib.load().mi_energy_dense_f64(_ptr(Qs, C.c_double), Qs.shape[0], _ptr(X, C.c_uint8), X.shape[0],
                                               float(offset), _ptr(out, C.c_double), int(device)))
    return out
```

Measured before the change: 485.7 billion.

## Pack pair-kernel neighbour indices as 16-bit halves and pipeline their unpack

Adds a second adjacency packing for the pair kernel in which the LDS neighbour byte-offsets are stored as 16-bit halves, two per word. This cuts the per-slot adjacency fetch from 8448 to about 6400 bytes, or 6144 when the trimmed row form is used. In the threshold-wavefront D=16 form, the neighbour words for the next slot are fetched one step ahead and unpacked into address registers during the current slot's gather wait, to hide the extra unpack ALU work. It is on by default when there are 256 or fewer slots, costs extra device memory for the new buffers, and adds a query for the bytes fetched per slot.

```diff
diff --git a/include/mi_sa.h b/include/mi_sa.h
--- a/include/mi_sa.h
+++ b/include/mi_sa.h
@@ -92,6 +92,8 @@
 
 int mi_sa_last_kernel_name(mi_sa_problem *p, char *out, int len);
 
+int mi_sa_last_adjacency_bytes_per_slot(mi_sa_problem *p, int *out_bytes);
+
 int mi_sa_fetch(mi_sa_problem *p, void *out_states, double *out_energy, uint64_t *out_stats);
 
 int mi_sa_problem_label_agreement(mi_sa_problem *p, int groups, double *out_ari, double *out_nmi, int64_t *out_pair_sum,
diff --git a/scrna_seq_qannealing_clustering_amd/_lib.py b/scrna_seq_qannealing_clustering_amd/_lib.py
--- a/scrna_seq_qannealing_clustering_amd/_lib.py
+++ b/scrna_seq_qannealing_clustering_amd/_lib.py
@@ -64,6 +64,7 @@
         "mi_sa_last_kernel_ms": (C.c_int, [vp, f32p]),
         "mi_sa_last_launch_count": (C.c_int, [vp, ip]),
         "mi_sa_last_kernel_name": (C.c_int, [vp, C.c_char_p, C.c_int]),
+        "mi_sa_last_adjacency_bytes_per_slot": (C.c_int, [vp, ip]),
         "mi_sa_fetch": (C.c_int, [vp, vp, f64p, u64p]),
         "mi_sa_best": (C.c_int, [vp, ip, f64p, u64p, vp]),
         "mi_multi_gpu_anneal": (C.c_int, [pp, C.c_int, C.c_int, C.c_uint32, C.c_int, f64p, C.c_uint64, C.c_int]),
@@ -120,7 +121,7 @@
     "mi_last_error", "mi_abi_version", "mi_device_count", "mi_device_info",
     "mi_sa_problem_create_dense_f32", "mi_sa_problem_create_csr_rank1_f32",
     "mi_sa_problem_create_potts_csr_f32", "mi_sa_problem_destroy", "mi_sa_problem_info",
-    "mi_sa_set_option", "mi_sa_plan_slot_order", "mi_sa_plan_slot_layout", "mi_sa_problem_set_absent", "mi_sa_problem_set_pair_weights", "mi_sa_problem_set_node_weights", "mi_sa_problem_set_node_weight_groups", "mi_sa_problem_set_merge_moves", "mi_sa_problem_set_energy_model_f64", "mi_sa_debug_pace", "mi_sa_debug_stats", "mi_sa_anneal", "mi_sa_anneal_ex", "mi_sa_tempering_begin", "mi_sa_tempering_exchange", "mi_sa_tempering_exchange_dev", "mi_sa_device_results", "mi_sa_tempering_state", "mi_sa_sync", "mi_sa_last_kernel_ms", "mi_sa_last_launch_count", "mi_sa_last_kernel_name", "mi_sa_fetch", "mi_sa_best",
+    "mi_sa_last_adjacency_bytes_per_slot", "mi_sa_set_option", "mi_sa_plan_slot_order", "mi_sa_plan_slot_layout", "mi_sa_problem_set_absent", "mi_sa_problem_set_pair_weights", "mi_sa_problem_set_node_weights", "mi_sa_problem_set_node_weight_groups", "mi_sa_problem_set_merge_moves", "mi_sa_problem_set_energy_model_f64", "mi_sa_debug_pace", "mi_sa_debug_stats", "mi_sa_anneal", "mi_sa_anneal_ex", "mi_sa_tempering_begin", "mi_sa_tempering_exchange", "mi_sa_tempering_exchange_dev", "mi_sa_device_results", "mi_sa_tempering_state", "mi_sa_sync", "mi_sa_last_kernel_ms", "mi_sa_last_launch_count", "mi_sa_last_kernel_name", "mi_sa_fetch", "mi_sa_best",
     "mi_multi_gpu_anneal", "mi_multi_gpu_best", "mi_multi_gpu_fetch", "mi_sa_qubo_dense_f32", "mi_energy_dense_f32", "mi_energy_dense_f64", "mi_energy_dense_f32_ex",
     "mi_snn_build_f32", "mi_snn_build_ex_f32", "mi_snn_build_rounded_f32", "mi_snn_fetch_codes", "mi_snn_info", "mi_snn_fetch", "mi_snn_kernel_ms", "mi_snn_destroy",
     "mi_jaccard_cluster_stats", "mi_label_agreement_u16", "mi_sa_problem_label_agreement",
diff --git a/scrna_seq_qannealing_clustering_amd/csrc/mi_sa.hip b/scrna_seq_qannealing_clustering_amd/csrc/mi_sa.hip
--- a/scrna_seq_qannealing_clustering_amd/csrc/mi_sa.hip
+++ b/scrna_seq_qannealing_clustering_amd/csrc/mi_sa.hip
@@ -153,6 +153,9 @@
     uint4 *d_adj4r = nullptr;
     int k2p_rw = 0;
     std::vector<uint32_t> h_adj4r;
+    uint4 *d_adj16 = nullptr;
+    uint4 *d_adj16r = nullptr;
+    std::vector<uint32_t> h_adj16;
     uint32_t *d_slot_flags = nullptr;
     int k2_state_bytes = 0;
     int32_t *d_wgt = nullptr;
@@ -196,6 +199,8 @@
     int opt_k3_fast = 0;
     int opt_k2_tw = 0;
     int opt_k2_trim = 0;
+    int opt_k2_nbr16 = 0;
+    int last_adj_bytes = 0;
     int opt_k2_split_max = 1024;
     int opt_unit_rows = 0;
     int resident_waves = 0;
@@ -425,6 +430,23 @@
                 }
                 out[at_col] = 4u * hc[((size_t)t * D + k) * 64 + lane];
                 memcpy(&out[at_val], &hv[((size_t)t * D + k) * 64 + lane], 4);
+            }
+    return out;
+}
+
+static std::vector<uint32_t> pack_pair_adjacency16(const std::vector<uint32_t> &hc, const std::vector<float> &hv, int slots, int D)
+{
+    const int G = D / 4;
+    const size_t slot_words = (size_t)(G / 2 + G) * 256;
+    std::vector<uint32_t> out((size_t)slots * slot_words, 0u);
+    for (int t = 0; t < slots; ++t)
+        for (int lane = 0; lane < 64; ++lane)
+            for (int k = 0; k < D; ++k) {
+                const size_t src = ((size_t)t * D + k) * 64 + lane;
+                const size_t at_nbr = (size_t)t * slot_words + (size_t)(k / 8) * 256 + (size_t)lane * 4 + ((k / 2) & 3);
+                const size_t at_val = (size_t)t * slot_words + (size_t)(G / 2 + k / 4) * 256 + (size_t)lane * 4 + (k & 3);
+                out[at_nbr] |= (4u * hc[src]) << (16 * (k & 1));
+                memcpy(&out[at_val], &hv[src], 4);
             }
     return out;
 }
@@ -560,6 +582,7 @@
                                 4u * hc[((size_t)t * D + k) * 64 + lane];
                 HIP_TRY(hipMalloc((void **)&p->d_adj4p, ha.size() * sizeof(uint32_t)));
                 HIP_TRY(hipMemcpy(p->d_adj4p, ha.data(), ha.size() * sizeof(uint32_t), hipMemcpyHostToDevice));
+                if (slots <= 256) p->h_adj16 = pack_pair_adjacency16(hc, hv, slots, D);
                 if (D == 16 && maxdeg >= 13 && maxdeg < 16) {
                     p->h_adj4r = pack_pair_adjacency(hc, hv, slots, D, maxdeg);
                     p->k2p_rw = maxdeg;
@@ -760,6 +783,18 @@
             HIP_TRY(hipMemcpy(p->d_adj4r, p->h_adj4r.data(), p->h_adj4r.size() * sizeof(uint32_t), hipMemcpyHostToDevice));
             std::vector<uint32_t>().swap(p->h_adj4r);
         }
+        if (!p->h_adj16.empty()) {
+            HIP_TRY(hipMalloc((void **)&p->d_adj16, p->h_adj16.size() * sizeof(uint32_t)));
+            HIP_TRY(hipMemcpy(p->d_adj16, p->h_adj16.data(), p->h_adj16.size() * sizeof(uint32_t), hipMemcpyHostToDevice));
+            if (p->k2p_rw) {
+                for (int t = 0; t < p->slots; ++t)
+                    for (int lane = 0; lane < 64; ++lane)
+                        memcpy(&p->h_adj16[(size_t)t * 1536 + 5 * 256 + (size_t)lane * 4 + 3], &hl[(size_t)t * 64 + lane], 4);
+                HIP_TRY(hipMalloc((void **)&p->d_adj16r, p->h_adj16.size() * sizeof(uint32_t)));
+                HIP_TRY(hipMemcpy(p->d_adj16r, p->h_adj16.data(), p->h_adj16.size() * sizeof(uint32_t), hipMemcpyHostToDevice));
+            }
+            std::vector<uint32_t>().swap(p->h_adj16);
+        }
         return MI_OK;
     });
     if (rc) { mi_sa_problem_destroy(p); return rc; }
@@ -992,7 +1027,7 @@
     (void)settle(p);
     (void)hipSetDevice(p->device);
     if (p->stream) (void)hipStreamSynchronize(p->stream);
-    void *bufs[] = {p->d_merge_cq, p->d_gconst, p->d_nwq, p->d_ncw, p->d_nw64, p->d_wgt, p->d_xg, p->d_pt_rung, p->d_pt_betas, p->d_pt_energy, p->d_pt_ladder, p->d_pt_temps, p->d_pt_stats, p->d_adj4p, p->d_adj4r, p->d_ell_val64, p->d_lin64, p->d_Q2xl, p->d_diagxl, p->d_rows, p->d_meta, p->d_adj4, p->d_slot_flags, p->d_Qm, p->d_fields, p->d_ctrl, p->d_ell_col, p->d_ell_val, p->d_lin, p->d_pace, p->d_Qp, p->d_Qs, p->d_temps, p->d_init, p->d_states, p->d_energy, p->d_stats};
+    void *bufs[] = {p->d_merge_cq, p->d_gconst, p->d_nwq, p->d_ncw, p->d_nw64, p->d_wgt, p->d_xg, p->d_pt_rung, p->d_pt_betas, p->d_pt_energy, p->d_pt_ladder, p->d_pt_temps, p->d_pt_stats, p->d_adj4p, p->d_adj4r, p->d_adj16, p->d_adj16r, p->d_ell_val64, p->d_lin64, p->d_Q2xl, p->d_diagxl, p->d_rows, p->d_meta, p->d_adj4, p->d_slot_flags, p->d_Qm, p->d_fields, p->d_ctrl, p->d_ell_col, p->d_ell_val, p->d_lin, p->d_pace, p->d_Qp, p->d_Qs, p->d_temps, p->d_init, p->d_states, p->d_energy, p->d_stats};
     for (void *b : bufs)
         if (b) (void)hipFree(b);
     if (p->ev0) (void)hipEventDestroy(p->ev0);
@@ -1060,6 +1095,7 @@
     if (!strcmp(key, "k2_wide") && value >= 0 && value <= 2) { p->opt_k2_wide = (int)value; return MI_OK; }
     if (!strcmp(key, "k2_tw") && value >= 0 && value <= 2) { p->opt_k2_tw = (int)value; return MI_OK; }
     if (!strcmp(key, "k2_trim") && value >= 0 && value <= 2) { p->opt_k2_trim = (int)value; return MI_OK; }
+    if (!strcmp(key, "k2_nbr16") && value >= 0 && value <= 2) { p->opt_k2_nbr16 = (int)value; return MI_OK; }
     if (!strcmp(key, "k3_fast") && value >= 0 && value <= 2) { p->opt_k3_fast = (int)value; return MI_OK; }
     if (!strcmp(key, "min_cluster_size") && value >= 0) {
         if (p->kind != MI_KIND_POTTS_CSR) return fail(MI_EINVAL, "min_cluster_size applies to Potts problems");
@@ -1122,6 +1158,7 @@
     if (!resident || init)
         HIP_TRY(hipStreamSynchronize(p->stream));
     g_kernel.clear();
+    p->last_adj_bytes = 0;
     const float *temps_buf = resident ? p->d_pt_temps : p->d_temps;
 
     if (p->kind == MI_KIND_DENSE && p->xl_chunks > 0) {
@@ -1315,7 +1352,9 @@
                 rc = mi_launch_csr_rank1_split(a, p->k2_free_block / 64, p->stream);
             } else if (choice == 1) {
                 a.adj4 = p->d_adj4p;
-                rc = mi_launch_csr_rank1_pair(a, p->opt_k2_pair == 1 ? (tw && p->D == 16 && pair_wgs <= 8 * cus) : tw_pair, p->stream);
+                const bool n16 = p->opt_k2_nbr16 != 2;
+                rc = mi_launch_csr_rank1_pair(a, p->opt_k2_pair == 1 ? (tw && p->D == 16 && pair_wgs <= 8 * cus) : tw_pair, p->stream,
+                                              n16 ? p->d_adj16 : nullptr, n16 && p->opt_k2_trim != 2 ? p->d_adj16r : nullptr, &p->last_adj_bytes);
             } else {
                 rc = mi_launch_csr_rank1(a, p->stream, tw && R <= 1024 && (p->D == 16 || p->D == 32) && p->k2_state_bytes <= 1);
             }
@@ -1484,6 +1523,15 @@
     return MI_OK;
 }
 
+int mi_sa_last_adjacency_bytes_per_slot(mi_sa_problem *p, int *out_bytes)
+{
+    if (!p || !out_bytes) return fail(MI_EINVAL, "NULL argument");
+    if (const int rc_w = settle(p)) return rc_w;
+    if (!p->has_run) return fail(MI_ESTATE, "no anneal has been run on this problem");
+    *out_bytes = p->last_adj_bytes;
+    return MI_OK;
+}
+
 int mi_sa_last_kernel_name(mi_sa_problem *p, char *out, int len)
 {
     if (!p || !out || len < 1) return fail(MI_EINVAL, "NULL argument");
diff --git a/scrna_seq_qannealing_clustering_amd/csrc/mi_sa_device.h b/scrna_seq_qannealing_clustering_amd/csrc/mi_sa_device.h
--- a/scrna_seq_qannealing_clustering_amd/csrc/mi_sa_device.h
+++ b/scrna_seq_qannealing_clustering_amd/csrc/mi_sa_device.h
@@ -312,7 +312,7 @@
     return v;
 }
 int mi_launch_csr_rank1(const EllArgs &, hipStream_t, bool tw = false);
-int mi_launch_csr_rank1_pair(const EllArgs &, bool tw, hipStream_t);
+int mi_launch_csr_rank1_pair(const EllArgs &, bool tw, hipStream_t, const uint4 *adj16 = nullptr, const uint4 *adj16_trim = nullptr, int *adj_bytes = nullptr);
 int mi_launch_csr_rank1_split(const EllArgs &, int nw, hipStream_t);
 int mi_launch_csr_rank1_wide(const EllArgs &, int spb, bool tw, hipStream_t);
 int mi_launch_potts(const EllArgs &, hipStream_t);
diff --git a/scrna_seq_qannealing_clustering_amd/csrc/sparse_pair_kernels.hip b/scrna_seq_qannealing_clustering_amd/csrc/sparse_pair_kernels.hip
--- a/scrna_seq_qannealing_clustering_amd/csrc/sparse_pair_kernels.hip
+++ b/scrna_seq_qannealing_clustering_amd/csrc/sparse_pair_kernels.hip
@@ -15,10 +15,12 @@
 __device__ __forceinline__ float half_lo(uint32_t w) { return (float)__builtin_bit_cast(half_t, (uint16_t)w); }
 __device__ __forceinline__ float half_hi(uint32_t w) { return (float)__builtin_bit_cast(half_t, (uint16_t)(w >> 16)); }
 
-template <int D, bool TW, bool WGT = false, int RW = D>
+template <int D, bool TW, bool WGT = false, int RW = D, int N16 = 0>
 __global__ void __launch_bounds__(TW ? 128 : 64, TW ? 1 : 2) k_anneal_csr_rank1_pair(EllArgs a)
 {
     static_assert(RW > D - 4 && RW <= D, "trimmed rows drop part of the last group of four only");
+    static_assert(N16 == 0 || !WGT, "the weighted form keeps the 32-bit packing");
+    static_assert(N16 != 2 || (TW && D == 16), "the pipelined unpack lives in the threshold-wavefront form's gather window");
     extern __shared__ __attribute__((aligned(16))) char lds[];
     const int lane = threadIdx.x & 63;
     const int pair = blockIdx.x;
@@ -103,18 +105,52 @@
 
     constexpr int G = D / 4;
     constexpr int LW = RW - 4 * (G - 1);
-    constexpr int SLOT_BYTES = (G - 1) * 2048 + (LW == 3 ? 1792 : LW * 512);
+    constexpr int GC = N16 ? G / 2 : G;
+    constexpr int SLOT_BYTES = N16 ? (GC + G) * 1024 : (G - 1) * 2048 + (LW == 3 ? 1792 : LW * 512);
     const __amdgpu_buffer_rsrc_t rs_adj = __builtin_amdgcn_make_buffer_rsrc(
         const_cast<uint4 *>(a.adj4), 0, slots * SLOT_BYTES, 0x00020000);
     const __amdgpu_buffer_rsrc_t rs_lin = __builtin_amdgcn_make_buffer_rsrc(
         const_cast<float *>(a.lin), 0, slots * 256, 0x00020000);
-    struct SlotAdj { u32x4 col[G]; u32x4 val[G]; uint32_t lin; };
+    struct SlotAdj { u32x4 col[GC]; u32x4 val[G]; uint32_t lin; };
+    struct NbrPack { u32x4 w[GC]; };
     const int lane16 = lane * 16;
+    auto fetch_block16 = [&](int t, int b) {
+        const int tt = t < slots ? t : slots - 1;
+        return __builtin_amdgcn_raw_buffer_load_b128(rs_adj, lane16 + (b & 3) * 1024, tt * SLOT_BYTES + (b >> 2) * 4096, 0);
+    };
+    auto fetch_nbr16 = [&](int t) {
+        NbrPack q;
+#pragma unroll
+        for (int b = 0; b < GC; ++b) q.w[b] = fetch_block16(t, b);
+        return q;
+    };
+    auto fetch_val16 = [&](int t) {
+        SlotAdj p;
+#pragma unroll
+        for (int g = 0; g < G; ++g) p.val[g] = fetch_block16(t, GC + g);
+        if constexpr (RW < D) p.lin = p.val[G - 1][3];
+        else p.lin = __builtin_amdgcn_raw_buffer_load_b32(rs_lin, lane * 4, (t < slots ? t : slots - 1) * 256, 0);
+        return p;
+    };
+    uint32_t m16 = 0xffffu;
+    asm("" : "+s"(m16));
+    auto unpack16 = [&](const u32x4 *w, int e) -> uint32_t {
+        const uint32_t pw = w[e / 8][(e / 2) & 3];
+        return (e & 1) ? pw >> 16 : (pw & m16);
+    };
+    uint32_t addr[16];
 #ifdef MI_K2P_NOFETCH
     auto fetch_real = [&](int t) {
 #else
     auto fetch_adj = [&](int t) {
 #endif
+        if constexpr (N16 != 0) {
+            SlotAdj p = fetch_val16(t);
+            const NbrPack q = fetch_nbr16(t);
+#pragma unroll
+            for (int b = 0; b < GC; ++b) p.col[b] = q.w[b];
+            return p;
+        }
         SlotAdj p;
         const int tt = t < slots ? t : slots - 1;
         const int soff = tt * SLOT_BYTES;
@@ -160,7 +196,7 @@
     const float cp = a.c_pair;
     uint32_t ring_buf = 0u;
 
-    auto slot_body = [&](auto c_in_group, int t, const SlotAdj &cur, uint32_t wordA, uint32_t wordB) {
+    auto slot_body = [&](auto c_in_group, int t, const SlotAdj &cur, NbrPack &nxt, uint32_t wordA, uint32_t wordB) {
         constexpr int C = decltype(c_in_group)::value;
         const int i = t * 64 + lane;
         uint32_t own;
@@ -197,13 +233,28 @@
 #ifdef MI_K2P_DBG_LINEAR
                 asm volatile("ds_read_b32 %0, %1" : "=v"(word[k]) : "v"((cur.col[g0 + k / 4][k & 3] & 0x3f00u) + lane * 4));
 #else
+                {
+                    if constexpr (N16 == 2) asm volatile("ds_read_b32 %0, %1" : "=v"(word[k]) : "v"(addr[k]));
+                    else if constexpr (N16 == 1) asm volatile("ds_read_b32 %0, %1" : "=v"(word[k]) : "v"(unpack16(cur.col, 4 * g0 + k)));
+                    else
                 asm volatile("ds_read_b32 %0, %1" : "=v"(word[k]) : "v"(cur.col[g0 + k / 4][k & 3]));
+                }
 #endif
             if (g0 == 0 && TW) {
+                if constexpr (N16 == 2)
+                    asm volatile("s_waitcnt lgkmcnt(%4)" : "+v"(own), "+v"(thr2), "+v"(nxt.w[0]), "+v"(nxt.w[1]) : "n"(NK0 < 15 ? NK0 : 15) : "memory");
+                else
                 asm volatile("s_waitcnt lgkmcnt(%2)" : "+v"(own), "+v"(thr2) : "n"(NK0 < 15 ? NK0 : 15) : "memory");
 #ifndef MI_K2P_DBG_TERMS_AFTER
                 own_terms();
 #endif
+                if constexpr (N16 == 2) {
+#pragma unroll
+                    for (int k = 0; k < NK0; ++k) {
+                        addr[k] = unpack16(nxt.w, k);
+                        asm volatile("" : "+v"(addr[k]));
+                    }
+                }
                 asm volatile("s_waitcnt lgkmcnt(0)"
                              : "+v"(word[0]), "+v"(word[1]), "+v"(word[2]), "+v"(word[3]), "+v"(word[4]), "+v"(word[5]),
                                "+v"(word[6]), "+v"(word[7]), "+v"(word[8]), "+v"(word[9]), "+v"(word[10]), "+v"(word[11]),
@@ -301,30 +352,62 @@
             }
         }
         const uint32_t sw = (uint32_t)s + a.sweep_offset;
-        SlotAdj P = fetch_adj(0), Q;
+        if constexpr (N16 == 2) {
+            SlotAdj P = fetch_val16(0), Q;
+            NbrPack NA = fetch_nbr16(0), NB;
+#pragma unroll
+            for (int k = 0; k < (RW < 16 ? RW : 16); ++k) addr[k] = unpack16(NA.w, k);
+            NA = fetch_nbr16(1);
 #pragma unroll 1
-        for (int t = 0; t < slots; t += 4) {
-            if constexpr (TW) {
+            for (int t = 0; t < slots; t += 4) {
                 K2P_TICK(t_top);
                 __builtin_amdgcn_s_barrier();
                 K2P_TICK(t_barrier);
-            } else {
-                philox4x32_10((uint32_t)((t >> 2) * 64 + lane), sw, gidA, 0u, a.seed_lo, a.seed_hi, wa);
-                philox4x32_10((uint32_t)((t >> 2) * 64 + lane), sw, gidB, 0u, a.seed_lo, a.seed_hi, wb);
-            }
-            Q = fetch_adj(t + 1);
-            slot_body(integral_constant<int, 0>{}, t, P, wa[0], wb[0]);
-            if (t + 1 < slots) {
-                P = fetch_adj(t + 2);
-                slot_body(integral_constant<int, 1>{}, t + 1, Q, wa[1], wb[1]);
-                if (t + 2 < slots) {
-                    Q = fetch_adj(t + 3);
-                    slot_body(integral_constant<int, 2>{}, t + 2, P, wa[2], wb[2]);
-                    P = fetch_adj(t + 4);
-                    if (t + 3 < slots) slot_body(integral_constant<int, 3>{}, t + 3, Q, wa[3], wb[3]);
-                }
-            }
-            if constexpr (TW) ring_buf ^= 2048u;
+                Q = fetch_val16(t + 1);
+                NB = fetch_nbr16(t + 2);
+                slot_body(integral_constant<int, 0>{}, t, P, NA, wa[0], wb[0]);
+                if (t + 1 < slots) {
+                    P = fetch_val16(t + 2);
+                    NA = fetch_nbr16(t + 3);
+                    slot_body(integral_constant<int, 1>{}, t + 1, Q, NB, wa[1], wb[1]);
+                    if (t + 2 < slots) {
+                        Q = fetch_val16(t + 3);
+                        NB = fetch_nbr16(t + 4);
+                        slot_body(integral_constant<int, 2>{}, t + 2, P, NA, wa[2], wb[2]);
+                        P = fetch_val16(t + 4);
+                        NA = fetch_nbr16(t + 5);
+                        if (t + 3 < slots) slot_body(integral_constant<int, 3>{}, t + 3, Q, NB, wa[3], wb[3]);
+                    }
+                }
+                ring_buf ^= 2048u;
+            }
+        } else {
+            NbrPack none;
+            SlotAdj P = fetch_adj(0), Q;
+    #pragma unroll 1
+            for (int t = 0; t < slots; t += 4) {
+                if constexpr (TW) {
+                    K2P_TICK(t_top);
+                    __builtin_amdgcn_s_barrier();
+                    K2P_TICK(t_barrier);
+                } else {
+                    philox4x32_10((uint32_t)((t >> 2) * 64 + lane), sw, gidA, 0u, a.seed_lo, a.seed_hi, wa);
+                    philox4x32_10((uint32_t)((t >> 2) * 64 + lane), sw, gidB, 0u, a.seed_lo, a.seed_hi, wb);
+                }
+                Q = fetch_adj(t + 1);
+                slot_body(integral_constant<int, 0>{}, t, P, none, wa[0], wb[0]);
+                if (t + 1 < slots) {
+                    P = fetch_adj(t + 2);
+                    slot_body(integral_constant<int, 1>{}, t + 1, Q, none, wa[1], wb[1]);
+                    if (t + 2 < slots) {
+                        Q = fetch_adj(t + 3);
+                        slot_body(integral_constant<int, 2>{}, t + 2, P, none, wa[2], wb[2]);
+                        P = fetch_adj(t + 4);
+                        if (t + 3 < slots) slot_body(integral_constant<int, 3>{}, t + 3, Q, none, wa[3], wb[3]);
+                    }
+                }
+                if constexpr (TW) ring_buf ^= 2048u;
+            }
         }
         accepted += (unsigned long long)accA + (liveB ? (unsigned long long)accB : 0ull);
         accA = accB = 0;
@@ -391,22 +474,42 @@
 
 }
 
-int mi_launch_csr_rank1_pair(const EllArgs &a, bool tw, hipStream_t st)
+int mi_launch_csr_rank1_pair(const EllArgs &a, bool tw, hipStream_t st, const uint4 *adj16, const uint4 *adj16_trim, int *adj_bytes)
 {
     if (!a.adj4) return fail(MI_EHIP, "csr_rank1 pair kernel: packed adjacency missing");
+#ifdef MI_K2P_NOFETCH
+    adj16 = adj16_trim = nullptr;
+#endif
     if (tw && ((size_t)a.slots * 256 + 4096) * 8 > 160 * 1024 && a.R > 2 * 7 * 256) tw = false;
+    auto fetches = [&](int bytes) { if (adj_bytes) *adj_bytes = bytes; };
     if (a.wslot >= 0) {
         if (a.D != 16) return fail(MI_EUNSUPPORTED, "csr_rank1 pair kernel: pair-term weights at slot-ELL width %d not built", a.D);
+        fetches(8448);
         return tw ? launch_pair(k_anneal_csr_rank1_pair<16, true, true>, a, true, st)
                   : launch_pair(k_anneal_csr_rank1_pair<16, false, true>, a, false, st);
     }
+    EllArgs b = a;
+    if (a.D == 16 && tw && a.adj4_trim && adj16_trim) {
+        b.adj4 = adj16_trim;
+        fetches(6144);
+        if (a.trim_rw == 15) return launch_pair(k_anneal_csr_rank1_pair<16, true, false, 15, 2>, b, true, st, 15);
+        if (a.trim_rw == 14) return launch_pair(k_anneal_csr_rank1_pair<16, true, false, 14, 2>, b, true, st, 14);
+        if (a.trim_rw == 13) return launch_pair(k_anneal_csr_rank1_pair<16, true, false, 13, 2>, b, true, st, 13);
+    }
     if (a.D == 16 && tw && a.adj4_trim) {
-        EllArgs b = a;
         b.adj4 = a.adj4_trim;
+        fetches(a.trim_rw == 15 ? 7936 : (a.trim_rw == 14 ? 7424 : 6912));
         if (a.trim_rw == 15) return launch_pair(k_anneal_csr_rank1_pair<16, true, false, 15>, b, true, st, 15);
         if (a.trim_rw == 14) return launch_pair(k_anneal_csr_rank1_pair<16, true, false, 14>, b, true, st, 14);
         if (a.trim_rw == 13) return launch_pair(k_anneal_csr_rank1_pair<16, true, false, 13>, b, true, st, 13);
     }
+    if (adj16 && ((a.D == 16 && tw) || a.D == 32)) {
+        b.adj4 = adj16;
+        fetches(a.D == 16 ? 6400 : 12544);
+        if (a.D == 16) return launch_pair(k_anneal_csr_rank1_pair<16, true, false, 16, 2>, b, true, st);
+        return launch_pair(k_anneal_csr_rank1_pair<32, false, false, 32, 1>, b, false, st);
+    }
+    fetches(a.D == 16 ? 8448 : 16640);
     if (a.D == 16 && tw) return launch_pair(k_anneal_csr_rank1_pair<16, true>, a, true, st);
     if (a.D == 16) return launch_pair(k_anneal_csr_rank1_pair<16, false>, a, false, st);
     if (a.D == 32) return launch_pair(k_anneal_csr_rank1_pair<32, false>, a, false, st);
diff --git a/scrna_seq_qannealing_clustering_amd/engine.py b/scrna_seq_qannealing_clustering_amd/engine.py
--- a/scrna_seq_qannealing_clustering_amd/engine.py
+++ b/scrna_seq_qannealing_clustering_amd/engine.py
@@ -477,6 +477,11 @@
         _lib.check(_lib.load().mi_sa_last_kernel_name(self._h, buf, 256))
         return buf.value.decode()
 
+    def adjacency_bytes_per_slot(self) -> int:
+        k = C.c_int(0)
+        _lib.check(_lib.load().mi_sa_last_adjacency_bytes_per_slot(self._h, C.byref(k)))
+        return int(k.value)
+
     def fetch(self, states: bool = True, energies: bool = True):
         if self._last is None:
             raise RuntimeError("fetch() before anneal()")
```

Result: faster. 502.3 billion (median of 6 runs) (+3.4%).
